# WarranWeng/EBFI-BE

Hardware: AMD Instinct MI355X
Metric: interpolated frames/sec (train fwd+bwd) at B=8 256x256 (higher is better)
Workload: dtype bf16x3 fwd (f16 KernelConv) / f16 bwd; 1 GPU; EVFIAutoEx (config/train_ours.yml defaults, 5.69 M params) train step: fwd + Lap/census loss + bwd + flat grad all-reduce + Adam; B=8 per GPU, 256x256 frames, TB=16 event bins, Poisson(0.35) event counts; global_batch=8, parallelism=dp1, world_size=1, launch=hipGraph replay of fwd+loss+bwd+grad packing; all-reduce and Adam eager, graph_capture_failed=False, fp16_steps_skipped=0

## Files before the change

ebfi-be_amd/csrc/conv2d.hip:

```cpp
#include <type_traits>

#include "common.hpp"
#include "c16.hpp"

using namespace ebfi;

namespace {

typedef float f32x16 __attribute__((ext_vector_type(16)));

enum { ACT_NONE = 0, ACT_LEAKY = 1, ACT_SIGMOID = 2 };

struct ConvGeom {
    int B, Cin, H, W, Cout, Ho, Wo, pad;
    int groups = 1;
    int store = 0;
};

struct EpiExtra {
    const float *addend;
    const float *mask_y;
    int mask_act;
    float mask_slope;
    _Float16 *out16 = nullptr;
    float *slot16 = nullptr;
    int planar16 = 0;
    const _Float16 *mask16 = nullptr;
    const float *post_scale = nullptr;
    const float *post_res = nullptr;
    int post_resC = 0;
    _Float16 *pre16 = nullptr;
    float *pre_slot = nullptr;
};

__device__ __forceinline__ float act_apply(float v, int act, float slope) {
    if (act == ACT_LEAKY) return v > 0.f ? v : v * slope;
    if (act == ACT_SIGMOID) return 1.f / (1.f + __expf(-v));
    return v;
}
__device__ __forceinline__ float act_grad(float y, int act, float slope) {
    if (act == ACT_LEAKY) return y > 0.f ? 1.f : slope;
    if (act == ACT_SIGMOID) return y * (1.f - y);
    return 1.f;
}

template <int DACT>
__device__ __forceinline__ float act_grad_c(float y, float slope) {
    if constexpr (DACT == ACT_LEAKY) return y > 0.f ? 1.f : slope;
    else if constexpr (DACT == ACT_SIGMOID) return y * (1.f - y);
    else return 1.f;
}

constexpr int TY = 4, TX = 64;

constexpr unsigned SENT = 0x80000000u;
__device__ __forceinline__ __amdgpu_buffer_rsrc_t make_rsrc(const float *p, unsigned bytes) {
    return __builtin_amdgcn_make_buffer_rsrc(const_cast<float *>(p), 0, bytes, 0x00020000);
}
template <int N>
__device__ __forceinline__ void wait_vmcnt() {
    static_assert(N >= 0 && N < 64, "vmcnt is a 6-bit counter");
    __builtin_amdgcn_s_waitcnt(((N >> 4) << 14) | (0x7 << 4) | (0xf << 8) | (N & 15));
}
__device__ __forceinline__ unsigned sel_off(bool ok, unsigned off) {
    asm volatile("" : "+v"(off));
    return ok ? off : 0x80000000u;
}
__device__ __forceinline__ float buf_ld(__amdgpu_buffer_rsrc_t r, unsigned byte_off) {
    return __uint_as_float(__builtin_amdgcn_raw_buffer_load_b32(r, byte_off, 0, 0));
}
__device__ __forceinline__ void buf_st(__amdgpu_buffer_rsrc_t r, unsigned byte_off, float v) {
    __builtin_amdgcn_raw_buffer_store_b32(__float_as_uint(v), r, byte_off, 0, 0);
}

template <int MT, int XM = 0>
__device__ __forceinline__ void store_out_tile(float *__restrict__ out, const float *__restrict__ bias, const f32x16 (&acc)[MT][2],
                                               const ConvGeom &g, int b, int co_base, int yo, int x0, int lane, int act,
                                               float slope, EpiExtra ex = EpiExtra{nullptr, nullptr, 0, 0.f}, float oscale = 1.f,
                                               float *amax16 = nullptr, float *amax_pre = nullptr) {
    const int HWo = g.Ho * g.Wo;
    const unsigned plane = (unsigned)HWo * 4u;
    constexpr bool EXTRA = (XM & 7) != 0, XAM = (XM & 1) != 0, X16 = (XM & 2) != 0, XRC = (XM & 4) != 0;
    constexpr bool XST = (XM & 8) != 0;
    if constexpr (EXTRA) {
        asm volatile("" : "+v"(lane));
    }
    const bool has32 = out != nullptr;
    const float *anyp = bias ? bias : (out ? out : reinterpret_cast<const float *>(ex.slot16));
    const __amdgpu_buffer_rsrc_t ro = make_rsrc(has32 ? out + (int64_t)b * g.Cout * HWo : anyp, has32 ? (unsigned)g.Cout * plane : 0u);
    const __amdgpu_buffer_rsrc_t rb = make_rsrc(bias ? bias : anyp, bias ? (unsigned)g.Cout * 4u : 0u);
    const bool has_a = XAM && ex.addend != nullptr, has_m = XAM && ex.mask_y != nullptr, has16 = X16 && ex.out16 != nullptr;
    const bool has_m16 = XAM && ex.mask16 != nullptr;
    const __amdgpu_buffer_rsrc_t ra = make_rsrc(has_a ? ex.addend + (int64_t)b * g.Cout * HWo : anyp, has_a ? (unsigned)g.Cout * plane : 0u);
    const __amdgpu_buffer_rsrc_t rm = make_rsrc(has_m ? ex.mask_y + (int64_t)b * g.Cout * HWo : anyp, has_m ? (unsigned)g.Cout * plane : 0u);
    const int cb16 = g.Cout >> 4;
    const bool planar = X16 && ex.planar16 != 0;
    const __amdgpu_buffer_rsrc_t rm16 = __builtin_amdgcn_make_buffer_rsrc(
        has_m16 ? const_cast<_Float16 *>(ex.mask16) + (int64_t)b * cb16 * HWo * 16 : const_cast<_Float16 *>(reinterpret_cast<const _Float16 *>(anyp)), 0,
        has_m16 ? (unsigned)cb16 * (unsigned)HWo * 32u : 0u, 0x00020000);
    const __amdgpu_buffer_rsrc_t r16 = __builtin_amdgcn_make_buffer_rsrc(
        has16 ? ex.out16 + (planar ? (int64_t)b * g.Cout * HWo : (int64_t)b * cb16 * HWo * 16)
              : const_cast<_Float16 *>(reinterpret_cast<const _Float16 *>(anyp)), 0,
        has16 ? (planar ? (unsigned)g.Cout * (unsigned)HWo * 2u : (unsigned)cb16 * (unsigned)HWo * 32u) : 0u, 0x00020000);
    const float s16 = has16 ? ex.slot16[0] : 1.f;
    const bool has_rc = XRC && ex.post_scale != nullptr;
    const __amdgpu_buffer_rsrc_t rps = make_rsrc(has_rc ? ex.post_scale + (int64_t)b * g.Cout : anyp, has_rc ? (unsigned)g.Cout * 4u : 0u);
    const __amdgpu_buffer_rsrc_t rrs = make_rsrc(has_rc ? ex.post_res + (int64_t)b * ex.post_resC * HWo : anyp,
                                                 has_rc ? (unsigned)ex.post_resC * plane : 0u);
    const bool has_p16 = has_rc && ex.pre16 != nullptr;
    const __amdgpu_buffer_rsrc_t rp16 = __builtin_amdgcn_make_buffer_rsrc(
        has_p16 ? ex.pre16 + (int64_t)b * cb16 * HWo * 16 : const_cast<_Float16 *>(reinterpret_cast<const _Float16 *>(anyp)), 0,
        has_p16 ? (unsigned)cb16 * (unsigned)HWo * 32u : 0u, 0x00020000);
    const float sp16 = has_p16 ? ex.pre_slot[0] : 1.f;
    const int res_shift = has_rc ? co_base - co_base % ex.post_resC : 0;
    float am = 0.f, amp = 0.f;
    const int h = lane >> 5, l31 = lane & 31;
    struct BlockIn {
        float add[8];
        float my[8];
        unsigned m16[4];
        float res[8];
    };
    auto shuffled_base = [&](int m) { return (unsigned)(((co_base + m * 32) >> 2) + h) * 4u * plane; };
    auto unshuffled_base = [&](int m, bool px_ok, int xo) {
        return px_ok ? (unsigned)(4 * (co_base + m * 32 + 4 * h) + 2 * (yo & 1) + (xo & 1)) * (plane >> 2) +
                           (unsigned)((yo >> 1) * (g.Wo >> 1) + (xo >> 1)) * 4u
                     : SENT;
    };
    auto blk_geom = [&](int m, int n, int j, bool &px_ok, unsigned &base, int &cblk, int &xo) {
        xo = x0 + n * 32 + l31;
        px_ok = yo < g.Ho && xo < g.Wo;
        base = (px_ok && co_base + m * 32 + 4 * h < g.Cout) ? (unsigned)(co_base + m * 32 + 4 * h) * plane + (unsigned)(yo * g.Wo + xo) * 4u : SENT;
        cblk = ((co_base + m * 32) >> 4) + j;
    };
    auto row_off = [](int j, int i) { return (unsigned)((i & 3) + 8 * (2 * j + (i >> 2))); };
    [[maybe_unused]] auto issue = [&](int m, int n, int j, BlockIn &in) {
        bool px_ok; unsigned base; int cblk, xo;
        blk_geom(m, n, j, px_ok, base, cblk, xo);
        if constexpr (XAM) {
            if (has_a) {
#pragma unroll
                for (int i = 0; i < 8; ++i) in.add[i] = buf_ld(ra, base + row_off(j, i) * plane);
            }
            if (has_m) {
#pragma unroll
                for (int i = 0; i < 8; ++i) in.my[i] = buf_ld(rm, base + row_off(j, i) * plane);
            }
            if (has_m16) {
                typedef unsigned u32x2_m __attribute__((ext_vector_type(2)));
                const unsigned om = (px_ok && cblk < cb16) ? ((unsigned)cblk * (unsigned)HWo * 2u + (unsigned)(yo * 2 * g.Wo + xo)) * 16u + 8u * (unsigned)h : SENT;
                const u32x2_m lo = __builtin_amdgcn_raw_buffer_load_b64(rm16, om, 0, 0);
                const u32x2_m hi = __builtin_amdgcn_raw_buffer_load_b64(rm16, om + (unsigned)g.Wo * 16u, 0, 0);
                in.m16[0] = lo.x; in.m16[1] = lo.y; in.m16[2] = hi.x; in.m16[3] = hi.y;
            }
        }
        if constexpr (XRC) {
            if (has_rc) {
                const unsigned rbase = base == SENT ? SENT : base - (unsigned)res_shift * plane;
#pragma unroll
                for (int i = 0; i < 8; ++i) in.res[i] = buf_ld(rrs, rbase + row_off(j, i) * plane);
            }
        }
    };
    [[maybe_unused]] auto finish = [&](int m, int n, int j, const BlockIn &in, auto actf) {
        bool px_ok; unsigned base; int cblk, xo;
        blk_geom(m, n, j, px_ok, base, cblk, xo);
        float u[8];
#pragma unroll
        for (int i = 0; i < 8; ++i) u[i] = acc[m][n][8 * j + i] * oscale;
        [[maybe_unused]] float psc[8];
        if constexpr (XRC) {
            if (has_rc) {
#pragma unroll
                for (int i = 0; i < 8; ++i) psc[i] = buf_ld(rps, (unsigned)(co_base + m * 32 + 4 * h) * 4u + row_off(j, i) * 4u);
            }
        }
        if (bias != nullptr) {
            float t[8];
#pragma unroll
            for (int i = 0; i < 8; ++i) t[i] = buf_ld(rb, (unsigned)(co_base + m * 32 + 4 * h) * 4u + row_off(j, i) * 4u);
#pragma unroll
            for (int i = 0; i < 8; ++i) u[i] += t[i];
        }
        if constexpr (XAM) {
            if (has_a) {
#pragma unroll
                for (int i = 0; i < 8; ++i) u[i] += in.add[i];
            }
        }
#pragma unroll
        for (int i = 0; i < 8; ++i) u[i] = actf(u[i]);
        if constexpr (XAM) {
            if (has_m) {
#pragma unroll
                for (int i = 0; i < 8; ++i) u[i] *= in.my[i] > 0.f ? 1.f : ex.mask_slope;
            }
            if (has_m16) {
#pragma unroll
                for (int i = 0; i < 8; ++i) {
                    const unsigned hbits = (in.m16[i >> 1] >> (16 * (i & 1))) & 0xffffu;
                    u[i] *= (hbits != 0u && hbits < 0x8000u) ? 1.f : ex.mask_slope;
                }
            }
        }
        if constexpr (XRC) {
            if (has_rc) {
                if (has_p16) {
                    const unsigned o16 = (px_ok && cblk < cb16) ? ((unsigned)cblk * (unsigned)HWo * 2u + (unsigned)((yo * 2 + h) * g.Wo + xo)) * 16u : SENT;
#pragma unroll
                    for (int i = 0; i < 8; ++i) amp = amax_acc(amp, u[i]);
                    const u32x4_c16 q = c16_gather_halves(pack_f16(u[0] * sp16, u[1] * sp16), pack_f16(u[2] * sp16, u[3] * sp16),
                                                          pack_f16(u[4] * sp16, u[5] * sp16), pack_f16(u[6] * sp16, u[7] * sp16));
                    __builtin_amdgcn_raw_buffer_store_b128(q, rp16, o16, 0, 0);
                }
#pragma unroll
                for (int i = 0; i < 8; ++i) u[i] = u[i] * psc[i] + in.res[i];
            }
        }
        if (has32) {
            if (XST && g.store == 1) {
                const unsigned b1 = px_ok ? shuffled_base(m) + (unsigned)(2 * yo * 2 * g.Wo + 2 * xo) * 4u : SENT;
#pragma unroll
                for (int q = 0; q < 2; ++q) {
#pragma unroll
                    for (int py = 0; py < 2; ++py) {
                        typedef float f32x2_st __attribute__((ext_vector_type(2)));
                        typedef unsigned u32x2_st __attribute__((ext_vector_type(2)));
                        const f32x2_st v{u[4 * q + 2 * py], u[4 * q + 2 * py + 1]};
                        __builtin_amdgcn_raw_buffer_store_b64(__builtin_bit_cast(u32x2_st, v), ro,
                                                              b1 + (unsigned)(2 * (2 * j + q)) * 4u * plane + (unsigned)(py * 2 * g.Wo) * 4u, 0, 0);
                    }
                }
            } else {
                const unsigned sb = (XST && g.store == 2) ? unshuffled_base(m, px_ok, xo) : base;
#pragma unroll
                for (int i = 0; i < 8; ++i) __builtin_amdgcn_raw_buffer_store_b32(__float_as_uint(u[i]), ro, sb + row_off(j, i) * plane, 0, 0);
            }
        }
        if constexpr (X16) {
            if (has16) {
#pragma unroll
                for (int i = 0; i < 8; ++i) am = amax_acc(am, u[i]);
                if (planar) {
                    const unsigned pb = (px_ok && co_base + m * 32 + 4 * h < g.Cout)
                                            ? (unsigned)(co_base + m * 32 + 4 * h) * (unsigned)HWo * 2u + (unsigned)(yo * g.Wo + xo) * 2u : SENT;
#pragma unroll
                    for (int i = 0; i < 8; ++i) {
                        const _Float16 hv = (_Float16)(u[i] * s16);
                        __builtin_amdgcn_raw_buffer_store_b16(__builtin_bit_cast(unsigned short, hv), r16, pb + row_off(j, i) * (unsigned)HWo * 2u, 0, 0);
                    }
                } else {
                    const u32x4_c16 q = c16_gather_halves(pack_f16(u[0] * s16, u[1] * s16), pack_f16(u[2] * s16, u[3] * s16),
                                                          pack_f16(u[4] * s16, u[5] * s16), pack_f16(u[6] * s16, u[7] * s16));
                    const unsigned o16 = (px_ok && cblk < cb16)
                                             ? ((unsigned)cblk * (unsigned)HWo * 2u + (unsigned)((yo * 2 + h) * g.Wo + xo)) * 16u : SENT;
                    __builtin_amdgcn_raw_buffer_store_b128(q, r16, o16, 0, 0);
                }
            }
        }
    };
    auto emit = [&](auto actf) {
        if constexpr (EXTRA) {
            constexpr int NBLK = MT * 4;
            BlockIn ia, ib;
            issue(0, 0, 0, ia);
#pragma unroll
            for (int k = 0; k < NBLK; ++k) {
                const int m = k >> 2, n = (k >> 1) & 1, j = k & 1;
                if (k + 1 < NBLK) issue((k + 1) >> 2, ((k + 1) >> 1) & 1, (k + 1) & 1, (k & 1) ? ia : ib);
                finish(m, n, j, (k & 1) ? ib : ia, actf);
                __builtin_amdgcn_sched_barrier(0);
            }
        } else {
#pragma unroll
            for (int m = 0; m < MT; ++m) {
                float bvm[16];
#pragma unroll
                for (int r = 0; r < 16; ++r) bvm[r] = buf_ld(rb, (unsigned)(co_base + m * 32 + (r & 3) + 8 * (r >> 2) + 4 * h) * 4u);
#pragma unroll
                for (int n = 0; n < 2; ++n) {
                    const int xo = x0 + n * 32 + l31;
                    const bool px_ok = yo < g.Ho && xo < g.Wo;
                    if (XST && g.store == 1) {
                        const unsigned b1 = px_ok ? shuffled_base(m) + (unsigned)(2 * yo * 2 * g.Wo + 2 * xo) * 4u : SENT;
#pragma unroll
                        for (int k = 0; k < 4; ++k) {
#pragma unroll
                            for (int py = 0; py < 2; ++py) {
                                typedef float f32x2_st __attribute__((ext_vector_type(2)));
                                typedef unsigned u32x2_st __attribute__((ext_vector_type(2)));
                                const int r = 4 * k + 2 * py;
                                const f32x2_st v{actf(acc[m][n][r] * oscale + bvm[r]), actf(acc[m][n][r + 1] * oscale + bvm[r + 1])};
                                __builtin_amdgcn_raw_buffer_store_b64(__builtin_bit_cast(u32x2_st, v), ro,
                                                                      b1 + (unsigned)(2 * k) * 4u * plane + (unsigned)(py * 2 * g.Wo) * 4u, 0, 0);
                            }
                        }
                        continue;
                    }
                    const unsigned base = (XST && g.store == 2) ? unshuffled_base(m, px_ok, xo)
                                          : (px_ok && co_base + m * 32 + 4 * h < g.Cout)
                                              ? (unsigned)(co_base + m * 32 + 4 * h) * plane + (unsigned)(yo * g.Wo + xo) * 4u : SENT;
#pragma unroll
                    for (int r = 0; r < 16; ++r)
                        __builtin_amdgcn_raw_buffer_store_b32(__float_as_uint(actf(acc[m][n][r] * oscale + bvm[r])), ro,
                                                              base + (unsigned)((r & 3) + 8 * (r >> 2)) * plane, 0, 0);
                }
            }
        }
    };
    if constexpr (EXTRA) {
        const float sl = act == ACT_LEAKY ? slope : 1.f;
        emit([sl](float v) { return v > 0.f ? v : v * sl; });
    } else {
        if (act == ACT_LEAKY) emit([slope](float v) { return v > 0.f ? v : v * slope; });
        else if (act == ACT_SIGMOID) emit([](float v) { return 1.f / (1.f + __expf(-v)); });
        else emit([](float v) { return v; });
    }
    if (amax16) *amax16 = amax_acc(*amax16, am);
    if constexpr (XRC) {
        if (amax_pre) *amax_pre = amax_acc(*amax_pre, amp);
    }
}

struct FacEpi {
    const float *ev;
    int C;
};

template <int MT>
__device__ __forceinline__ void fac_epilogue_tile(float *__restrict__ out, const float *__restrict__ bias, const f32x16 (&acc)[MT][2],
                                                  const ConvGeom &g, const FacEpi &fac, int b, int co_base, int yo, int x0, int lane,
                                                  float slope, float oscale = 1.f) {
    constexpr int K = 5, R = 2;
    const int HW = g.Ho * g.Wo;
    const int h = lane >> 5, l31 = lane & 31;
    const __amdgpu_buffer_rsrc_t rb = make_rsrc(bias, (unsigned)g.Cout * 4u);
    float part[MT][2];
#pragma unroll
    for (int m = 0; m < MT; ++m) {
        const int c = (co_base >> 5) + m;
        const bool c_ok = c < fac.C;
        const __amdgpu_buffer_rsrc_t rev = make_rsrc(fac.ev + ((int64_t)b * fac.C + (c_ok ? c : 0)) * HW, c_ok ? (unsigned)HW * 4u : 0u);
        float bv[16];
#pragma unroll
        for (int r = 0; r < 16; ++r) bv[r] = buf_ld(rb, (unsigned)(co_base + m * 32 + (r & 3) + 8 * (r >> 2) + 4 * h) * 4u);
#pragma unroll
        for (int n = 0; n < 2; ++n) {
            const int xo = x0 + n * 32 + l31;
            unsigned rowoff[K], coloff[K];
#pragma unroll
            for (int i = 0; i < K; ++i) {
                rowoff[i] = (unsigned)(min(max(yo + i - R, 0), g.Ho - 1) * g.Wo) * 4u;
                coloff[i] = (unsigned)min(max(xo + i - R, 0), g.Wo - 1) * 4u;
            }
            float e[16];
#pragma unroll
            for (int r = 0; r < 16; ++r) {
                constexpr int dummy = 0;
                const int t0 = (r & 3) + 8 * (r >> 2), t1 = t0 + 4;
                const unsigned o0 = t0 < K * K ? rowoff[t0 / K] + coloff[t0 % K] : rowoff[dummy] + coloff[dummy];
                const unsigned o1 = t1 < K * K ? rowoff[t1 / K] + coloff[t1 % K] : rowoff[dummy] + coloff[dummy];
                e[r] = buf_ld(rev, h ? o1 : o0);
            }
            float sum = 0.f;
#pragma unroll
            for (int r = 0; r < 16; ++r) {
                float f = acc[m][n][r] * oscale + bv[r];
                f = f > 0.f ? f : f * slope;
                sum = fmaf(f, e[r], sum);
            }
            part[m][n] = sum;
        }
    }
#pragma unroll
    for (int m = 0; m < MT; ++m) {
        const int c = (co_base >> 5) + m;
        const float p0 = part[m][0] + __shfl_xor(part[m][0], 32, 64);
        const float p1 = part[m][1] + __shfl_xor(part[m][1], 32, 64);
        const int xo = x0 + h * 32 + l31;
        if (c < fac.C && yo < g.Ho && xo < g.Wo) out[((int64_t)b * fac.C + c) * HW + (int64_t)yo * g.Wo + xo] = h ? p1 : p0;
    }
}

template <int KS, int S, int MT, int CK, bool TR, int DACT>
__global__ __launch_bounds__(256) void conv_fwd_f32(const float *__restrict__ x, const float *__restrict__ dact_y,
                                                    const float *__restrict__ w, const float *__restrict__ bias,
                                                    float *__restrict__ out, ConvGeom g, int act, float slope,
                                                    float dslope) {
    constexpr int KK = KS * KS;
    constexpr int IH = S * (TY - 1) + KS, IW = S * (TX - 1) + KS;
    constexpr int PS = IH * IW;
    constexpr int COS = 32 * MT;
    constexpr int COSP = TR ? COS + 4 : COS + 1;
    constexpr int NPOS = (PS + 255) / 256;
    constexpr int WEL = KK * CK * COS;
    constexpr int NW = (WEL + 255) / 256;
    __shared__ float sIn[CK * PS];
    __shared__ float sW[KK * CK * COSP];

    const int tid = threadIdx.x, lane = tid & 63, wave = tid >> 6;
    const int tiles_x = (g.Wo + TX - 1) / TX, tiles_y = (g.Ho + TY - 1) / TY;
    int t = blockIdx.x;
// ... 1786 lines not shown
int launch_wgrad_x3_w(hipStream_t st, const float *x, const float *gout, const float *yact, float *slab, float *gpre_out,
                      const ConvGeom &g, float dslope, int nsplit, int need_bias) {
    using C = WCfg<KS, 1, WTXO>;
    constexpr int CIB = CIBT ? CIBT : X3CIB<KS>::value;
    const size_t lds = (size_t)2 * (64 * GS + (CIB + 1) * C::PS) * sizeof(unsigned);
    if (int rc = ensure_dynamic_lds(reinterpret_cast<const void *>(&conv_wgrad_x3<KS, WTXO, DACT, WX, CIBT>), (int)lds)) return rc;
    const int64_t tiles = (int64_t)g.B * ceil_div(g.Ho, WTY) * ceil_div(g.Wo, C::WTX);
    dim3 grid((unsigned)nsplit, (unsigned)ceil_div(g.Cout, 64), (unsigned)ceil_div(g.Cin, CIB));
    ProfScope ps("conv_wgrad_x3", st, 2.0 * g.B * g.Ho * g.Wo * (double)g.Cout * g.Cin * KS * KS,
                 conv_bytes_wgrad(g, KS * KS, DACT != 0, gpre_out != nullptr));
    hipLaunchKernelGGL((conv_wgrad_x3<KS, WTXO, DACT, WX, CIBT>), grid, dim3(WX), lds, st, x, gout, yact, slab, gpre_out, g, dslope,
                       (int)tiles, need_bias);
    return check_launch("conv_wgrad_x3");
}

template <int DACT>
int launch_wgrad_x3_ws(hipStream_t st, const float *x, const float *gout, const float *yact, float *slab, float *gpre_out,
                       const ConvGeom &g, float dslope, int nsplit, int need_bias) {
    using C = WCfg<3, 1, 32>;
    const size_t lds = (size_t)2 * (64 * GS + 65 * C::PS) * sizeof(unsigned);
    if (int rc = ensure_dynamic_lds(reinterpret_cast<const void *>(&conv_wgrad_x3_ws<DACT>), (int)lds)) return rc;
    const int64_t tiles = (int64_t)g.B * ceil_div(g.Ho, WTY) * ceil_div(g.Wo, C::WTX);
    dim3 grid((unsigned)nsplit, (unsigned)ceil_div(g.Cout, 64), (unsigned)ceil_div(g.Cin, 64));
    ProfScope ps("conv_wgrad_x3_ws", st, 2.0 * g.B * g.Ho * g.Wo * (double)g.Cout * g.Cin * 9,
                 conv_bytes_wgrad(g, 9, DACT != 0, gpre_out != nullptr));
    hipLaunchKernelGGL((conv_wgrad_x3_ws<DACT>), grid, dim3(512), lds, st, x, gout, yact, slab, gpre_out, g, dslope, (int)tiles, need_bias);
    return check_launch("conv_wgrad_x3_ws");
}

template <int KS, int WTXO, int DACT>
int launch_wgrad_x3_d(hipStream_t st, const float *x, const float *gout, const float *yact, float *slab, float *gpre_out,
                      const ConvGeom &g, float dslope, int nsplit, int need_bias) {
    if constexpr (KS == 3) {
        if (wgrad_x3_ws(g, KS)) return launch_wgrad_x3_ws<DACT>(st, x, gout, yact, slab, gpre_out, g, dslope, nsplit, need_bias);
        if (wgrad_x3_small_wg(g, KS))
            return launch_wgrad_x3_w<KS, WTXO, DACT, 256, 32>(st, x, gout, yact, slab, gpre_out, g, dslope, nsplit, need_bias);
    }
    return launch_wgrad_x3_w<KS, WTXO, DACT, WXT, 0>(st, x, gout, yact, slab, gpre_out, g, dslope, nsplit, need_bias);
}

template <int KS, int WTXO>
int launch_wgrad_x3_t(hipStream_t st, const float *x, const float *gout, const float *yact, float *slab, float *gpre_out,
                      const ConvGeom &g, int dact, float dslope, int nsplit, int need_bias) {
    if (dact == ACT_LEAKY) return launch_wgrad_x3_d<KS, WTXO, ACT_LEAKY>(st, x, gout, yact, slab, gpre_out, g, dslope, nsplit, need_bias);
    if (dact == ACT_SIGMOID) return launch_wgrad_x3_d<KS, WTXO, ACT_SIGMOID>(st, x, gout, yact, slab, gpre_out, g, dslope, nsplit, need_bias);
    return launch_wgrad_x3_d<KS, WTXO, ACT_NONE>(st, x, gout, yact, slab, gpre_out, g, dslope, nsplit, need_bias);
}

int launch_wgrad_x3(hipStream_t st, const float *x, const float *gout, const float *yact, float *slab, float *gpre_out,
                    const ConvGeom &g, int ks, int dact, float dslope, int nsplit, int need_bias) {
    if (ks == 1) return launch_wgrad_x3_t<1, 0>(st, x, gout, yact, slab, gpre_out, g, dact, dslope, nsplit, need_bias);
    if (ks == 7) return launch_wgrad_x3_t<7, 32>(st, x, gout, yact, slab, gpre_out, g, dact, dslope, nsplit, need_bias);
    return launch_wgrad_x3_t<3, 32>(st, x, gout, yact, slab, gpre_out, g, dact, dslope, nsplit, need_bias);
}

template <int KS, int DACT>
int launch_wgrad_bf16_d(hipStream_t st, const float *x, const float *gout, const float *yact, float *slab, const ConvGeom &g,
                        float dslope, int nsplit, int need_bias) {
    using C = WCfgB<KS>;
    const size_t lds = (size_t)C::LDS_ELEMS * 2;
    if (int rc = ensure_dynamic_lds(reinterpret_cast<const void *>(&conv_wgrad_bf16<KS, DACT>), (int)lds)) return rc;
    const int64_t tiles = (int64_t)g.B * ceil_div(g.Ho, WTY) * ceil_div(g.Wo, C::WTX);
    dim3 grid((unsigned)nsplit, (unsigned)ceil_div(g.Cout, 64), (unsigned)ceil_div(g.Cin, C::CIB));
    ProfScope ps("conv_wgrad_bf16", st, 2.0 * g.B * g.Ho * g.Wo * (double)g.Cout * g.Cin * KS * KS,
                 conv_bytes_wgrad(g, KS * KS, DACT != 0, false));
    hipLaunchKernelGGL((conv_wgrad_bf16<KS, DACT>), grid, dim3(256), lds, st, x, gout, yact, slab, g, dslope, (int)tiles,
                       need_bias);
    return check_launch("conv_wgrad_bf16");
}

template <int KS>
int launch_wgrad_bf16(hipStream_t st, const float *x, const float *gout, const float *yact, float *slab, const ConvGeom &g,
                      int dact, float dslope, int nsplit, int need_bias) {
    if (dact == ACT_LEAKY) return launch_wgrad_bf16_d<KS, ACT_LEAKY>(st, x, gout, yact, slab, g, dslope, nsplit, need_bias);
    if (dact == ACT_SIGMOID) return launch_wgrad_bf16_d<KS, ACT_SIGMOID>(st, x, gout, yact, slab, g, dslope, nsplit, need_bias);
    return launch_wgrad_bf16_d<KS, ACT_NONE>(st, x, gout, yact, slab, g, dslope, nsplit, need_bias);
}

constexpr int NTWS = 768;
template <int XM, bool FAC = false>
__global__ __launch_bounds__(NTWS) void conv_fwd_bf16x3_ws(const float *__restrict__ x, const __bf16 *__restrict__ wp,
                                                           const float *__restrict__ bias, float *__restrict__ out, ConvGeom g, int K16,
                                                           int act, float slope, EpiExtra epi, int tiles_total, FacEpi fac) {
    constexpr bool EXTRA = (XM & 7) != 0;
    constexpr int KS = 3, KK = 9, MT = 2;
    constexpr int IH = TYB - 1 + KS, IW = TX - 1 + KS, PS = IH * IW, COS = 32 * MT;
    constexpr int NCW = 8, PT = 256;
    constexpr int WPIECES = KK * COS * 2, NWB = (2 * WPIECES + PT - 1) / PT;
    constexpr int INB = PS * 32, WB = KK * COS * 32, BUFB = 2 * INB + 2 * WB;
    extern __shared__ __attribute__((aligned(16))) char smd[];
    const int tid = threadIdx.x, lane = tid & 63, wave = tid >> 6;
    const int tiles_x = (g.Wo + TX - 1) / TX, tiles_y = (g.Ho + TYB - 1) / TYB;
    const int co_base = blockIdx.y * COS;
    const int grp = co_base / (g.Cout / g.groups);
    const int HW = g.H * g.W;
    const unsigned plane_bytes = (unsigned)HW * 4u, x_bytes = (unsigned)g.Cin * plane_bytes;
    const int nchunks = K16 / CKB;
    const int G = gridDim.x;
    int ntiles_mine = 0;
    for (int t = blockIdx.x; t < tiles_total; t += G) ++ntiles_mine;
    const int nitems = ntiles_mine * nchunks;
    const bool xcd_map = (gridDim.x & 7) == 0;
    auto tile_coords = [&](int tt, int &tb, int &ty0, int &tx0) {
        int u = xcd_map ? xcd_tile(tt, tiles_total) : tt;
        const int txi = u % tiles_x; u /= tiles_x;
        const int tyi = u % tiles_y;
        tb = u / tiles_y; ty0 = tyi * TYB; tx0 = txi * TX;
    };

    if (wave < NCW) {
        __builtin_amdgcn_s_setprio(1);
        f32x16 acc[MT][2];
#pragma unroll
        for (int m = 0; m < MT; ++m)
#pragma unroll
            for (int n = 0; n < 2; ++n)
#pragma unroll
                for (int e = 0; e < 16; ++e) acc[m][n][e] = 0.f;
        const int hsel = lane >> 5, l31 = lane & 31;
        const int a_lane = 2 * INB + l31 * 32 + ((hsel ^ ((l31 >> 3) & 1)) << 4);
        const int pbase = wave * IW + l31;
        unsigned fbits = 0;
#pragma unroll
        for (int tap = 0; tap < KK; ++tap)
            fbits |= (unsigned)((((pbase + (tap / KS) * IW + (tap % KS)) >> 3) & 1) ^ hsel) << tap;
        bf16x8 ah[2][MT], al[2][MT], bh[2][2], bl[2][2];
        [[maybe_unused]] float amax16 = 0.f, amax_pre = 0.f;
        auto tap_read = [&](const char *base, int tap, int set) {
            const int ky = tap / KS, kx = tap - ky * KS;
            const char *bp = base + pbase * 32 + (int)(((fbits >> tap) & 1u) << 4) + (ky * IW + kx) * 32;
            const char *ap = base + a_lane + tap * COS * 32;
#pragma unroll
            for (int m = 0; m < MT; ++m) {
                ah[set][m] = *reinterpret_cast<const bf16x8 *>(ap + m * 1024);
#ifndef ABL_ONE_MFMA
                al[set][m] = *reinterpret_cast<const bf16x8 *>(ap + m * 1024 + WB);
#endif
            }
#pragma unroll
            for (int n = 0; n < 2; ++n) {
                bh[set][n] = *reinterpret_cast<const bf16x8 *>(bp + n * 1024);
#ifndef ABL_ONE_MFMA
                bl[set][n] = *reinterpret_cast<const bf16x8 *>(bp + n * 1024 + INB);
#endif
            }
        };
        auto tap_mfma = [&](int set) {
#pragma unroll
            for (int m = 0; m < MT; ++m)
#pragma unroll
                for (int n = 0; n < 2; ++n) {
#ifndef ABL_ONE_MFMA
                    acc[m][n] = __builtin_amdgcn_mfma_f32_32x32x16_bf16(al[set][m], bh[set][n], acc[m][n], 0, 0, 0);
                    acc[m][n] = __builtin_amdgcn_mfma_f32_32x32x16_bf16(ah[set][m], bl[set][n], acc[m][n], 0, 0, 0);
#endif
                    acc[m][n] = __builtin_amdgcn_mfma_f32_32x32x16_bf16(ah[set][m], bh[set][n], acc[m][n], 0, 0, 0);
                }
        };
        __syncthreads();
        int item = 0, tcur = blockIdx.x;
        for (int ti = 0; ti < ntiles_mine; ++ti, tcur += G) {
            for (int chunk = 0; chunk < nchunks; ++chunk, ++item) {
                const char *base = smd + (item & 1) * BUFB;
#ifdef WSF_NO_CONSUME
                if (g.pad != 12345) { } else
#endif
                {
                    tap_read(base, 0, 0);
#pragma unroll
                    for (int tap = 0; tap < KK; ++tap) {
                        if (tap + 1 < KK) tap_read(base, tap + 1, (tap + 1) & 1);
                        __builtin_amdgcn_sched_barrier(0);
                        tap_mfma(tap & 1);
                        __builtin_amdgcn_sched_barrier(0);
                    }
                }
                __syncthreads();
            }
            int cb_, cy0, cx0;
            tile_coords(tcur, cb_, cy0, cx0);
            if constexpr (FAC) {
                fac_epilogue_tile<MT>(out, bias, acc, g, fac, cb_, co_base, cy0 + wave, cx0, lane, slope);
            } else {
                if constexpr ((XM & 6) != 0) saturate_fp16_conversions(true);
                store_out_tile<MT, XM>(out, bias, acc, g, cb_, co_base, cy0 + wave, cx0, lane, act, slope, epi, 1.f, &amax16, &amax_pre);
                if constexpr ((XM & 6) != 0) saturate_fp16_conversions(false);
            }
#pragma unroll
            for (int m = 0; m < MT; ++m)
#pragma unroll
                for (int n = 0; n < 2; ++n)
#pragma unroll
                    for (int e = 0; e < 16; ++e) acc[m][n][e] = 0.f;
        }
        if constexpr (EXTRA) {
            if (epi.out16 != nullptr) ScaleSlot{epi.slot16}.record(amax16);
            if constexpr ((XM & 4) != 0) {
                if (epi.pre16 != nullptr) ScaleSlot{epi.pre_slot}.record(amax_pre);
            }
        }
        return;
    }
    const int ptid = tid - 64 * NCW;
    const unsigned img_bytes = (unsigned)KK * (unsigned)g.Cout * (unsigned)K16 * 2u;
    const __amdgpu_buffer_rsrc_t rwt = __builtin_amdgcn_make_buffer_rsrc(const_cast<__bf16 *>(wp), 0, 2u * img_bytes, 0x00020000);
    constexpr int SH = (4 - (KS / 2) % 4) % 4;
    constexpr int NQ = (IW + SH + 3) / 4;
    constexpr int NITEM = IH * NQ * 2;
    constexpr int NIT = (NITEM + PT - 1) / PT;
    int it_qh[NIT], it_qr[NIT], it_qq[NIT];
#pragma unroll
    for (int k = 0; k < NIT; ++k) {
        const int id = ptid + k * PT;
        it_qh[k] = id & 1;
        it_qr[k] = (id >> 1) / NQ;
        it_qq[k] = (id >> 1) - it_qr[k] * NQ;
    }
    unsigned w_off[NWB];
    int w_dst[NWB];
#pragma unroll
    for (int it = 0; it < NWB; ++it) {
        const int i = ptid + it * PT;
        const int sel = i >= WPIECES ? 1 : 0, j = i - sel * WPIECES;
        const int row = j >> 1, half = j & 1;
        const int tap = row / COS, co = row - tap * COS;
        w_off[it] = i < 2 * WPIECES ? (unsigned)sel * img_bytes + (unsigned)(((tap * g.Cout + co_base + co) * K16 + half * 8) * 2) : SENT;
        w_dst[it] = 2 * INB + sel * WB + row * 32 + ((half ^ ((row >> 3) & 1)) << 4);
    }
    u32x4 rq[NIT][8];
    u32x4 rw[NWB];
    int pf_tile = blockIdx.x, pf_chunk = 0;
    unsigned pf_off[NIT];
    const float *pf_src = x;
    unsigned pf_bytes = 0u;
    auto pf_setup = [&]() {
        const bool live = pf_tile < tiles_total;
        int tb, ty0, tx0;
        tile_coords(live ? pf_tile : 0, tb, ty0, tx0);
#pragma unroll
        for (int k = 0; k < NIT; ++k) {
            const int yy = ty0 - g.pad + it_qr[k], xq = tx0 - g.pad - SH + 4 * it_qq[k];
            const bool ok = live && ptid + k * PT < NITEM && yy >= 0 && yy < g.H && xq >= 0 && xq + 3 < g.W;
            pf_off[k] = ok ? (unsigned)(yy * g.W + xq) * 4u + (unsigned)(8 * it_qh[k]) * plane_bytes : SENT;
        }
        pf_src = x + ((int64_t)tb * g.groups + grp) * g.Cin * HW;
        pf_bytes = live ? x_bytes : 0u;
    };
    auto prefetch = [&]() {
        const __amdgpu_buffer_rsrc_t r = make_rsrc(pf_src, pf_bytes);
        const unsigned cb = (unsigned)pf_chunk * (unsigned)CKB * plane_bytes;
#pragma unroll
        for (int k = 0; k < NIT; ++k)
#pragma unroll
            for (int c = 0; c < 8; ++c) rq[k][c] = __builtin_amdgcn_raw_buffer_load_b128(r, pf_off[k] + cb + (unsigned)c * plane_bytes, 0, 0);
        const unsigned wb = (unsigned)pf_chunk * (unsigned)(CKB * 2);
#pragma unroll
        for (int it = 0; it < NWB; ++it) {
#ifdef ABL_ONE_MFMA
            if (ptid + it * PT >= WPIECES) continue;
#endif
            rw[it] = __builtin_amdgcn_raw_buffer_load_b128(rwt, w_off[it] + wb, 0, 0);
        }
        if (++pf_chunk == nchunks) {
            pf_chunk = 0;
            pf_tile += G;
            pf_setup();
        }
    };
    auto commit = [&](int buf) {
        char *base = smd + buf * BUFB;
#pragma unroll
        for (int k = 0; k < NIT; ++k)
            if (ptid + k * PT < NITEM) {
#pragma unroll
                for (int j = 0; j < 4; ++j) {
                    const int c = 4 * it_qq[k] + j - SH;
                    if (c < 0 || c >= IW) continue;
                    u32x4 hv, lv;
#pragma unroll
                    for (int e = 0; e < 8; e += 2) {
                        const float v0 = __uint_as_float(rq[k][e][j]), v1 = __uint_as_float(rq[k][e + 1][j]);
                        const __bf16 a0 = (__bf16)v0, a1 = (__bf16)v1;
                        hv[e >> 1] = pack_bf16((float)a0, (float)a1);
                        lv[e >> 1] = pack_bf16(v0 - (float)a0, v1 - (float)a1);
                    }
                    const int pos = it_qr[k] * IW + c;
                    const int d = pos * 32 + ((it_qh[k] ^ ((pos >> 3) & 1)) << 4);
                    *reinterpret_cast<u32x4 *>(base + d) = hv;
#ifndef ABL_ONE_MFMA
                    *reinterpret_cast<u32x4 *>(base + INB + d) = lv;
#endif
                }
            }
#pragma unroll
        for (int it = 0; it < NWB; ++it) {
#ifdef ABL_ONE_MFMA
            if (ptid + it * PT >= WPIECES) continue;
#endif
            if (ptid + it * PT < 2 * WPIECES) *reinterpret_cast<u32x4 *>(base + w_dst[it]) = rw[it];
        }
    };
    pf_setup();
    prefetch();
    commit(0);
    prefetch();
    __syncthreads();
    for (int item = 0; item < nitems; ++item) {
#ifndef WSF_NO_PRODUCE
        commit((item + 1) & 1);
        prefetch();
#endif
        __syncthreads();
    }
}

#include "conv2d_f16.inc.hpp"
#include "conv2d_thin.inc.hpp"
#include "conv2d_shift.inc.hpp"

size_t bf16_pack_bytes(int M, int K, int ks) { return (size_t)ks * ks * M * (size_t)((K + 15) / 16 * 16) * 2; }

template <int KS>
int launch_fwd_bf16(hipStream_t st, const float *x, const float *dact_y, const float *w, const float *bias, float *out,
                    const ConvGeom &g, int transposed, int act, float slope, int dact, float dslope, void *workspace,
                    size_t ws_bytes, int x3 = 0, EpiExtra epi = EpiExtra{nullptr, nullptr, 0, 0.f}) {
    const int K16 = (g.Cin + 15) / 16 * 16;
    const size_t need = bf16_pack_bytes(g.Cout, g.Cin, KS) * (x3 ? 2 : 1);
    if (!workspace || ws_bytes < need) return fail(EBFI_ERR_WORKSPACE, "conv2d bf16: workspace %zu bytes < required %zu", ws_bytes, need);
    __bf16 *wp = static_cast<__bf16 *>(workspace);
    const int64_t total = (int64_t)KS * KS * g.Cout * K16;
    if (w != nullptr) {
        ProfScope ps("conv_pack_w_bf16", st);
        hipLaunchKernelGGL(conv_pack_w_bf16, dim3((unsigned)ceil_div(total, 256)), dim3(256), 0, st, w, wp, g.Cout, g.Cin, K16,
                           KS * KS, transposed, x3);
        if (int rc = check_launch("conv_pack_w_bf16")) return rc;
    }
    const int ty = x3 ? TYB : TY;
    const int64_t tiles = (int64_t)g.B * ceil_div(g.Ho, ty) * ceil_div(g.Wo, TX);
    if (tiles > 2147483647LL) return fail(EBFI_ERR_ARG, "conv2d: too many tiles");
    const char *name = x3 ? (transposed ? "conv_fwd_bf16x3_db/dgrad" : "conv_fwd_bf16x3_db/fwd")
                          : (transposed ? "conv_fwd_bf16/dgrad" : "conv_fwd_bf16/fwd");
    const double flops = 2.0 * g.B * g.Ho * g.Wo * (double)g.Cout * g.Cin * KS * KS;
    const bool few = x3 && epi.out16 == nullptr && epi.post_scale == nullptr && g.store == 0 && tiles * ceil_div(g.Cout, 64) <= 128;
    const int mt = (g.Cout <= 32 || few) ? 1 : 2;
    dim3 grid((unsigned)tiles, (unsigned)ceil_div(g.Cout, 32 * mt));
    if (g.store != 0 && !x3) return fail(EBFI_ERR_UNSUPPORTED, "conv2d: shuffled output layouts are written by the split-precision kernels only");
    if (x3) {
        constexpr int PSX = (TYB - 1 + KS) * (TX - 1 + KS);
        const size_t lds = (size_t)2 * (2 * PSX * 32 + 2 * KS * KS * 32 * mt * 32) + KB_LDS_BYTES;
        const bool vec4 = g.W % 4 == 0 && g.pad == KS / 2 && aligned16(x) && (!dact_y || aligned16(dact_y));
        const bool extra = epi.addend != nullptr || epi.mask_y != nullptr || epi.out16 != nullptr || epi.post_scale != nullptr;
        const bool use_ws = KS == 3 && mt == 2 && vec4 && dact == ACT_NONE;
        if (epi.out16 != nullptr && !use_ws)
            return fail(EBFI_ERR_UNSUPPORTED, "conv2d: the fp16 side image is written by the wave-specialised 3x3 kernel only "
                        "(W %% 4 == 0, same padding, more than 32 output channels, 16-byte aligned input)");
        if (epi.post_scale != nullptr && !use_ws)
            return fail(EBFI_ERR_UNSUPPORTED, "conv2d: the ResidualControl epilogue is written by the wave-specialised 3x3 kernel only");
        if (g.store != 0 && (!use_ws || extra))
            return fail(EBFI_ERR_UNSUPPORTED, "conv2d: a shuffled output layout is written by the wave-specialised 3x3 kernel only (W %% 4 == 0, "
                        "same padding, more than 32 output channels, 16-byte aligned input), without epilogue extras");
        if (use_ws) name = transposed ? "conv_fwd_bf16x3_ws/dgrad" : (epi.post_scale ? "conv_fwd_bf16x3_ws/fwd_rc" :
                                                                      (epi.out16 ? "conv_fwd_bf16x3_ws/fwd_img" :
                                                                       (g.store ? "conv_fwd_bf16x3_ws/fwd_shuffle" : "conv_fwd_bf16x3_ws/fwd")));
        ProfScope ps(name, st, flops, conv_bytes_fwd(g, KS * KS, dact != 0));
#define EBFI_LAUNCH_X3V(MT_, DA_, VEC_)                                                                                   \
    do {                                                                                                                 \
        if (int rc_ = ensure_dynamic_lds(reinterpret_cast<const void *>(&conv_fwd_bf16x3_db<KS, MT_, DA_, VEC_>), 160 * 1024)) \
            return rc_;                                                                                                  \
        hipLaunchKernelGGL((conv_fwd_bf16x3_db<KS, MT_, DA_, VEC_>), (VEC_ == 1 && DA_ == 0 && KS == 3) ? pgrid : grid,    \
                           dim3(NTB), lds, st, x, dact_y, wp, bias, out, g, K16, act, slope, dslope, epi, (int)tiles);   \
    } while (0)
#define EBFI_LAUNCH_X3(MT_, DA_)                                                                                          \
    do {                                                                                                                 \
        if constexpr (DA_ != ACT_NONE) {                                                                                 \
            if (vec == 4) EBFI_LAUNCH_X3V(MT_, DA_, 4);                                                                  \
            else EBFI_LAUNCH_X3V(MT_, DA_, 1);                                                                           \
        } else EBFI_LAUNCH_X3V(MT_, DA_, 1);                                                                             \
    } while (0)
        const int vec = vec4 && dact != ACT_NONE ? 4 : 1;
        const int64_t co_blocks = ceil_div(g.Cout, 32 * mt);
        int64_t gx = 256 / co_blocks;
        if (gx < 1) gx = 1;
        if (gx > tiles) gx = tiles;
        const dim3 pgrid((unsigned)gx, (unsigned)co_blocks);
        if constexpr (KS == 3) {
            if (use_ws) {
#define EBFI_LAUNCH_X3WS(XM_)                                                                                              \
    do {                                                                                                                   \
        if (int rc_ = ensure_dynamic_lds(reinterpret_cast<const void *>(&conv_fwd_bf16x3_ws<XM_>), 160 * 1024)) return rc_; \
        hipLaunchKernelGGL((conv_fwd_bf16x3_ws<XM_>), pgrid, dim3(NTWS), lds, st, x, wp, bias, out, g, K16, act, slope, epi,  \
                           (int)tiles, FacEpi{nullptr, 0});                                                               \
    } while (0)
                const bool xam = epi.addend != nullptr || epi.mask_y != nullptr, x16 = epi.out16 != nullptr;
                if (epi.post_scale != nullptr) {
                    if (xam) return fail(EBFI_ERR_UNSUPPORTED, "conv2d: the ResidualControl epilogue comes without addend / mask");
                    if (x16) EBFI_LAUNCH_X3WS(6);
                    else EBFI_LAUNCH_X3WS(4);
                }
                else if (g.store != 0) EBFI_LAUNCH_X3WS(8);
                else if (xam && x16) EBFI_LAUNCH_X3WS(3);
                else if (x16) EBFI_LAUNCH_X3WS(2);
                else if (xam) EBFI_LAUNCH_X3WS(1);
                else EBFI_LAUNCH_X3WS(0);
#undef EBFI_LAUNCH_X3WS
                return check_launch(name);
            }
        }
        if (mt == 1) {
            if (dact == ACT_LEAKY) EBFI_LAUNCH_X3(1, ACT_LEAKY);
            else if (dact == ACT_SIGMOID) EBFI_LAUNCH_X3(1, ACT_SIGMOID);
            else EBFI_LAUNCH_X3(1, ACT_NONE);
        } else {
            if (dact == ACT_LEAKY) EBFI_LAUNCH_X3(2, ACT_LEAKY);
            else if (dact == ACT_SIGMOID) EBFI_LAUNCH_X3(2, ACT_SIGMOID);
            else EBFI_LAUNCH_X3(2, ACT_NONE);
        }
#undef EBFI_LAUNCH_X3V
#undef EBFI_LAUNCH_X3
        return check_launch(name);
    }
    {
        ProfScope ps(name, st, flops, conv_bytes_fwd(g, KS * KS, dact != 0));
#define EBFI_LAUNCH_BF16(MT_, DA_)                                                                                     \
    hipLaunchKernelGGL((conv_fwd_bf16<KS, MT_, DA_>), grid, dim3(256), 0, st, x, dact_y, wp, bias, out, g, K16, act, slope, \
                       dslope)
        if (mt == 1) {
            if (dact == ACT_LEAKY) EBFI_LAUNCH_BF16(1, ACT_LEAKY);
            else if (dact == ACT_SIGMOID) EBFI_LAUNCH_BF16(1, ACT_SIGMOID);
            else EBFI_LAUNCH_BF16(1, ACT_NONE);
        } else {
            if (dact == ACT_LEAKY) EBFI_LAUNCH_BF16(2, ACT_LEAKY);
            else if (dact == ACT_SIGMOID) EBFI_LAUNCH_BF16(2, ACT_SIGMOID);
            else EBFI_LAUNCH_BF16(2, ACT_NONE);
        }
#undef EBFI_LAUNCH_BF16
    }
    return check_launch(name);
}

}

extern "C" size_t ebfi_conv2d_bf16_workspace(int Cin, int Cout, int ksize) {
    const int m = Cin > Cout ? Cin : Cout;
    return 2 * bf16_pack_bytes(m, m, ksize);
}

namespace {
constexpr int C7_IH = TYB + 6, C7_IW = TX + 6, C7_PS = C7_IH * C7_IW;
constexpr int C7_INB = C7_PS * 32, C7_ROWS = 16, C7_WB = 49 * C7_ROWS * 32;
constexpr int C7_LDS = 2 * C7_INB + 2 * C7_WB;
constexpr int C7_NPOS = (C7_PS + NTB - 1) / NTB;
constexpr int C7_PIECES = 49 * C7_ROWS * 2;
constexpr int C7_NWP = (C7_PIECES + NTB - 1) / NTB;

__global__ __launch_bounds__(NTB) void conv7_x3_kernel(const float *__restrict__ x, const float *__restrict__ w,
                                                       const float *__restrict__ bias, float *__restrict__ out, int K, int H,
                                                       int W, int M, int Ho, int Wo, int pad, int tr, int act, float slope) {
    extern __shared__ __attribute__((aligned(16))) char smd[];
    const int tid = threadIdx.x, lane = tid & 63, wave = tid >> 6;
    const int tiles_x = (Wo + TX - 1) / TX, tiles_y = (Ho + TYB - 1) / TYB;
    int t = (gridDim.x & 7) == 0 ? xcd_tile((int)blockIdx.x, (int)gridDim.x) : (int)blockIdx.x;
    const int tx = t % tiles_x; t /= tiles_x;
    const int ty = t % tiles_y;
    const int b = t / tiles_y;
    const int y0 = ty * TYB, x0 = tx * TX;
    const int iy0 = y0 - pad, ix0 = x0 - pad;
    const unsigned plane_bytes = (unsigned)(H * W) * 4u;
    const __amdgpu_buffer_rsrc_t rx = make_rsrc(x + (int64_t)b * K * H * W, (unsigned)K * plane_bytes);
    const __amdgpu_buffer_rsrc_t rw = make_rsrc(w, (unsigned)(M * K * 49) * 4u);

    unsigned in_off[C7_NPOS];
    int in_dst[C7_NPOS];
#pragma unroll
    for (int q = 0; q < C7_NPOS; ++q) {
        const int pos = tid + q * NTB;
        const int r = pos / C7_IW, c = pos - r * C7_IW;
        const int yy = iy0 + r, xx = ix0 + c;
// ... 669 lines not shown
        return fail(EBFI_ERR_UNSUPPORTED, "kernelconv_fac_fused_x3: needs W %% 4 == 0 and a 16-byte aligned input (W = %d)", W);
    if (B == 0) return EBFI_OK;
    hipStream_t st = static_cast<hipStream_t>(stream);
    const int64_t tiles = (int64_t)B * ceil_div(g.Ho, TYB) * ceil_div(g.Wo, TX);
    if (tiles > 2147483647LL) return fail(EBFI_ERR_ARG, "kernelconv_fac_fused_x3: too many tiles");
    constexpr int PSX = (TYB - 1 + 3) * (TX - 1 + 3);
    const size_t lds = (size_t)2 * (2 * PSX * 32 + 2 * 9 * 32 * 2 * 32) + KB_LDS_BYTES;
    const int64_t co_blocks = ceil_div(g.Cout, 64);
    int64_t gx = 256 / co_blocks;
    if (gx < 1) gx = 1;
    if (gx > tiles) gx = tiles;
    const double flops = 2.0 * B * g.Ho * g.Wo * (double)(C * 25) * Cin * 9 + 2.0 * B * g.Ho * g.Wo * (double)C * 25;
    const double bytes = 4.0 * B * (double)g.Ho * g.Wo * (Cin + 2.0 * C);
    ProfScope ps("conv_fwd_bf16x3_ws/kernelconv_fac", st, flops, bytes);
    if (int rc = ensure_dynamic_lds(reinterpret_cast<const void *>(&conv_fwd_bf16x3_ws<0, true>), 160 * 1024)) return rc;
    hipLaunchKernelGGL((conv_fwd_bf16x3_ws<0, true>), dim3((unsigned)gx, (unsigned)co_blocks), dim3(NTWS), lds, st,
                       static_cast<const float *>(input), static_cast<const __bf16 *>(packed), static_cast<const float *>(bias32),
                       static_cast<float *>(output), g, K16, ACT_LEAKY, slope, EpiExtra{nullptr, nullptr, 0, 0.f}, (int)tiles,
                       FacEpi{static_cast<const float *>(feat), C});
    return check_launch("conv_fwd_bf16x3_ws/kernelconv_fac");
}

extern "C" int ebfi_kernelconv_fac_fused_f16(const void *input, int input_is_c16, const void *packed16, size_t packed_bytes,
                                             const void *bias32, const void *feat, void *output, int B, int Cin, int H, int W, int C,
                                             int fac_ksize, float slope, void *in_slot, const void *w_slot, void *stream) {
    if (!input || !packed16 || !bias32 || !feat || !output || !in_slot || !w_slot)
        return fail(EBFI_ERR_ARG, "kernelconv_fac_fused_f16: null argument");
    if (fac_ksize != 5) return fail(EBFI_ERR_UNSUPPORTED, "kernelconv_fac_fused_f16: FAC kernel size %d (5 is built)", fac_ksize);
    if (C < 1) return fail(EBFI_ERR_ARG, "kernelconv_fac_fused_f16: %d channels", C);
    ConvGeom g;
    if (int rc = make_geom(g, B, Cin, H, W, C * 32, 3, 1, 1)) return rc;
    if ((int64_t)(Cin + 64) * H * W * 4 >= (1LL << 31) - (1LL << 26))
        return fail(EBFI_ERR_ARG, "kernelconv_fac_fused_f16: one sample exceeds the 2 GiB reach of 32-bit buffer offsets");
    const int K16 = (Cin + 15) / 16 * 16;
    const size_t need = (size_t)9 * g.Cout * K16 * 2;
    if (packed_bytes < need) return fail(EBFI_ERR_WORKSPACE, "kernelconv_fac_fused_f16: packed image %zu bytes < required %zu", packed_bytes, need);
    if (W % 4 != 0 || !aligned16(input))
        return fail(EBFI_ERR_UNSUPPORTED, "kernelconv_fac_fused_f16: needs W %% 4 == 0 and a 16-byte aligned input (W = %d)", W);
    if (input_is_c16 != 0 && input_is_c16 != 1) return fail(EBFI_ERR_ARG, "kernelconv_fac_fused_f16: input storage %d", input_is_c16);
    if (input_is_c16 && Cin % 16 != 0) return fail(EBFI_ERR_UNSUPPORTED, "kernelconv_fac_fused_f16: an fp16 input image needs Cin %% 16 == 0");
    if (B == 0) return EBFI_OK;
    hipStream_t st = static_cast<hipStream_t>(stream);
    const int64_t tiles = (int64_t)B * ceil_div(g.Ho, TYB) * ceil_div(g.Wo, TX);
    if (tiles > 2147483647LL) return fail(EBFI_ERR_ARG, "kernelconv_fac_fused_f16: too many tiles");
    constexpr int PSX = (TYB - 1 + 3) * (TX - 1 + 3);
    const size_t lds = (size_t)2 * (PSX * 32 + 9 * 64 * 32) + KB_LDS_BYTES;
    const int64_t co_blocks = ceil_div(g.Cout, 64);
    int64_t gx = 256 / co_blocks;
    if (gx < 1) gx = 1;
    if (gx > tiles) gx = tiles;
    const double flops = 2.0 * B * g.Ho * g.Wo * (double)(C * 25) * Cin * 9 + 2.0 * B * g.Ho * g.Wo * (double)C * 25;
    const double bytes = B * (double)g.Ho * g.Wo * ((input_is_c16 ? 2.0 : 4.0) * Cin + 8.0 * C);
    ProfScope ps(input_is_c16 ? "conv_fwd_f16_ws/kernelconv_fac_img" : "conv_fwd_f16_ws/kernelconv_fac", st, flops, bytes);
#define EBFI_LAUNCH_FACF16(IN_)                                                                                          \
    do {                                                                                                                 \
        if (int rc = ensure_dynamic_lds(reinterpret_cast<const void *>(&conv_fwd_f16_ws<false, IN_, false, true>), 160 * 1024)) return rc; \
        hipLaunchKernelGGL((conv_fwd_f16_ws<false, IN_, false, true>), dim3((unsigned)gx, (unsigned)co_blocks), dim3(NTF16), lds, st, \
                           static_cast<const float *>(input), static_cast<const _Float16 *>(packed16),                   \
                           static_cast<const float *>(bias32), static_cast<float *>(output), g, K16, ACT_LEAKY, slope,   \
                           EpiExtra{nullptr, nullptr, 0, 0.f}, (int)tiles, ScaleSlot{static_cast<float *>(in_slot)},    \
                           static_cast<const float *>(w_slot), FacEpi{static_cast<const float *>(feat), C});             \
    } while (0)
    if (input_is_c16) EBFI_LAUNCH_FACF16(true);
    else EBFI_LAUNCH_FACF16(false);
#undef EBFI_LAUNCH_FACF16
    return check_launch("conv_fwd_f16_ws/kernelconv_fac");
}

extern "C" int ebfi_conv2d_packed_f16_c16(const void *input, int input_is_c16, const void *packed16, size_t packed_bytes,
                                          const void *bias, void *output, int B, int Cin_per_group, int H, int W, int Cout, int ksize,
                                          int pad, int groups, int act, float slope, const void *addend, const void *mask_y,
                                          int mask_act, float mask_slope, void *in_slot, const void *w_slot, void *out16,
                                          void *slot16, int out16_planar, int mask_is_c16, void *stream);
extern "C" int ebfi_conv2d_packed_f16(const void *input, const void *packed16, size_t packed_bytes, const void *bias, void *output,
                                      int B, int Cin_per_group, int H, int W, int Cout, int ksize, int pad, int groups, int act,
                                      float slope, const void *addend, const void *mask_y, int mask_act, float mask_slope,
                                      void *in_slot, const void *w_slot, void *stream) {
    if (!output) return fail(EBFI_ERR_ARG, "conv2d_packed_f16: null argument");
    return ebfi_conv2d_packed_f16_c16(input, 0, packed16, packed_bytes, bias, output, B, Cin_per_group, H, W, Cout, ksize, pad, groups,
                                      act, slope, addend, mask_y, mask_act, mask_slope, in_slot, w_slot, nullptr, nullptr, 0, 0, stream);
}

namespace {
int packed_f16_impl(const void *input, int input_is_c16, const void *packed16, size_t packed_bytes,
                    const void *bias, void *output, int B, int Cin_per_group, int H, int W, int Cout, int ksize,
                    int pad, int groups, int act, float slope, const void *addend, const void *mask_y,
                    int mask_act, float mask_slope, void *in_slot, const void *w_slot, void *out16,
                    void *slot16, int out16_planar, int mask_is_c16, int out_layout, void *stream);
}

extern "C" int ebfi_conv2d_packed_f16_c16(const void *input, int input_is_c16, const void *packed16, size_t packed_bytes,
                                          const void *bias, void *output, int B, int Cin_per_group, int H, int W, int Cout, int ksize,
                                          int pad, int groups, int act, float slope, const void *addend, const void *mask_y,
                                          int mask_act, float mask_slope, void *in_slot, const void *w_slot, void *out16,
                                          void *slot16, int out16_planar, int mask_is_c16, void *stream) {
    return packed_f16_impl(input, input_is_c16, packed16, packed_bytes, bias, output, B, Cin_per_group, H, W, Cout, ksize, pad, groups, act,
                           slope, addend, mask_y, mask_act, mask_slope, in_slot, w_slot, out16, slot16, out16_planar, mask_is_c16, 0, stream);
}

extern "C" int ebfi_conv2d_packed_f16_shuffled(const void *input, int input_is_c16, const void *packed16, size_t packed_bytes,
                                               const void *bias, void *output, int B, int Cin, int H, int W, int Cout, int act, float slope,
                                               const void *mask_y, int mask_act, float mask_slope, void *in_slot, const void *w_slot,
                                               int out_layout, void *stream) {
    return packed_f16_impl(input, input_is_c16, packed16, packed_bytes, bias, output, B, Cin, H, W, Cout, 3, 1, 1, act, slope, nullptr, mask_y,
                           mask_act, mask_slope, in_slot, w_slot, nullptr, nullptr, 0, 0, out_layout, stream);
}

namespace {
int packed_f16_impl(const void *input, int input_is_c16, const void *packed16, size_t packed_bytes,
                    const void *bias, void *output, int B, int Cin_per_group, int H, int W, int Cout, int ksize,
                    int pad, int groups, int act, float slope, const void *addend, const void *mask_y,
                    int mask_act, float mask_slope, void *in_slot, const void *w_slot, void *out16,
                    void *slot16, int out16_planar, int mask_is_c16, int out_layout, void *stream) {
    if (!input || !packed16 || (!output && !out16)) return fail(EBFI_ERR_ARG, "conv2d_packed_f16: null argument");
    if ((out16 != nullptr) != (slot16 != nullptr)) return fail(EBFI_ERR_ARG, "conv2d_packed_f16: out16 and slot16 come together");
    if (out16 && !out16_planar && (Cout % 16 != 0 || !aligned16(out16)))
        return fail(EBFI_ERR_UNSUPPORTED, "conv2d_packed_f16: fp16 output image needs Cout %% 16 == 0");
    if (mask_is_c16 && mask_y && (Cout % 16 != 0 || !aligned16(mask_y)))
        return fail(EBFI_ERR_UNSUPPORTED, "conv2d_packed_f16: an fp16 mask image needs Cout %% 16 == 0");
    if (out16_planar && (!out16 || output || W % 4 != 0 || !aligned16(out16)))
        return fail(EBFI_ERR_UNSUPPORTED, "conv2d_packed_f16: planar fp16 output comes alone (output NULL), W %% 4 == 0");
    if (input_is_c16 < 0 || input_is_c16 > 2) return fail(EBFI_ERR_ARG, "conv2d_packed_f16: input storage %d", input_is_c16);
    if (input_is_c16 == 1 && (Cin_per_group % 16 != 0 || !in_slot))
        return fail(EBFI_ERR_UNSUPPORTED, "conv2d_packed_f16: an fp16 input image needs Cin %% 16 == 0 and its scale slot");
    if (input_is_c16 == 2 && !in_slot) return fail(EBFI_ERR_ARG, "conv2d_packed_f16: a planar fp16 input needs its scale slot");
    if (act < 0 || act > 2 || mask_act < 0 || mask_act > 2) return fail(EBFI_ERR_ARG, "conv2d_packed_f16: unknown activation");
    if (ksize != 3 || pad != 1) return fail(EBFI_ERR_UNSUPPORTED, "conv2d_packed_f16: 3x3 same-padded convolutions only (k=%d pad=%d)", ksize, pad);
    if (groups < 1 || Cout % groups != 0 || (groups > 1 && (Cout / groups) % 64 != 0))
        return fail(EBFI_ERR_ARG, "conv2d_packed_f16: %d output channels in %d groups (groups need multiples of 64 channels)", Cout, groups);
    if ((input_is_c16 != 1 && W % 4 != 0) || !aligned16(input))
        return fail(EBFI_ERR_UNSUPPORTED, "conv2d_packed_f16: needs W %% 4 == 0 and a 16-byte aligned input (W = %d)", W);
    ConvGeom g;
    if (int rc = make_geom(g, B, Cin_per_group, H, W, Cout, ksize, 1, pad)) return rc;
    if ((int64_t)groups * (Cin_per_group + 64) * H * W * 4 >= (1LL << 31) - (1LL << 26) || (int64_t)(Cout + 64) * H * W * 4 >= (1LL << 31) - (1LL << 26))
        return fail(EBFI_ERR_ARG, "conv2d_packed_f16: one sample exceeds the 2 GiB reach of 32-bit buffer offsets");
    g.groups = groups;
    if (int rc = check_out_layout("conv2d_packed_f16", out_layout, Cout, g.Ho, g.Wo, output, addend, out16)) return rc;
    g.store = out_layout;
    const int K16 = (g.Cin + 15) / 16 * 16;
    const size_t need = (size_t)9 * g.Cout * K16 * 2;
    if (packed_bytes < need) return fail(EBFI_ERR_WORKSPACE, "conv2d_packed_f16: packed image %zu bytes < required %zu", packed_bytes, need);
    if (B == 0) return EBFI_OK;
    hipStream_t st = static_cast<hipStream_t>(stream);
    if ((addend || mask_y || out16) && (act == ACT_SIGMOID || mask_act == ACT_SIGMOID))
        return fail(EBFI_ERR_UNSUPPORTED, "conv2d_packed_f16: the epilogue extras take LeakyReLU / no activation only");
    const bool m16 = mask_is_c16 != 0 && mask_y != nullptr && mask_act == ACT_LEAKY;
    const EpiExtra epi{static_cast<const float *>(addend), (mask_act == ACT_LEAKY && !m16) ? static_cast<const float *>(mask_y) : nullptr,
                       mask_act, mask_slope, static_cast<_Float16 *>(out16), static_cast<float *>(slot16), out16_planar ? 1 : 0,
                       m16 ? static_cast<const _Float16 *>(mask_y) : nullptr};
    const int64_t tiles = (int64_t)B * ceil_div(g.Ho, TYB) * ceil_div(g.Wo, TX);
    if (tiles > 2147483647LL) return fail(EBFI_ERR_ARG, "conv2d_packed_f16: too many tiles");
    constexpr int PSX = (TYB - 1 + 3) * (TX - 1 + 3);
    const size_t lds = (size_t)2 * (PSX * 32 + 9 * 64 * 32) + KB_LDS_BYTES;
    const int64_t co_blocks = ceil_div(g.Cout, 64);
    int64_t gx = 256 / co_blocks;
    if (gx < 1) gx = 1;
    if (gx > tiles) gx = tiles;
    const dim3 grid((unsigned)gx, (unsigned)co_blocks);
    const bool extra = epi.addend != nullptr || epi.mask_y != nullptr || epi.mask16 != nullptr || epi.out16 != nullptr;
    const double flops = 2.0 * g.B * g.Ho * g.Wo * (double)g.Cout * g.Cin * 9;
    const double px = (double)g.B * g.Ho * g.Wo;
    const double io_bytes = px * g.groups * g.Cin * (input_is_c16 ? 2.0 : 4.0) + px * g.Cout * ((output ? 4.0 : 0.0) + (out16 ? 2.0 : 0.0)) +
                            px * g.Cout * ((addend ? 4.0 : 0.0) + (mask_y ? (m16 ? 2.0 : 4.0) : 0.0)) + 2.0 * 9 * (double)g.Cout * g.Cin;
    ProfScope ps(g.store ? (input_is_c16 ? "conv_fwd_f16_ws/img_shuffle" : "conv_fwd_f16_ws/f32_shuffle") :
                 input_is_c16 == 2 ? "conv_fwd_f16_ws/p16_f32" : out16_planar ? (input_is_c16 ? "conv_fwd_f16_ws/img_p16" : "conv_fwd_f16_ws/f32_p16") :
                 input_is_c16 ? (out16 ? (output ? "conv_fwd_f16_ws/img_both" : "conv_fwd_f16_ws/img_img") : "conv_fwd_f16_ws/img_f32")
                              : (out16 ? "conv_fwd_f16_ws/f32_img" : "conv_fwd_f16_ws/f32_f32"), st, flops, io_bytes);
    const ScaleSlot isl{static_cast<float *>(in_slot)};
    const float *x = static_cast<const float *>(input), *bs = static_cast<const float *>(bias);
    const _Float16 *wp = static_cast<const _Float16 *>(packed16);
    float *o = static_cast<float *>(output);
#define EBFI_LAUNCH_F16WS(EX_, IN_)                                                                                      \
    do {                                                                                                                 \
        if (int rc_ = ensure_dynamic_lds(reinterpret_cast<const void *>(&conv_fwd_f16_ws<EX_, IN_>), 160 * 1024)) return rc_; \
        hipLaunchKernelGGL((conv_fwd_f16_ws<EX_, IN_>), grid, dim3(NTF16), lds, st, x, wp, bs, o, g, K16, act, slope, epi,   \
                           (int)tiles, isl, static_cast<const float *>(w_slot), FacEpi{nullptr, 0});                    \
    } while (0)
    if (input_is_c16 == 2) {
        if (extra || g.store) return fail(EBFI_ERR_UNSUPPORTED, "conv2d_packed_f16: planar fp16 input with epilogue extras / a shuffled output");
        if (int rc_ = ensure_dynamic_lds(reinterpret_cast<const void *>(&conv_fwd_f16_ws<false, false, true>), 160 * 1024)) return rc_;
        hipLaunchKernelGGL((conv_fwd_f16_ws<false, false, true>), grid, dim3(NTF16), lds, st, x, wp, bs, o, g, K16, act, slope, epi,
                           (int)tiles, isl, static_cast<const float *>(w_slot), FacEpi{nullptr, 0});
    } else if (g.store != 0) {
#define EBFI_LAUNCH_F16ST(IN_)                                                                                           \
    do {                                                                                                                 \
        if (int rc_ = ensure_dynamic_lds(reinterpret_cast<const void *>(&conv_fwd_f16_ws<true, IN_, false, false, true>), 160 * 1024)) return rc_; \
        hipLaunchKernelGGL((conv_fwd_f16_ws<true, IN_, false, false, true>), grid, dim3(NTF16), lds, st, x, wp, bs, o, g, K16, act, slope, epi, \
                           (int)tiles, isl, static_cast<const float *>(w_slot), FacEpi{nullptr, 0});                    \
    } while (0)
        if (input_is_c16) EBFI_LAUNCH_F16ST(true);
        else EBFI_LAUNCH_F16ST(false);
#undef EBFI_LAUNCH_F16ST
    } else if (extra && input_is_c16) EBFI_LAUNCH_F16WS(true, true);
    else if (extra) EBFI_LAUNCH_F16WS(true, false);
    else if (input_is_c16) EBFI_LAUNCH_F16WS(false, true);
    else EBFI_LAUNCH_F16WS(false, false);
#undef EBFI_LAUNCH_F16WS
    return check_launch("conv_fwd_f16_ws");
}
}

extern "C" int ebfi_conv2d_backward_weight_f16g_ex(const void *input, const void *grad_output, const void *saved_output,
                                                   void *grad_weight, void *grad_bias, void *grad_preact_out, int grad_preact_is_c16,
                                                   int B, int Cin_per_group, int H, int W, int Cout, int ksize, int pad, int groups,
                                                   int act, float slope, void *x_slot, void *g_slot, void *workspace,
                                                   size_t workspace_bytes, void *stream);
extern "C" int ebfi_conv2d_backward_weight_f16g(const void *input, const void *grad_output, const void *saved_output,
                                                void *grad_weight, void *grad_bias, void *grad_preact_out, int B,
                                                int Cin_per_group, int H, int W, int Cout, int ksize, int pad, int groups, int act,
                                                float slope, void *x_slot, void *g_slot, void *workspace,
                                                size_t workspace_bytes, void *stream) {
    return ebfi_conv2d_backward_weight_f16g_ex(input, grad_output, saved_output, grad_weight, grad_bias, grad_preact_out, 0, B,
                                               Cin_per_group, H, W, Cout, ksize, pad, groups, act, slope, x_slot, g_slot, workspace,
                                               workspace_bytes, stream);
}

extern "C" int ebfi_conv2d_backward_weight_f16g_ex(const void *input, const void *grad_output, const void *saved_output,
                                                   void *grad_weight, void *grad_bias, void *grad_preact_out, int grad_preact_is_c16,
                                                   int B, int Cin_per_group, int H, int W, int Cout, int ksize, int pad, int groups,
                                                   int act, float slope, void *x_slot, void *g_slot, void *workspace,
                                                   size_t workspace_bytes, void *stream) {
    if (!input || !grad_output || !grad_weight) return fail(EBFI_ERR_ARG, "conv2d_backward_weight_f16g: null argument");
    const bool gp16 = grad_preact_is_c16 != 0 && grad_preact_out != nullptr;
    if (gp16 && (act == ACT_NONE || Cout % 16 != 0 || !g_slot))
        return fail(EBFI_ERR_ARG, "conv2d_backward_weight_f16g: an fp16 image of grad * act' needs an activation, Cout %% 16 == 0 and g_slot");
    if (ksize != 3) return fail(EBFI_ERR_UNSUPPORTED, "conv2d_backward_weight_f16g: k=%d", ksize);
    const bool ragged_ci = Cin_per_group % 64 != 0;
    if (ragged_ci && (groups != 1 || Cin_per_group < 16))
        return fail(EBFI_ERR_UNSUPPORTED, "conv2d_backward_weight_f16g: %d input channels per group", Cin_per_group);
    if (act < 0 || act > 2 || (act != ACT_NONE && !saved_output)) return fail(EBFI_ERR_ARG, "conv2d_backward_weight_f16g: activation / saved_output");
    if (groups < 1 || Cout % groups != 0 || (groups > 1 && (Cout / groups) % 64 != 0))
        return fail(EBFI_ERR_ARG, "conv2d_backward_weight_f16g: %d output channels in %d groups", Cout, groups);
    ConvGeom g;
    if (int rc = make_geom(g, B, Cin_per_group, H, W, Cout, ksize, 1, pad)) return rc;
    g.groups = groups;
    const size_t need = ebfi_conv2d_backward_weight_workspace(B, Cin_per_group, H, W, Cout, ksize, 1, pad, EBFI_F32);
    if (!workspace || workspace_bytes < need)
        return fail(EBFI_ERR_WORKSPACE, "conv2d_backward_weight_f16g: workspace %zu bytes < required %zu", workspace_bytes, need);
    hipStream_t st = static_cast<hipStream_t>(stream);
    const int64_t n_weight = (int64_t)Cout * Cin_per_group * 9, n_total = n_weight + Cout;
    if (B == 0) {
        (void)hipMemsetAsync(grad_weight, 0, (size_t)n_weight * sizeof(float), st);
        if (grad_bias) (void)hipMemsetAsync(grad_bias, 0, (size_t)Cout * sizeof(float), st);
        return EBFI_OK;
    }
    float *slab = static_cast<float *>(workspace);
    if (!gp16) {
        if (const ShiftPlan sp = shift_wgrad_plan(g, 3, 1, input, grad_output, saved_output, grad_preact_out); sp.kind != 0)
            return launch_wgrad_shift(st, sp, static_cast<const float *>(input), static_cast<const float *>(grad_output),
                                      static_cast<const float *>(saved_output), static_cast<float *>(grad_preact_out), slab, g, act, slope,
                                      static_cast<float *>(grad_weight), static_cast<float *>(grad_bias));
        if (const ThinPlan tp = thin_wgrad_plan(g, 3, 1, input, grad_output, saved_output, grad_preact_out); tp.kind != 0)
            return launch_wgrad_thin(st, tp, static_cast<const float *>(input), static_cast<const float *>(grad_output),
                                     static_cast<const float *>(saved_output), static_cast<float *>(grad_preact_out), slab, g, 3, act, slope,
                                     static_cast<float *>(grad_weight), static_cast<float *>(grad_bias));
    }
    int nsplit = wgrad_x3_splits(g, 3);
    const int64_t tr_tiles = (int64_t)g.B * ceil_div(g.Ho, TRH) * ceil_div(g.Wo, TRW);
    const bool tr_ok = pad == 1 && W % 4 == 0 && aligned16(input) && aligned16(grad_output) &&
                       (act == ACT_NONE || aligned16(saved_output)) && (!grad_preact_out || aligned16(grad_preact_out));
    if (tr_ok) {
        const int64_t tiles = tr_tiles;
        if (tiles > 2147483647LL) return fail(EBFI_ERR_ARG, "conv2d_backward_weight_f16g: too many tiles");
        if (nsplit > tiles) nsplit = (int)tiles;
        dim3 grid((unsigned)nsplit, (unsigned)ceil_div(g.Cout, 64), (unsigned)ceil_div(g.Cin, 64));
        const ScaleSlot xs{static_cast<float *>(x_slot)}, gs{static_cast<float *>(g_slot)};
        ProfScope ps("conv_wgrad_f16_tr/f32", st, 2.0 * g.B * g.Ho * g.Wo * (double)g.Cout * g.Cin * 9,
                     conv_bytes_wgrad(g, 9, act != ACT_NONE, grad_preact_out != nullptr) -
                         (gp16 ? 2.0 * g.B * g.Ho * g.Wo * (double)g.Cout : 0.0));
#define EBFI_LAUNCH_WTR(DA_)                                                                                               \
    do {                                                                                                                   \
        if (int rc_ = ensure_dynamic_lds(reinterpret_cast<const void *>(&conv_wgrad_f16_tr<DA_>), TR_LDS + KB_LDS_BYTES)) return rc_;       \
        hipLaunchKernelGGL((conv_wgrad_f16_tr<DA_>), grid, dim3(512), TR_LDS + KB_LDS_BYTES, st, static_cast<const float *>(input),           \
                           static_cast<const float *>(grad_output), static_cast<const float *>(saved_output),              \
                           static_cast<float *>(grad_preact_out), slab, g, slope, (int)tiles, grad_bias != nullptr ? 1 : 0,  \
                           xs, gs, gp16 ? 1 : 0);                                                                          \
    } while (0)
        if (act == ACT_LEAKY) EBFI_LAUNCH_WTR(ACT_LEAKY);
        else if (act == ACT_SIGMOID) EBFI_LAUNCH_WTR(ACT_SIGMOID);
        else EBFI_LAUNCH_WTR(ACT_NONE);
#undef EBFI_LAUNCH_WTR
        if (int rc = check_launch("conv_wgrad_f16_tr")) return rc;
// ... 219 lines not shown
```

ebfi-be_amd/csrc/conv2d_f16.inc.hpp:

```cpp


constexpr int NTF16 = 512;
template <bool EXTRA, bool IN16 = false, bool INP16 = false, bool FAC = false, bool ST = false>
__global__ __launch_bounds__(NTF16) void conv_fwd_f16_ws(const float *__restrict__ x, const _Float16 *__restrict__ wp,
                                                         const float *__restrict__ bias, float *__restrict__ out, ConvGeom g, int K16,
                                                         int act, float slope, EpiExtra epi, int tiles_total, ScaleSlot in_slot,
                                                         const float *__restrict__ w_slot, FacEpi fac) {
    static_assert(!FAC || (!EXTRA && !INP16), "the FAC epilogue comes without epilogue extras (input: fp32 planes or a c16 image)");
    constexpr int KS = 3, KK = 9, MT = 2, RW = 2;
    constexpr int IH = TYB - 1 + KS, IW = TX - 1 + KS, PS = IH * IW, COS = 32 * MT;
    constexpr int NCW = TYB / RW, PT = 256;
    constexpr int WPIECES = KK * COS * 2, NWB = (WPIECES + PT - 1) / PT;
    constexpr int INB = PS * 32, WB = KK * COS * 32, BUFB = INB + WB;
    static_assert(NCW == 4 && NTF16 == 64 * NCW + PT, "wave roles");
    extern __shared__ __attribute__((aligned(16))) char smd[];
    const int tid = threadIdx.x, lane = tid & 63, wave = tid >> 6;
    const int tiles_x = (g.Wo + TX - 1) / TX, tiles_y = (g.Ho + TYB - 1) / TYB;
    const int co_base = blockIdx.y * COS;
    const int grp = co_base / (g.Cout / g.groups);
    const int HW = g.H * g.W;
    constexpr unsigned ES = INP16 ? 2u : 4u;
    const unsigned plane_bytes = (unsigned)HW * ES, x_bytes = (unsigned)g.Cin * plane_bytes;
    const int nchunks = K16 / CKB;
    const int G = gridDim.x;
    int ntiles_mine = 0;
    for (int t = blockIdx.x; t < tiles_total; t += G) ++ntiles_mine;
    const int nitems = ntiles_mine * nchunks;
    constexpr int NSTG = IN16 ? 3 : 2;
    const int nitems_pad = (nitems + NSTG - 1) / NSTG * NSTG;
    const bool xcd_map = (gridDim.x & 7) == 0;
    auto tile_coords = [&](int tt, int &tb, int &ty0, int &tx0) {
        int u = xcd_map ? xcd_tile(tt, tiles_total) : tt;
        const int txi = u % tiles_x; u /= tiles_x;
        const int tyi = u % tiles_y;
        tb = u / tiles_y; ty0 = tyi * TYB; tx0 = txi * TX;
    };
    const float sx = in_slot.scale();
    [[maybe_unused]] constexpr int KB_LDS_OFF = 2 * BUFB;
    KB_CLEAR_SELF();
    KB_STAMP(0);

    if (wave < NCW) {
        __builtin_amdgcn_s_setprio(1);
        f32x16 acc[RW][MT][2];
#pragma unroll
        for (int r = 0; r < RW; ++r)
#pragma unroll
            for (int m = 0; m < MT; ++m)
#pragma unroll
                for (int n = 0; n < 2; ++n)
#pragma unroll
                    for (int e = 0; e < 16; ++e) acc[r][m][n][e] = 0.f;
        const float oscale = 1.f / (sx * (w_slot ? w_slot[0] : 1.f));
        [[maybe_unused]] float amax16 = 0.f;
        const int hsel = lane >> 5, l31 = lane & 31;
        const int a_lane = INB + l31 * 32 + ((hsel ^ ((l31 >> 3) & 1)) << 4);
        const int pbase = RW * wave * IW + l31;
        unsigned fbits = 0;
#pragma unroll
        for (int r = 0; r < RW; ++r)
#pragma unroll
            for (int tap = 0; tap < KK; ++tap)
                fbits |= (unsigned)((((pbase + r * IW + (tap / KS) * IW + (tap % KS)) >> 3) & 1) ^ hsel) << (r * KK + tap);
        f16x8 af[2][MT], bf[2][RW][2];
        auto tap_read = [&](const char *base, int tap, int set) {
            const int ky = tap / KS, kx = tap - ky * KS;
            const char *ap = base + a_lane + tap * COS * 32;
#pragma unroll
            for (int m = 0; m < MT; ++m) af[set][m] = *reinterpret_cast<const f16x8 *>(ap + m * 1024);
#pragma unroll
            for (int r = 0; r < RW; ++r) {
                const char *bp = base + (pbase + r * IW) * 32 + (int)(((fbits >> (r * KK + tap)) & 1u) << 4) + (ky * IW + kx) * 32;
#pragma unroll
                for (int n = 0; n < 2; ++n) bf[set][r][n] = *reinterpret_cast<const f16x8 *>(bp + n * 1024);
            }
        };
        auto tap_mfma = [&](int set) {
#pragma unroll
            for (int r = 0; r < RW; ++r)
#pragma unroll
                for (int m = 0; m < MT; ++m)
#pragma unroll
                    for (int n = 0; n < 2; ++n)
                        acc[r][m][n] = __builtin_amdgcn_mfma_f32_32x32x16_f16(af[set][m], bf[set][r][n], acc[r][m][n], 0, 0, 0);
        };
        __syncthreads();
        KB_STAMP(1);
        int item = 0, tcur = blockIdx.x;
        for (int ti = 0; ti < ntiles_mine; ++ti, tcur += G) {
            for (int chunk = 0; chunk < nchunks; ++chunk, ++item) {
                const char *base = smd + (item & 1) * BUFB;
                if (item < 12) KB_STAMP(2 + 2 * item);
                tap_read(base, 0, 0);
#pragma unroll
                for (int tap = 0; tap < KK; ++tap) {
                    if (tap + 1 < KK) tap_read(base, tap + 1, (tap + 1) & 1);
                    __builtin_amdgcn_sched_barrier(0);
                    tap_mfma(tap & 1);
                    __builtin_amdgcn_sched_barrier(0);
                }
                if (item < 12) KB_STAMP(3 + 2 * item);
                __syncthreads();
            }
            KB_STAMP(30);
            int cb_, cy0, cx0;
            tile_coords(tcur, cb_, cy0, cx0);
            static_assert(RW == 2, "epilogue is written out for two rows");
            if constexpr (FAC) {
                fac_epilogue_tile<MT>(out, bias, acc[0], g, fac, cb_, co_base, cy0 + RW * wave, cx0, lane, slope, oscale);
                fac_epilogue_tile<MT>(out, bias, acc[1], g, fac, cb_, co_base, cy0 + RW * wave + 1, cx0, lane, slope, oscale);
            } else {
                if constexpr (EXTRA) saturate_fp16_conversions(true);
                store_out_tile<MT, (EXTRA ? 3 : 0) | (ST ? 8 : 0)>(out, bias, acc[0], g, cb_, co_base, cy0 + RW * wave, cx0, lane, act, slope, epi, oscale, &amax16);
                store_out_tile<MT, (EXTRA ? 3 : 0) | (ST ? 8 : 0)>(out, bias, acc[1], g, cb_, co_base, cy0 + RW * wave + 1, cx0, lane, act, slope, epi, oscale, &amax16);
                if constexpr (EXTRA) saturate_fp16_conversions(false);
            }
#pragma unroll
            for (int r = 0; r < RW; ++r)
#pragma unroll
                for (int m = 0; m < MT; ++m)
#pragma unroll
                    for (int n = 0; n < 2; ++n)
#pragma unroll
                        for (int e = 0; e < 16; ++e) acc[r][m][n][e] = 0.f;
        }
        for (int k = nitems; k < nitems_pad; ++k) __syncthreads();
        KB_STAMP(31);
        KB_FLUSH_SELF();
        if constexpr (EXTRA) {
            if (epi.out16 != nullptr) ScaleSlot{epi.slot16}.record(amax16);
        }
        return;
    }
    saturate_fp16_conversions();
    KB_STAMP(20);
    const int ptid = tid - 64 * NCW;
    const unsigned img_bytes = (unsigned)KK * (unsigned)g.Cout * (unsigned)K16 * 2u;
    const __amdgpu_buffer_rsrc_t rwt = __builtin_amdgcn_make_buffer_rsrc(const_cast<_Float16 *>(wp), 0, img_bytes, 0x00020000);
    if constexpr (IN16) {
        constexpr int NPIECE = PS * 2, NPK = (NPIECE + PT - 1) / PT;
        int p_row[NPK], p_col[NPK], p_half[NPK], p_dst[NPK];
#pragma unroll
        for (int k = 0; k < NPK; ++k) {
            const int id = ptid + k * PT;
            const int t = id / IW;
            p_col[k] = id - t * IW;
            p_half[k] = t & 1;
            p_row[k] = t >> 1;
            const int pos = p_row[k] * IW + p_col[k];
            p_dst[k] = pos * 32 + ((p_half[k] ^ ((pos >> 3) & 1)) << 4);
        }
        unsigned w_off[NWB];
        int w_dst[NWB];
#pragma unroll
        for (int it = 0; it < NWB; ++it) {
            const int j = ptid + it * PT;
            const int row = j >> 1, half = j & 1;
            const int tap = row / COS, co = row - tap * COS;
            w_off[it] = j < WPIECES ? (unsigned)(((tap * g.Cout + co_base + co) * K16 + half * 8) * 2) : SENT;
            w_dst[it] = INB + row * 32 + ((half ^ ((row >> 3) & 1)) << 4);
        }
        struct Stage16 {
            u32x4 rq[NPK];
            u32x4 rw[NWB];
        };
        Stage16 sa, sb, sc;
        const unsigned blk_bytes = (unsigned)HW * 32u;
        const _Float16 *x16 = reinterpret_cast<const _Float16 *>(x);
        const int cbg = g.Cin >> 4;
        int pf_tile = blockIdx.x, pf_chunk = 0;
        unsigned pf_off[NPK];
        const _Float16 *pf_src = x16;
        unsigned pf_bytes = 0u;
        auto pf_setup = [&]() {
            const bool live = pf_tile < tiles_total;
            int tb, ty0, tx0;
            tile_coords(live ? pf_tile : 0, tb, ty0, tx0);
#pragma unroll
            for (int k = 0; k < NPK; ++k) {
                const int yy = ty0 - g.pad + p_row[k], xx = tx0 - g.pad + p_col[k];
                const bool ok = live && ptid + k * PT < NPIECE && yy >= 0 && yy < g.H && xx >= 0 && xx < g.W;
                pf_off[k] = ok ? (unsigned)((yy * 2 + p_half[k]) * g.W + xx) * 16u : SENT;
            }
            pf_src = x16 + ((int64_t)tb * g.groups + grp) * cbg * HW * 16;
            pf_bytes = live ? (unsigned)cbg * blk_bytes : 0u;
        };
        auto prefetch = [&](Stage16 &s) {
            const uint64_t pa = reinterpret_cast<uint64_t>(pf_src);
            const uint64_t pu = ((uint64_t)(unsigned)__builtin_amdgcn_readfirstlane((unsigned)(pa >> 32)) << 32) |
                                (uint64_t)(unsigned)__builtin_amdgcn_readfirstlane((unsigned)pa);
            const __amdgpu_buffer_rsrc_t r = __builtin_amdgcn_make_buffer_rsrc(
                reinterpret_cast<_Float16 *>(pu), 0, (unsigned)__builtin_amdgcn_readfirstlane(pf_bytes), 0x00020000);
            const unsigned cb = (unsigned)__builtin_amdgcn_readfirstlane(pf_chunk) * blk_bytes;
#pragma unroll
            for (int k = 0; k < NPK; ++k) s.rq[k] = __builtin_amdgcn_raw_buffer_load_b128(r, pf_off[k] + cb, 0, 0);
            const unsigned wb = (unsigned)__builtin_amdgcn_readfirstlane(pf_chunk) * (unsigned)(CKB * 2);
#pragma unroll
            for (int it = 0; it < NWB; ++it) s.rw[it] = __builtin_amdgcn_raw_buffer_load_b128(rwt, w_off[it] + wb, 0, 0);
            if (++pf_chunk == nchunks) {
                pf_chunk = 0;
                pf_tile += G;
                pf_setup();
            }
        };
        auto commit = [&](int buf, Stage16 &s) {
            char *base = smd + buf * BUFB;
            wait_vmcnt<2 * (NPK + NWB)>();
#pragma unroll
            for (int k = 0; k < NPK; ++k)
                if (ptid + k * PT < NPIECE) *reinterpret_cast<u32x4 *>(base + p_dst[k]) = s.rq[k];
#pragma unroll
            for (int it = 0; it < NWB; ++it)
                if (ptid + it * PT < WPIECES) *reinterpret_cast<u32x4 *>(base + w_dst[it]) = s.rw[it];
// ... 1014 lines not shown
```

ebfi-be_amd/csrc/fuse.hip:

```cpp
#include "common.hpp"
#include "c16.hpp"

using namespace ebfi;

namespace {

typedef float f4 __attribute__((ext_vector_type(4)));

__global__ __launch_bounds__(256) void src_fwd_kernel(const float *__restrict__ a0, const float *__restrict__ s0,
                                                      const float *__restrict__ a1, const float *__restrict__ s1,
                                                      const float *__restrict__ x, float *__restrict__ out, int C, int64_t HW4,
                                                      int64_t total4, int64_t a_bs4) {
    const int64_t i = (int64_t)blockIdx.x * 256 + threadIdx.x;
    if (i >= total4) return;
    const int64_t bc = i / HW4, r = i - bc * HW4;
    const int64_t b = bc / C, c = bc - b * C;
    const f4 zero = {0.f, 0.f, 0.f, 0.f};
    const f4 xv = x ? reinterpret_cast<const f4 *>(x)[i] : zero;
    const int64_t ia = b * a_bs4 + c * HW4 + r;
    const f4 v0 = reinterpret_cast<const f4 *>(a0)[ia], v1 = reinterpret_cast<const f4 *>(a1)[ia];
    const float k0 = s0[bc], k1 = s1 ? s1[bc] : 1.f;
    f4 *o = reinterpret_cast<f4 *>(out);
    o[(b * 2 * C + c) * HW4 + r] = v0 * k0 + xv;
    o[(b * 2 * C + C + c) * HW4 + r] = v1 * k1 + xv;
// ... 60 lines not shown
    float acc = 0.f;
    for (int r = 0; r < R; ++r) {
        const int j = idx[i * R + r];
        if (j >= 0) acc += src[j];
    }
    out[i] = acc;
}

__global__ __launch_bounds__(256) void prodmean_fwd_kernel(const float *__restrict__ a, const float *__restrict__ b,
                                                           float *__restrict__ out, int64_t HW4) {
    __shared__ float red[4];
    const f4 *pa = reinterpret_cast<const f4 *>(a) + (int64_t)blockIdx.x * HW4;
    const f4 *pb = reinterpret_cast<const f4 *>(b) + (int64_t)blockIdx.x * HW4;
    float d = 0.f;
    for (int64_t i = threadIdx.x; i < HW4; i += 256) {
        const f4 u = pa[i], v = pb[i];
        d += (u.x * v.x + u.y * v.y) + (u.z * v.z + u.w * v.w);
    }
#pragma unroll
    for (int s = 32; s >= 1; s >>= 1) d += __shfl_xor(d, s, 64);
    if ((threadIdx.x & 63) == 0) red[threadIdx.x >> 6] = d;
    __syncthreads();
    if (threadIdx.x == 0) out[blockIdx.x] = ((red[0] + red[1]) + (red[2] + red[3])) / (float)(HW4 * 4);
}

__global__ __launch_bounds__(256) void prodmean_bwd_kernel(const float *__restrict__ a, const float *__restrict__ b,
                                                           const float *__restrict__ g, float *__restrict__ ga,
                                                           float *__restrict__ gb, int64_t HW4, int64_t total4) {
    const int64_t i = (int64_t)blockIdx.x * 256 + threadIdx.x;
    if (i >= total4) return;
    const float k = g[i / HW4] / (float)(HW4 * 4);
    const f4 u = reinterpret_cast<const f4 *>(a)[i], v = reinterpret_cast<const f4 *>(b)[i];
    reinterpret_cast<f4 *>(ga)[i] = v * k;
    reinterpret_cast<f4 *>(gb)[i] = u * k;
}

typedef unsigned u4 __attribute__((ext_vector_type(4)));

__device__ __forceinline__ void c16_store_quad(_Float16 *__restrict__ dst, int64_t piece0, const f4 (&v)[8], float s, float &amax) {
#pragma unroll
    for (int j = 0; j < 4; ++j) {
        u4 q;
#pragma unroll
        for (int e = 0; e < 8; e += 2) {
            const float a = v[e][j], b = v[e + 1][j];
            amax = amax_acc(amax, a, b);
            q[e >> 1] = pack_f16(a * s, b * s);
        }
        *reinterpret_cast<u4 *>(dst + (piece0 + j) * 8) = q;
    }
}
__device__ __forceinline__ int64_t c16_piece(int64_t b, int64_t CB, int64_t cb, int64_t HW4, int64_t q, int W4, int half) {
    const int64_t y = q / W4, xq = q - y * W4;
    return ((b * CB + cb) * (HW4 * 4) * 2) + ((y * 2 + half) * W4 + xq) * 4;
}

__global__ __launch_bounds__(256) void to_c16_kernel(const float *__restrict__ src, const float *__restrict__ mask_y, float mask_slope,
                                                     _Float16 *__restrict__ dst, float *__restrict__ slot, int C, int64_t HW4,
                                                     int W4, int64_t total) {
    saturate_fp16_conversions();
    const int64_t i = (int64_t)blockIdx.x * 256 + threadIdx.x;
    float amax = 0.f;
    if (i < total) {
        const int64_t q = i % HW4, bg = i / HW4;
        const int64_t G8 = C / 8, b = bg / G8, cg = bg - b * G8;
        const f4 *p = reinterpret_cast<const f4 *>(src) + (b * C + cg * 8) * HW4 + q;
        f4 v[8];
#pragma unroll
        for (int e = 0; e < 8; ++e) v[e] = p[e * HW4];
        if (mask_y) {
            const f4 *m = reinterpret_cast<const f4 *>(mask_y) + (b * C + cg * 8) * HW4 + q;
#pragma unroll
            for (int e = 0; e < 8; ++e) {
                const f4 y = m[e * HW4];
                v[e].x *= y.x > 0.f ? 1.f : mask_slope; v[e].y *= y.y > 0.f ? 1.f : mask_slope;
                v[e].z *= y.z > 0.f ? 1.f : mask_slope; v[e].w *= y.w > 0.f ? 1.f : mask_slope;
            }
        }
        c16_store_quad(dst, c16_piece(b, C / 16, cg / 2, HW4, q, W4, (int)(cg & 1)), v, slot[0], amax);
    }
    ScaleSlot{slot}.record(amax);
}

__global__ __launch_bounds__(256) void to_c16_cat2_kernel(const float *__restrict__ src0, int C0, const float *__restrict__ src1, int C1,
                                                          _Float16 *__restrict__ dst, float *__restrict__ slot, int64_t HW4, int W4,
                                                          int64_t total) {
    saturate_fp16_conversions();
    const int64_t i = (int64_t)blockIdx.x * 256 + threadIdx.x;
    float amax = 0.f;
    if (i < total) {
        const int C = C0 + C1;
        const int64_t q = i % HW4, bg = i / HW4;
        const int64_t G8 = C / 8, b = bg / G8, cg = bg - b * G8;
        const int64_t c = cg * 8;
        const f4 *p = c < C0 ? reinterpret_cast<const f4 *>(src0) + (b * C0 + c) * HW4 + q
                             : reinterpret_cast<const f4 *>(src1) + (b * C1 + (c - C0)) * HW4 + q;
        f4 v[8];
#pragma unroll
        for (int e = 0; e < 8; ++e) v[e] = p[e * HW4];
        c16_store_quad(dst, c16_piece(b, C / 16, cg / 2, HW4, q, W4, (int)(cg & 1)), v, slot[0], amax);
    }
    ScaleSlot{slot}.record(amax);
}

__global__ __launch_bounds__(256) void src_fwd_c16_kernel(const float *__restrict__ a0, const float *__restrict__ s0,
                                                          const float *__restrict__ a1, const float *__restrict__ s1,
                                                          const float *__restrict__ x, float *__restrict__ out,
                                                          _Float16 *__restrict__ out16, float *__restrict__ slot, int C, int64_t HW4,
                                                          int W4, int64_t total, int64_t a_bs4) {
    saturate_fp16_conversions();
    const int64_t i = (int64_t)blockIdx.x * 256 + threadIdx.x;
    float amax = 0.f;
    if (i < total) {
        const int64_t q = i % HW4, bg = i / HW4;
        const int64_t G8 = 2 * C / 8, b = bg / G8, cg = bg - b * G8;
        const int64_t co = cg * 8;
        const bool second = co >= C;
        const int64_t c = second ? co - C : co;
        const f4 *pa = reinterpret_cast<const f4 *>(second ? a1 : a0) + b * a_bs4 + c * HW4 + q;
        const f4 *px = reinterpret_cast<const f4 *>(x) + (b * C + c) * HW4 + q;
        const float *ps = (second ? s1 : s0) + b * C + c;
        f4 v[8];
#pragma unroll
        for (int e = 0; e < 8; ++e) v[e] = pa[e * HW4] * ps[e] + px[e * HW4];
        if (out) {
            f4 *o = reinterpret_cast<f4 *>(out) + (b * 2 * C + co) * HW4 + q;
#pragma unroll
            for (int e = 0; e < 8; ++e) o[e * HW4] = v[e];
        }
        c16_store_quad(out16, c16_piece(b, 2 * C / 16, cg / 2, HW4, q, W4, (int)(cg & 1)), v, slot[0], amax);
    }
    ScaleSlot{slot}.record(amax);
}

template <bool A16>
__global__ __launch_bounds__(256) void src_bwd_c16_kernel(const float *__restrict__ gout, const float *__restrict__ a0,
                                                          const float *__restrict__ s0, const float *__restrict__ a1,
                                                          const float *__restrict__ s1, _Float16 *__restrict__ ga16,
                                                          float *__restrict__ slot, float *__restrict__ gx, float *__restrict__ gs0p,
                                                          float *__restrict__ gs1p, int B, int C, int64_t HW4, int W4, int64_t a_bs4,
                                                          int nslice, float mask_slope, const float *__restrict__ a_slot = nullptr) {
    saturate_fp16_conversions();
    __shared__ float red[4][16];
    const int G8 = C / 8;
    const int slice = blockIdx.x % nslice, bg = blockIdx.x / nslice;
    const int b = bg / G8, cg = bg - b * G8, c = cg * 8;
    const int64_t q0 = HW4 * slice / nslice, q1 = HW4 * (slice + 1) / nslice;
    float k0[8], k1[8], d0[8], d1[8];
#pragma unroll
    for (int e = 0; e < 8; ++e) k0[e] = s0[b * C + c + e], k1[e] = s1[b * C + c + e], d0[e] = 0.f, d1[e] = 0.f;
    const float sc = slot[0];
    float amax = 0.f;
    auto dm = [&](const f4 &v) {
        f4 m;
        m.x = v.x > 0.f ? 1.f : mask_slope; m.y = v.y > 0.f ? 1.f : mask_slope;
        m.z = v.z > 0.f ? 1.f : mask_slope; m.w = v.w > 0.f ? 1.f : mask_slope;
        return m;
    };
    const f4 *g0 = reinterpret_cast<const f4 *>(gout) + ((int64_t)b * 2 * C + c) * HW4;
    const f4 *g1 = reinterpret_cast<const f4 *>(gout) + ((int64_t)b * 2 * C + C + c) * HW4;
    const f4 *p0 = reinterpret_cast<const f4 *>(a0) + (int64_t)b * a_bs4 + (int64_t)c * HW4;
    const f4 *p1 = reinterpret_cast<const f4 *>(a1) + (int64_t)b * a_bs4 + (int64_t)c * HW4;
    [[maybe_unused]] const _Float16 *img = reinterpret_cast<const _Float16 *>(a0);
    [[maybe_unused]] const float ainv = A16 ? 1.f / a_slot[0] : 1.f;
    auto quad_from_image = [&](int64_t piece0, f4 (&v)[8]) {
        u4 pc[4];
// ... 127 lines not shown
            if (lane == 0) gv[p] = acc;
        }
    }
}
}

extern "C" int ebfi_scale_residual_cat_forward_ex(const float *a0, const float *s0, const float *a1, const float *s1,
                                                  const float *x, float *out, int B, int C, int64_t HW, int64_t a_batch_stride,
                                                  void *stream);
extern "C" int ebfi_scale_residual_cat_forward(const float *a0, const float *s0, const float *a1, const float *s1,
                                               const float *x, float *out, int B, int C, int64_t HW, void *stream) {
    return ebfi_scale_residual_cat_forward_ex(a0, s0, a1, s1, x, out, B, C, HW, (int64_t)C * HW, stream);
}

extern "C" int ebfi_scale_residual_cat_forward_ex(const float *a0, const float *s0, const float *a1, const float *s1,
                                                  const float *x, float *out, int B, int C, int64_t HW, int64_t a_batch_stride,
                                                  void *stream) {
    if (!a0 || !s0 || !a1 || !out) return fail(EBFI_ERR_ARG, "scale_residual_cat_forward: null argument");
    if (a_batch_stride % 4 != 0 || a_batch_stride < (int64_t)C * HW) return fail(EBFI_ERR_ARG, "scale_residual_cat_forward: batch stride");
    if (int rc = check_planes("scale_residual_cat_forward", B, C, HW)) return rc;
    if (B == 0) return EBFI_OK;
    hipStream_t st = static_cast<hipStream_t>(stream);
    const int64_t total4 = (int64_t)B * C * HW / 4;
    {
        ProfScope ps("scale_residual_cat_fwd", st, 0.0, 20.0 * B * C * (double)HW);
        hipLaunchKernelGGL(src_fwd_kernel, dim3((unsigned)ceil_div(total4, 256)), dim3(256), 0, st, a0, s0, a1, s1, x, out, C, HW / 4,
                           total4, a_batch_stride / 4);
    }
    return check_launch("scale_residual_cat_fwd");
}

extern "C" int ebfi_scale_residual_cat_backward_ex(const float *grad_out, const float *a0, const float *s0, const float *a1,
                                                   const float *s1, float *grad_a0, float *grad_a1, float *grad_x,
                                                   float *grad_s0, float *grad_s1, int B, int C, int64_t HW,
                                                   int64_t a_batch_stride, int64_t grad_a_batch_stride, int mask_leaky,
                                                   float mask_slope, void *stream);
extern "C" int ebfi_scale_residual_cat_backward(const float *grad_out, const float *a0, const float *s0, const float *a1,
                                                const float *s1, float *grad_a0, float *grad_a1, float *grad_x,
                                                float *grad_s0, float *grad_s1, int B, int C, int64_t HW, void *stream) {
    return ebfi_scale_residual_cat_backward_ex(grad_out, a0, s0, a1, s1, grad_a0, grad_a1, grad_x, grad_s0, grad_s1, B, C, HW,
                                               (int64_t)C * HW, (int64_t)C * HW, 0, 0.f, stream);
}

extern "C" int ebfi_scale_residual_cat_backward_ex(const float *grad_out, const float *a0, const float *s0, const float *a1,
                                                   const float *s1, float *grad_a0, float *grad_a1, float *grad_x,
                                                   float *grad_s0, float *grad_s1, int B, int C, int64_t HW,
                                                   int64_t a_batch_stride, int64_t grad_a_batch_stride, int mask_leaky,
                                                   float mask_slope, void *stream) {
    if (a_batch_stride % 4 != 0 || grad_a_batch_stride % 4 != 0 || a_batch_stride < (int64_t)C * HW ||
        grad_a_batch_stride < (int64_t)C * HW || (mask_leaky && !a1))
        return fail(EBFI_ERR_ARG, "scale_residual_cat_backward: batch stride / mask");
    if (!grad_out || !a0 || !s0 || !grad_a0 || !grad_a1 || !grad_s0 || (s1 && (!a1 || !grad_s1)))
        return fail(EBFI_ERR_ARG, "scale_residual_cat_backward: null argument");
    if (int rc = check_planes("scale_residual_cat_backward", B, C, HW)) return rc;
    if (B == 0) return EBFI_OK;
    hipStream_t st = static_cast<hipStream_t>(stream);
    {
        ProfScope ps("scale_residual_cat_bwd", st, 0.0, 28.0 * B * C * (double)HW);
        hipLaunchKernelGGL(src_bwd_kernel, dim3((unsigned)(B * C)), dim3(256), 0, st, grad_out, a0, s0, a1, s1, grad_a0, grad_a1,
                           grad_x, grad_s0, grad_s1, C, HW / 4, a_batch_stride / 4, grad_a_batch_stride / 4, mask_leaky, mask_slope);
    }
    return check_launch("scale_residual_cat_bwd");
}

extern "C" int ebfi_to_c16(const float *src, const float *mask_y, float mask_slope, void *dst16, void *slot, int B, int C, int H, int W,
                           void *stream) {
    const int64_t HW = (int64_t)H * W;
    if (!src || !dst16 || !slot) return fail(EBFI_ERR_ARG, "to_c16: null argument");
    if (W % 4 != 0) return fail(EBFI_ERR_UNSUPPORTED, "to_c16: W %% 4 != 0 (W = %d)", W);
    if (C % 16 != 0) return fail(EBFI_ERR_UNSUPPORTED, "to_c16: %d channels (multiples of 16)", C);
    if (int rc = check_planes("to_c16", B, C, HW)) return rc;
    if (!aligned16(src) || !aligned16(dst16) || (mask_y && !aligned16(mask_y))) return fail(EBFI_ERR_ARG, "to_c16: 16-byte aligned tensors");
    if (B == 0) return EBFI_OK;
    hipStream_t st = static_cast<hipStream_t>(stream);
    const int64_t total = (int64_t)B * (C / 8) * (HW / 4);
    {
        ProfScope ps("to_c16", st, 0.0, (mask_y ? 10.0 : 6.0) * B * C * (double)HW);
        hipLaunchKernelGGL(to_c16_kernel, dim3((unsigned)ceil_div(total, 256)), dim3(256), 0, st, src, mask_y, mask_slope,
                           static_cast<_Float16 *>(dst16), static_cast<float *>(slot), C, HW / 4, W / 4, total);
    }
    return check_launch("to_c16");
}

extern "C" int ebfi_to_c16_cat2(const float *src0, int C0, const float *src1, int C1, void *dst16, void *slot, int B, int H, int W,
                                void *stream) {
    const int64_t HW = (int64_t)H * W;
    if (!src0 || !src1 || !dst16 || !slot) return fail(EBFI_ERR_ARG, "to_c16_cat2: null argument");
    if (W % 4 != 0) return fail(EBFI_ERR_UNSUPPORTED, "to_c16_cat2: W %% 4 != 0 (W = %d)", W);
    if (C0 < 8 || C1 < 8 || C0 % 8 != 0 || C1 % 8 != 0 || (C0 + C1) % 16 != 0)
        return fail(EBFI_ERR_UNSUPPORTED, "to_c16_cat2: %d + %d channels (multiples of 8, a multiple of 16 together)", C0, C1);
    if (int rc = check_planes("to_c16_cat2", B, C0 + C1, HW)) return rc;
    if (!aligned16(src0) || !aligned16(src1) || !aligned16(dst16)) return fail(EBFI_ERR_ARG, "to_c16_cat2: 16-byte aligned tensors");
    if (B == 0) return EBFI_OK;
    hipStream_t st = static_cast<hipStream_t>(stream);
    const int64_t total = (int64_t)B * ((C0 + C1) / 8) * (HW / 4);
    {
        ProfScope ps("to_c16/cat2", st, 0.0, 6.0 * B * (C0 + C1) * (double)HW);
        hipLaunchKernelGGL(to_c16_cat2_kernel, dim3((unsigned)ceil_div(total, 256)), dim3(256), 0, st, src0, C0, src1, C1,
                           static_cast<_Float16 *>(dst16), static_cast<float *>(slot), HW / 4, W / 4, total);
    }
    return check_launch("to_c16/cat2");
}

extern "C" int ebfi_scale_residual_cat_forward_c16(const float *a0, const float *s0, const float *a1, const float *s1, const float *x,
                                                   float *out, void *out16, void *slot, int B, int C, int H, int W,
                                                   int64_t a_batch_stride, void *stream) {
    const int64_t HW = (int64_t)H * W;
    if (!a0 || !s0 || !a1 || !s1 || !x || !out16 || !slot) return fail(EBFI_ERR_ARG, "scale_residual_cat_forward_c16: null argument");
    if (W % 4 != 0) return fail(EBFI_ERR_UNSUPPORTED, "scale_residual_cat_forward_c16: W %% 4 != 0 (W = %d)", W);
    if (a_batch_stride % 4 != 0 || a_batch_stride < (int64_t)C * HW) return fail(EBFI_ERR_ARG, "scale_residual_cat_forward_c16: batch stride");
    if (C % 8 != 0) return fail(EBFI_ERR_UNSUPPORTED, "scale_residual_cat_forward_c16: %d channels (multiples of 8)", C);
    if (int rc = check_planes("scale_residual_cat_forward_c16", B, C, HW)) return rc;
    if (B == 0) return EBFI_OK;
    hipStream_t st = static_cast<hipStream_t>(stream);
    const int64_t total = (int64_t)B * (2 * C / 8) * (HW / 4);
    {
        ProfScope ps("scale_residual_cat_fwd", st, 0.0, (out ? 24.0 : 16.0) * B * C * (double)HW);
        hipLaunchKernelGGL(src_fwd_c16_kernel, dim3((unsigned)ceil_div(total, 256)), dim3(256), 0, st, a0, s0, a1, s1, x, out,
                           static_cast<_Float16 *>(out16), static_cast<float *>(slot), C, HW / 4, W / 4, total, a_batch_stride / 4);
    }
    return check_launch("scale_residual_cat_fwd");
}

extern "C" int ebfi_scale_residual_cat_backward_slices(void) { return 8; }

extern "C" int ebfi_scale_residual_cat_backward_c16(const float *grad_out, const float *a0, const float *s0, const float *a1,
                                                    const float *s1, void *grad_a16, void *slot, float *grad_x, float *grad_s0_part,
                                                    float *grad_s1_part, int B, int C, int H, int W, int64_t a_batch_stride,
                                                    float mask_slope, void *stream) {
    const int64_t HW = (int64_t)H * W;
    if (W % 4 != 0) return fail(EBFI_ERR_UNSUPPORTED, "scale_residual_cat_backward_c16: W %% 4 != 0 (W = %d)", W);
    if (!grad_out || !a0 || !s0 || !a1 || !s1 || !grad_a16 || !slot || !grad_x || !grad_s0_part || !grad_s1_part)
        return fail(EBFI_ERR_ARG, "scale_residual_cat_backward_c16: null argument");
    if (a_batch_stride % 4 != 0 || a_batch_stride < (int64_t)C * HW) return fail(EBFI_ERR_ARG, "scale_residual_cat_backward_c16: batch stride");
    if (C % 16 != 0) return fail(EBFI_ERR_UNSUPPORTED, "scale_residual_cat_backward_c16: %d channels (multiples of 16)", C);
    if (int rc = check_planes("scale_residual_cat_backward_c16", B, C, HW)) return rc;
    if (B == 0) return EBFI_OK;
    hipStream_t st = static_cast<hipStream_t>(stream);
    const int nslice = ebfi_scale_residual_cat_backward_slices();
    {
        ProfScope ps("scale_residual_cat_bwd", st, 0.0, 24.0 * B * C * (double)HW);
        hipLaunchKernelGGL(src_bwd_c16_kernel<false>, dim3((unsigned)(B * (C / 8) * nslice)), dim3(256), 0, st, grad_out, a0, s0, a1, s1,
                           static_cast<_Float16 *>(grad_a16), static_cast<float *>(slot), grad_x, grad_s0_part, grad_s1_part, B, C,
                           HW / 4, W / 4, a_batch_stride / 4, nslice, mask_slope, nullptr);
    }
    return check_launch("scale_residual_cat_bwd");
}

extern "C" int ebfi_scale_residual_cat_backward_c16a(const float *grad_out, const void *a16, const void *a_slot, const float *s0,
                                                     const float *s1, void *grad_a16, void *slot, float *grad_x, float *grad_s0_part,
                                                     float *grad_s1_part, int B, int C, int H, int W, float mask_slope, void *stream) {
    const int64_t HW = (int64_t)H * W;
    if (W % 4 != 0) return fail(EBFI_ERR_UNSUPPORTED, "scale_residual_cat_backward_c16a: W %% 4 != 0 (W = %d)", W);
    if (!grad_out || !a16 || !a_slot || !s0 || !s1 || !grad_a16 || !slot || !grad_x || !grad_s0_part || !grad_s1_part)
        return fail(EBFI_ERR_ARG, "scale_residual_cat_backward_c16a: null argument");
    if (C % 16 != 0) return fail(EBFI_ERR_UNSUPPORTED, "scale_residual_cat_backward_c16a: %d channels (multiples of 16)", C);
    if (!aligned16(a16) || !aligned16(grad_a16)) return fail(EBFI_ERR_ARG, "scale_residual_cat_backward_c16a: 16-byte aligned images");
    if (int rc = check_planes("scale_residual_cat_backward_c16a", B, C, HW)) return rc;
    if (B == 0) return EBFI_OK;
    hipStream_t st = static_cast<hipStream_t>(stream);
    const int nslice = ebfi_scale_residual_cat_backward_slices();
    {
        ProfScope ps("scale_residual_cat_bwd", st, 0.0, 20.0 * B * C * (double)HW);
        hipLaunchKernelGGL(src_bwd_c16_kernel<true>, dim3((unsigned)(B * (C / 8) * nslice)), dim3(256), 0, st, grad_out,
                           static_cast<const float *>(a16), s0, static_cast<const float *>(a16), s1, static_cast<_Float16 *>(grad_a16),
                           static_cast<float *>(slot), grad_x, grad_s0_part, grad_s1_part, B, C, HW / 4, W / 4, (int64_t)0, nslice,
// ... 84 lines not shown
```

ebfi-be_amd/ebfi_amd/_native.py:

```python
import ctypes
import os
import re
import subprocess
import threading

PKG_ROOT = os.path.dirname(os.path.dirname(os.path.abspath(__file__)))
REPO_ROOT = os.path.dirname(PKG_ROOT)
_DEV = os.environ.get("EBFI_DEV") == "1"


def dev_env(name, default=None):
    return os.environ.get(name, default) if _DEV else default


LIB_PATH = dev_env("EBFI_LIB_PATH") or os.path.join(PKG_ROOT, "lib", "libebfi_hip.so")
HEADER = os.path.join(REPO_ROOT, "include", "ebfi_hip.h")
BUILD_SCRIPT = os.path.join(PKG_ROOT, "csrc", "build.sh")

EBFI_F32, EBFI_F32_BF16MMA, EBFI_F32_BF16X3MMA = 0, 2, 3
EBFI_ERR_UNSUPPORTED = -3
ABI_VERSION = 14


class EbfiNativeError(RuntimeError):
    pass


_lock = threading.Lock()
_lib = None

_c = ctypes
_vp, _i, _i64, _sz = _c.c_void_p, _c.c_int, _c.c_int64, _c.c_size_t
_p64 = _c.POINTER(_c.c_int64)

SIGNATURES = {
    "ebfi_abi_version": (_i, []),
    "ebfi_last_error": (_c.c_char_p, []),
    "ebfi_fac_forward": (_i, [_vp, _p64, _p64, _vp, _p64, _p64, _i, _vp, _p64, _p64, _i, _vp]),
    "ebfi_fac_backward": (_i, [_vp, _p64, _p64, _vp, _p64, _p64, _i, _vp, _p64, _vp, _p64, _vp, _p64, _i, _vp]),
    "ebfi_fac_backward_ex": (_i, [_vp, _p64, _p64, _vp, _p64, _p64, _i, _vp, _p64, _vp, _p64, _vp, _p64, _c.c_float, _i, _vp]),
    "ebfi_dcn_forward": (_i, [_vp] * 6 + [_i] * 14 + [_i, _vp]),
    "ebfi_dcn_backward_workspace": (_sz, [_i] * 14 + [_i]),
    "ebfi_dcn_backward": (_i, [_vp] * 11 + [_i] * 14 + [_vp, _sz, _i, _vp]),
    "ebfi_conv2d_forward": (_i, [_vp] * 4 + [_i] * 8 + [_i, _c.c_float, _i, _vp]),
    "ebfi_conv2d_backward_data": (_i, [_vp] * 4 + [_i] * 8 + [_i, _c.c_float, _i, _vp]),
    "ebfi_conv2d_backward_weight_workspace": (_sz, [_i] * 8 + [_i]),
    "ebfi_conv2d_backward_weight": (_i, [_vp] * 5 + [_i] * 8 + [_i, _c.c_float, _vp, _sz, _i, _vp]),
    "ebfi_conv2d_backward_weight_ex": (_i, [_vp] * 6 + [_i] * 8 + [_i, _c.c_float, _vp, _sz, _i, _vp]),
    "ebfi_conv2d_bf16_workspace": (_sz, [_i, _i, _i]),
    "ebfi_conv2d_forward_bf16mma": (_i, [_vp] * 4 + [_i] * 8 + [_i, _c.c_float, _vp, _sz, _vp]),
    "ebfi_conv2d_backward_data_bf16mma": (_i, [_vp] * 4 + [_i] * 8 + [_i, _c.c_float, _vp, _sz, _vp]),
    "ebfi_conv2d_forward_bf16x3": (_i, [_vp] * 4 + [_i] * 8 + [_i, _c.c_float, _vp, _sz, _vp]),
    "ebfi_conv2d_backward_data_bf16x3": (_i, [_vp] * 4 + [_i] * 8 + [_i, _c.c_float, _vp, _sz, _vp]),
    "ebfi_conv2d_packed_bytes": (_sz, [_i, _i, _i, _i]),
    "ebfi_conv2d_pack_bf16x3": (_i, [_vp, _i, _i, _i, _i, _vp, _sz, _vp]),
    "ebfi_pack_table_bf16": (_i, [_vp, _vp, _i64, _vp, _vp]),
    "ebfi_f16_scales_finish": (_i, [_vp, _i, _vp, _vp]),
    "ebfi_pack_table_f16": (_i, [_vp, _vp, _i64, _vp, _vp, _vp, _vp]),
    "ebfi_conv2d_packed_f16": (_i, [_vp, _vp, _sz, _vp, _vp] + [_i] * 8 + [_i, _c.c_float, _vp, _vp, _i, _c.c_float, _vp, _vp, _vp]),
    "ebfi_conv2d_backward_weight_f16g": (_i, [_vp] * 6 + [_i] * 8 + [_i, _c.c_float, _vp, _vp, _vp, _sz, _vp]),
    "ebfi_conv2d_backward_weight_f16g_ex": (_i, [_vp] * 6 + [_i] * 9 + [_i, _c.c_float, _vp, _vp, _vp, _sz, _vp]),
    "ebfi_to_c16": (_i, [_vp, _vp, _c.c_float, _vp, _vp, _i, _i, _i, _i, _vp]),
    "ebfi_to_c16_cat2": (_i, [_vp, _i, _vp, _i, _vp, _vp, _i, _i, _i, _vp]),
    "ebfi_conv2d_packed_x3_c16": (_i, [_vp, _vp, _sz, _vp, _vp] + [_i] * 8 + [_i, _c.c_float, _vp, _vp, _i, _c.c_float, _vp, _vp, _i, _vp]),
    "ebfi_conv2d_packed_f16_c16": (_i, [_vp, _i, _vp, _sz, _vp, _vp] + [_i] * 8 + [_i, _c.c_float, _vp, _vp, _i, _c.c_float,
                                        _vp, _vp, _vp, _vp, _i, _i, _vp]),
    "ebfi_conv2d_backward_weight_f16c": (_i, [_vp, _vp, _i, _vp, _vp] + [_i] * 6 + [_vp, _vp, _vp, _sz, _vp]),
    "ebfi_conv2d_backward_weight_f16c_batch_workspace": (_sz, [_i, _vp, _vp]),
    "ebfi_conv2d_backward_weight_f16c_batch": (_i, [_i] + [_vp] * 9 + [_i, _i, _i, _vp, _sz, _vp]),
    "ebfi_fac_forward_p16": (_i, [_vp, _i, _vp, _vp, _vp, _i, _i, _i, _i, _i, _vp]),
    "ebfi_fac_backward_p16": (_i, [_vp, _i, _vp, _vp, _vp, _vp, _vp, _vp, _c.c_float, _i, _i, _i, _i, _i, _vp]),
    "ebfi_scale_residual_cat_forward_c16": (_i, [_vp] * 8 + [_i, _i, _i, _i, _i64, _vp]),
    "ebfi_scale_residual_cat_backward_slices": (_i, []),
    "ebfi_scale_residual_cat_backward_c16": (_i, [_vp] * 10 + [_i, _i, _i, _i, _i64, _c.c_float, _vp]),
    "ebfi_scale_residual_cat_backward_c16a": (_i, [_vp] * 10 + [_i, _i, _i, _i, _c.c_float, _vp]),
    "ebfi_conv2d_packed_x3_rc": (_i, [_vp, _vp, _sz, _vp, _vp] + [_i] * 6 + [_c.c_float, _vp, _vp, _i, _vp, _vp, _vp, _vp, _vp]),
    "ebfi_conv2d_thin_forward": (_i, [_vp, _vp, _vp, _vp] + [_i] * 8 + [_i, _c.c_float, _vp]),
    "ebfi_kernelconv_fac_fused_x3": (_i, [_vp, _vp, _sz, _vp, _vp, _vp] + [_i] * 6 + [_c.c_float, _vp]),
    "ebfi_kernelconv_fac_fused_f16": (_i, [_vp, _i, _vp, _sz, _vp, _vp, _vp] + [_i] * 6 + [_c.c_float, _vp, _vp, _vp]),
    "ebfi_conv2d_packed_x3": (_i, [_vp, _vp, _sz, _vp, _vp] + [_i] * 8 + [_i, _c.c_float, _vp, _vp, _i, _c.c_float, _vp]),
    "ebfi_conv2d_backward_weight_x3g": (_i, [_vp] * 4 + [_i] * 8 + [_vp, _sz, _vp]),
    "ebfi_scale_residual_cat_forward_ex": (_i, [_vp] * 6 + [_i, _i, _i64, _i64, _vp]),
    "ebfi_scale_residual_cat_backward_ex": (_i, [_vp] * 10 + [_i, _i, _i64, _i64, _i64, _i, _c.c_float, _vp]),
    "ebfi_scalar_conv_forward": (_i, [_vp, _vp, _vp, _vp, _i, _i, _i, _i, _c.c_float, _vp]),
    "ebfi_scalar_conv_backward": (_i, [_vp, _vp, _vp, _vp, _vp, _vp, _vp, _i, _i, _i, _i, _c.c_float, _vp]),
    "ebfi_events_workspace": (_sz, [_i]),
    "ebfi_events_to_stack": (_i, [_vp, _vp, _vp, _vp, _i64, _i, _i, _i, _vp, _vp, _sz, _vp]),
    "ebfi_frame2lap": (_i, [_vp, _vp, _i, _i, _i, _vp]),
    "ebfi_frame2dcp": (_i, [_vp, _vp, _vp, _i, _i, _i, _i, _vp]),
    "ebfi_scale_residual_cat_forward": (_i, [_vp] * 6 + [_i, _i, _i64, _vp]),
    "ebfi_scale_residual_cat_backward": (_i, [_vp] * 10 + [_i, _i, _i64, _vp]),
    "ebfi_prodmean_forward": (_i, [_vp, _vp, _vp, _i64, _i64, _vp]),
    "ebfi_prodmean_backward": (_i, [_vp] * 5 + [_i64, _i64, _vp]),
    "ebfi_gather_sum": (_i, [_vp, _vp, _vp, _i64, _i, _vp]),
    "ebfi_se_gate_workspace": (_c.c_size_t, [_i, _i, _i64]),
    "ebfi_se_gate_forward": (_i, [_vp] * 8 + [_i, _i, _i64, _i, _c.c_float, _vp]),
    "ebfi_se_gate_backward": (_i, [_vp] * 11 + [_i, _i, _i64, _i, _c.c_float, _vp]),
    "ebfi_conv2d_packed_x3_shuffled": (_i, [_vp, _vp, _c.c_size_t, _vp, _vp] + [_i] * 6 + [_c.c_float, _i, _vp]),
    "ebfi_conv2d_packed_f16_shuffled": (_i, [_vp, _i, _vp, _c.c_size_t, _vp, _vp] + [_i] * 6 + [_c.c_float, _vp, _i, _c.c_float, _vp, _vp, _i, _vp]),
    "ebfi_se_gate_forward_ps": (_i, [_vp] * 7 + [_i, _i, _i, _i, _i, _c.c_float, _vp]),
    "ebfi_se_gate_backward_ps": (_i, [_vp] * 10 + [_i, _i, _i, _i, _i, _c.c_float, _vp]),
    "ebfi_groupnorm_workspace": (_sz, [_i, _i]),
    "ebfi_groupnorm_forward": (_i, [_vp] * 6 + [_i, _i, _i64, _i, _c.c_float, _vp, _sz, _vp]),
    "ebfi_groupnorm_backward": (_i, [_vp] * 8 + [_i, _i, _i64, _i, _vp, _sz, _vp]),
    "ebfi_census_partials": (_i64, [_i, _i, _i]),
    "ebfi_census_forward": (_i, [_vp, _vp, _vp, _i, _i, _i, _i, _vp]),
    "ebfi_census_backward": (_i, [_vp, _vp, _vp, _vp, _i, _i, _i, _i, _vp]),
    "ebfi_gauss5_forward": (_i, [_vp, _vp, _i64, _i, _i, _c.c_float, _vp]),
    "ebfi_gauss5_backward": (_i, [_vp, _vp, _i64, _i, _i, _c.c_float, _vp]),
    "ebfi_ed_head_workspace": (_sz, [_i, _i, _i64]),
    "ebfi_ed_head_forward": (_i, [_vp] * 7 + [_i, _i, _i64, _i, _c.c_float, _vp, _sz, _vp]),
    "ebfi_ed_head_backward": (_i, [_vp] * 11 + [_i, _i, _i64, _i, _vp, _sz, _vp]),
    "ebfi_conv2d_backward_data_s2_bf16x3": (_i, [_vp, _vp, _vp, _i, _i, _i, _i, _i, _i, _i, _vp]),
    "ebfi_adam_step": (_i, [_vp, _vp, _vp, _vp, _vp, _i64] + [_c.c_double] * 4 + [_vp]),
    "ebfi_adam_step_guarded": (_i, [_vp, _vp, _vp, _vp, _vp, _i64] + [_c.c_double] * 4 + [_vp, _vp, _vp]),
    "ebfi_pad2d_backward": (_i, [_vp, _vp, _i64, _i, _i, _i, _i, _vp]),
    "ebfi_grad_gather": (_i, [_vp, _vp, _i, _vp, _i64, _i, _vp, _vp]),
    "ebfi_laploss_workspace_floats": (_i64, [_i64, _i, _i, _i]),
    "ebfi_laploss_partials": (_i64, [_i64, _i, _i, _i]),
    "ebfi_laploss_forward": (_i, [_vp, _vp, _vp, _c.c_float, _c.c_float, _vp, _vp, _i64, _i, _i, _i, _vp]),
    "ebfi_laploss_backward": (_i, [_vp, _vp, _vp, _i64, _i, _i, _i, _vp]),
    "ebfi_image_metrics_workspace": (_i64, [_i64, _i, _i, _i]),
    "ebfi_image_metrics": (_i, [_vp, _p64, _vp, _p64, _i64, _i, _i, _i, _c.c_float, _vp, _i64, _vp, _vp, _vp, _vp]),
    "ebfi_lpips_params_bytes": (_i64, []),
    "ebfi_lpips_pack_params": (_i, [_vp, _vp, _vp, _vp, _i64, _vp]),
    "ebfi_lpips_workspace": (_i64, [_i64, _i, _i, _i]),
    "ebfi_lpips_alex": (_i, [_vp, _p64, _vp, _p64, _i64, _i, _i, _i, _i, _vp, _vp, _i64, _vp, _vp, _vp]),
    "ebfi_charbonnier_workspace": (_i64, [_i64, _i, _i, _i]),
    "ebfi_charbonnier_forward": (_i, [_vp, _p64, _vp, _p64, _i64, _i, _i, _i, _c.c_float, _vp, _i64, _vp, _vp]),
    "ebfi_charbonnier_backward": (_i, [_vp, _p64, _vp, _p64, _i64, _i, _i, _i, _c.c_float, _vp, _vp, _vp]),
    "ebfi_duty_head_workspace": (_i64, [_i64, _i, _i]),
    "ebfi_duty_head_forward": (_i, [_vp, _p64, _vp, _i64, _i, _i, _c.c_float, _vp, _i64, _vp, _vp, _vp]),
    "ebfi_duty_head_backward": (_i, [_vp, _vp, _vp, _i64, _i, _i, _c.c_float, _vp, _vp]),
    "ebfi_prof_enable": (None, [_i]),
    "ebfi_prof_set_capacity": (_i, [_i]),
    "ebfi_prof_reset": (None, []),
    "ebfi_prof_collect": (_i, [_c.POINTER(_i)]),
    "ebfi_prof_num_kernels": (_i, []),
    "ebfi_prof_get": (_i, [_i, _c.POINTER(_c.c_char_p), _c.POINTER(_i64), _c.POINTER(_c.c_double)]),
    "ebfi_prof_get_work": (_i, [_i, _c.POINTER(_c.c_double), _c.POINTER(_c.c_double)]),
}


def declared_symbols():
    text = open(HEADER).read()
    text = re.sub(r"/\*.*?\*/", "", text, flags=re.S)
    return sorted(set(re.findall(r"\b(ebfi_[a-z0-9_]+)\s*\(", text)))


def build(verbose=False):
    out = None if verbose else subprocess.DEVNULL
    subprocess.check_call(["bash", BUILD_SCRIPT], stdout=out)
    return LIB_PATH


def _counted(fn, name, n):
    def call(*a):
        if len(a) != n:
            raise TypeError("%s takes %d arguments (include/ebfi_hip.h), %d given" % (name, n, len(a)))
# ... 99 lines not shown
```

ebfi-be_amd/ebfi_amd/model.py:

```python
from math import ceil, floor

import torch
import torch.nn as nn
import torch.nn.functional as F

from . import conv, fold3d, fused, norm
from .blur import Frame2DCP, Frame2Lap
from .fac import KernelConv2D


class BaseModel(nn.Module):

    def __str__(self):
        trainable = sum(p.numel() for p in self.parameters() if p.requires_grad)
        total = sum(p.numel() for p in self.parameters())
        return super().__str__() + "\nTrainable parameters: {} \nAll parameters: {}".format(trainable, total)


class ConvLayer(nn.Module):

    def __init__(self, in_channels, out_channels, kernel_size, stride=1, padding=0, activation="ReLU", norm=None,
                 BN_momentum=0.1):
        super().__init__()
        self.conv2d = nn.Conv2d(in_channels, out_channels, kernel_size, stride, padding, bias=(norm != "BN"))
# ... 89 lines not shown
                p.requires_grad = False
            self.eval()

    def ex_map(self, Event, BlurryLevel):
        ev = self.EventFeatExtract(Event)
        bl = self.BLFeatExtract(BlurryLevel)
        cat = fused.ed_head(ev, bl, self.GroupNorm)
        if cat is None:
            atten = torch.sigmoid(fused.product_mean(norm.group_norm(ev, self.GroupNorm), norm.group_norm(bl, self.GroupNorm)))
            cat = fused.scale_cat(ev, atten, bl)
        return self.Conv1(cat)

    def forward(self, Event, BlurryLevel):
        return torch.sigmoid(self.AVGPool(self.ex_map(Event, BlurryLevel)).view(-1, 1))


class ResidualControl(BaseModel):

    def __init__(self, BLinch=2, Tinch=1, Basech=16, step=4, norm=None, activation="LeakyReLU"):
        super().__init__()
        self.step = step

        def bank(make):
            return nn.ModuleList([nn.Sequential(*make()) for _ in range(step)])

        c3 = lambda cin: _conv(cin, Basech, 3, 1, 1, norm, activation)
        self.Conv1 = bank(lambda: [_conv(BLinch, Basech, 1, 1, 0, norm, activation)])
        self.Conv2 = bank(lambda: [_conv(Tinch, Basech, 1, 1, 0, norm, activation)])
        self.Conv3 = bank(lambda: [c3(Basech), c3(Basech)])
        self.Conv4 = bank(lambda: [c3(Basech), c3(Basech)])
        self.Conv5 = bank(lambda: [c3(2 * Basech)])
        initialize_weights([self.Conv1, self.Conv2, self.Conv3, self.Conv4, self.Conv5], 0.1)

    def _ebfi_bank_register(self, bank):
        from . import rc_fused
        rc_fused.register(bank, self)

    def forward(self, data, Ex, T):
        from . import rc_fused
        if rc_fused.usable(self, data):
            out = rc_fused.residual_control(self, data, Ex, T)
            if out is not None:
                return out
        ex, t = Ex[:, :, None, None], T[:, :, None, None]
        x = data
        for i in range(self.step):
            x = self.Conv5[i](fused.scale_residual_cat(self.Conv3[i](x), self.Conv1[i](ex), self.Conv4[i](x), self.Conv2[i](t), x))
        return x


class Modification(BaseModel):

    def __init__(self, FrameBasech=64, EventBasech=32, TB=16, KernelSize=5, norm=None, activation="LeakyReLU"):
        super().__init__()
        self.Conv1 = _conv(EventBasech, FrameBasech, 1, 1, 0, norm, activation)
        self.Conv2 = _conv(FrameBasech, FrameBasech, 3, 1, 1, norm, activation)
        self.KernelConv = _conv(2 * FrameBasech, FrameBasech * KernelSize ** 2, 3, 1, 1, norm, activation)
        self.KPN = KernelConv2D(kernel_size=KernelSize)
        self.Conv3 = _conv(FrameBasech, FrameBasech, 3, 1, 1, norm, activation)
        initialize_weights([self.Conv1, self.Conv2, self.Conv3, self.KernelConv], 0.1)
        self.KernelConv.conv2d._ebfi_fwd16 = "filters"

    def _ebfi_bank_register(self, bank):
        from . import fac
        kc, k = self.KernelConv, self.KPN.kernel_size
        c = kc.conv2d
        if bank.inference and k == 5 and kc.norm is None and isinstance(kc.activation, nn.LeakyReLU) and c.bias is not None and \
                c.kernel_size == (3, 3) and c.stride == (1, 1) and c.padding == (1, 1) and c.out_channels % (k * k) == 0:
            bank.register(c.weight, c.bias, "facrows", fac.fac_rows_fold_weight, fac.fac_rows_fold_bias, need_tr=False,
                          fwd16=bank.book is not None)

    def _fused_filters_apply(self, ev, frame):
        from . import fac, weightbank
        if torch.is_grad_enabled() and (ev.requires_grad or frame.requires_grad or any(p.requires_grad for p in self.KernelConv.parameters())):
            return None
        if conv.get_compute_dtype() != "bf16x3" or not frame.is_cuda or frame.dtype != torch.float32 or ev.dtype != torch.float32 or \
                frame.shape[-1] % 4 != 0 or frame.shape[0] != ev.shape[0] or frame.shape[2:] != ev.shape[2:]:
            return None
        site = weightbank.lookup(self.KernelConv.conv2d.weight, "facrows")
        if site is None:
            return None
        return fac.kernelconv_fac_fused((ev, frame), ev, site, self.KPN.kernel_size, float(self.KernelConv.activation.negative_slope))

    def forward(self, FrameTensor, EventTensor):
        ev = self.Conv1(EventTensor)
        from . import f16scale, fac as facmod, weightbank
        book = f16scale.active_book()
        c = self.KernelConv.conv2d
        site = weightbank.lookup(c.weight, "id") if (book is not None and conv.get_compute_dtype() == "bf16x3") else None
        if torch.is_grad_enabled() and site is not None and FrameTensor.shape[0] == ev.shape[0] and \
                FrameTensor.shape[2:] == ev.shape[2:]:
            fuse = self.KernelConv.native(FrameTensor)
            if fuse is not None and fuse[0] == conv.ACT_LEAKY and \
                    facmod.kernelconv_fac_train_usable(site, book, FrameTensor, ev, self.KPN.kernel_size):
                ev1 = self.Conv3(facmod.KernelConvFacTrain.apply(FrameTensor, ev, site, fuse[1], self.KPN.kernel_size, c.weight, c.bias))
                return FrameTensor * ev1 + self.Conv2(ev1)
        fused = self._fused_filters_apply(ev, FrameTensor)
        if fused is not None:
            ev1 = self.Conv3(fused)
            return FrameTensor * ev1 + self.Conv2(ev1)
        cat = torch.cat([ev, FrameTensor], dim=1)
        fuse = self.KernelConv.native(cat)
        if fuse is not None and fuse[0] == conv.ACT_LEAKY and ev.is_cuda:
            filters = self.KernelConv(cat, grad_is_preact=True)
            if site is not None and torch.is_grad_enabled():
                book.operand((site.key, "f"), filters)
            ev1 = self.Conv3(self.KPN(ev, filters, kernel_leaky_slope=fuse[1]))
        else:
            ev1 = self.Conv3(self.KPN(ev, self.KernelConv(cat)))
        return FrameTensor * ev1 + self.Conv2(ev1)


class identity(nn.Module):
    def __init__(self, *args):
        super().__init__()

    def forward(self, x):
        return x


class SEGating(nn.Module):

    def __init__(self, inplanes, reduction=16):
        super().__init__()
        self.pool = nn.AdaptiveAvgPool3d(1)
        self.attn_layer = nn.Sequential(nn.Conv3d(inplanes, inplanes, kernel_size=1, stride=1, bias=True), nn.Sigmoid())

    def forward(self, x, res=None, post_act=None):
        if fold3d.usable(x):
            return fold3d.se_gate(x, self.attn_layer[0], res, 0 if post_act is None else 1, post_act or 0.0)
        y = x * self.attn_layer(self.pool(x))
        if res is not None:
            y = y + res
        return y if post_act is None else F.leaky_relu(y, post_act)


def _norm3d(bn, ch):
    return nn.BatchNorm3d(ch) if bn else identity(ch)


class BasicBlock(nn.Module):
    expansion = 1

    def __init__(self, inplanes, planes, stride=1, downsample=None, bn=False):
        super().__init__()
        c3 = lambda cin, s: nn.Conv3d(cin, planes, kernel_size=(3, 3, 3), stride=s, padding=1, bias=False)
        self.conv1 = nn.Sequential(c3(inplanes, stride), _norm3d(bn, planes), nn.ReLU(inplace=True))
        self.conv2 = nn.Sequential(c3(planes, 1), _norm3d(bn, planes))
        self.fg = SEGating(planes)
        self.relu = nn.ReLU(inplace=True)
        self.downsample = downsample

    def forward(self, x):
        if fold3d.usable(x) and isinstance(self.conv1[1], identity):
            out = fold3d.conv3d_d2(x, self.conv1[0], conv.ACT_LEAKY, 0.0)
            res = x if self.downsample is None else fold3d.conv3d_d2(x, self.downsample[0])
            return self.fg(fold3d.conv3d_d2(out, self.conv2[0]), res, 0.0)
        out = self.fg(self.conv2(self.conv1(x)))
        res = x if self.downsample is None else self.downsample(x)
        return self.relu(out + res)


class VideoResNet(nn.Module):

    def __init__(self, channels, bn=False, layers=(2, 2, 2, 2)):
        super().__init__()
        self.stem = nn.Sequential(
            nn.Conv3d(3, channels[0], kernel_size=(3, 7, 7), stride=(1, 2, 2), padding=(1, 3, 3), bias=False),
            _norm3d(bn, channels[0]), nn.ReLU(inplace=True))
        inplanes = channels[0]
        spatial = [1, 2, 2, 1]
        for li in range(4):
            planes = channels[li]
            blocks = []
            for bi in range(layers[li]):
                ds, s = None, 1
                if bi == 0 and (spatial[li] != 1 or inplanes != planes):
                    s = (1, spatial[li], spatial[li])
                    ds = nn.Sequential(nn.Conv3d(inplanes, planes, kernel_size=1, stride=s, bias=False),
                                       _norm3d(bn, planes))
                blocks.append(BasicBlock(inplanes, planes, s, ds, bn))
                inplanes = planes
            setattr(self, "layer%d" % (li + 1), nn.Sequential(*blocks))
        for m in self.modules():
            if isinstance(m, nn.Conv3d):
                nn.init.kaiming_normal_(m.weight, mode="fan_out", nonlinearity="relu")
                if m.bias is not None:
                    nn.init.constant_(m.bias, 0)
            elif isinstance(m, nn.BatchNorm3d):
                nn.init.constant_(m.weight, 1)
# ... 222 lines not shown
```

include/ebfi_hip.h:

```cpp
#ifndef EBFI_HIP_H
#define EBFI_HIP_H

#include <stddef.h>
#include <stdint.h>

#ifdef __cplusplus
extern "C" {
#endif

#define EBFI_ABI_VERSION 14

typedef enum {
    EBFI_OK = 0,
    EBFI_ERR_ARG = -1,
    EBFI_ERR_LAUNCH = -2,
    EBFI_ERR_UNSUPPORTED = -3,
    EBFI_ERR_WORKSPACE = -4
} ebfi_status;

typedef enum { EBFI_F32 = 0, EBFI_F32_BF16MMA = 2, EBFI_F32_BF16X3MMA = 3 } ebfi_dtype;

int ebfi_abi_version(void);
const char *ebfi_last_error(void);

// ... 37 lines not shown
                      void *workspace, size_t workspace_bytes, int dtype, void *stream);

int ebfi_conv2d_forward(const void *input, const void *weight, const void *bias, void *output,
                        int B, int Cin, int H, int W, int Cout, int ksize, int stride, int pad,
                        int act, float slope, int dtype, void *stream);

int ebfi_conv2d_backward_data(const void *grad_output, const void *saved_output, const void *weight,
                              void *grad_input, int B, int Cin, int H, int W, int Cout, int ksize,
                              int stride, int pad, int act, float slope, int dtype, void *stream);

size_t ebfi_conv2d_backward_weight_workspace(int B, int Cin, int H, int W, int Cout, int ksize,
                                             int stride, int pad, int dtype);

int ebfi_conv2d_backward_weight(const void *input, const void *grad_output, const void *saved_output,
                                void *grad_weight, void *grad_bias,
                                int B, int Cin, int H, int W, int Cout, int ksize, int stride, int pad,
                                int act, float slope, void *workspace, size_t workspace_bytes,
                                int dtype, void *stream);

int ebfi_conv2d_backward_weight_ex(const void *input, const void *grad_output, const void *saved_output,
                                   void *grad_weight, void *grad_bias, void *grad_preact_out,
                                   int B, int Cin, int H, int W, int Cout, int ksize, int stride, int pad,
                                   int act, float slope, void *workspace, size_t workspace_bytes,
                                   int dtype, void *stream);

size_t ebfi_conv2d_bf16_workspace(int Cin, int Cout, int ksize);
int ebfi_conv2d_forward_bf16mma(const void *input, const void *weight, const void *bias, void *output,
                                int B, int Cin, int H, int W, int Cout, int ksize, int stride, int pad,
                                int act, float slope, void *workspace, size_t workspace_bytes, void *stream);
int ebfi_conv2d_backward_data_bf16mma(const void *grad_output, const void *saved_output, const void *weight,
                                      void *grad_input, int B, int Cin, int H, int W, int Cout, int ksize,
                                      int stride, int pad, int act, float slope,
                                      void *workspace, size_t workspace_bytes, void *stream);

int ebfi_conv2d_forward_bf16x3(const void *input, const void *weight, const void *bias, void *output,
                               int B, int Cin, int H, int W, int Cout, int ksize, int stride, int pad,
                               int act, float slope, void *workspace, size_t workspace_bytes, void *stream);
int ebfi_conv2d_backward_data_bf16x3(const void *grad_output, const void *saved_output, const void *weight,
                                     void *grad_input, int B, int Cin, int H, int W, int Cout, int ksize,
                                     int stride, int pad, int act, float slope,
                                     void *workspace, size_t workspace_bytes, void *stream);

int ebfi_conv2d_backward_data_s2_bf16x3(const void *grad_preact, const void *weight, void *grad_input, int B, int Cin,
                                        int H, int W, int Cout, int ksize, int pad, void *stream);

size_t ebfi_conv2d_packed_bytes(int Cin, int Cout, int ksize, int transposed);
int ebfi_conv2d_pack_bf16x3(const void *weight, int Cin, int Cout, int ksize, int transposed, void *packed,
                            size_t packed_bytes, void *stream);
int ebfi_pack_table_bf16(const float *src, const int32_t *table, int64_t n, void *out, void *stream);

int ebfi_conv2d_thin_forward(const void *input, const void *weight, const void *bias, void *output, int B, int Cin, int H, int W,
                             int Cout, int ksize, int stride, int pad, int act, float slope, void *stream);

int ebfi_conv2d_packed_x3(const void *input, const void *packed, size_t packed_bytes, const void *bias, void *output,
                          int B, int Cin_per_group, int H, int W, int Cout, int ksize, int pad, int groups, int act,
                          float slope, const void *addend, const void *mask_y, int mask_act, float mask_slope, void *stream);
int ebfi_kernelconv_fac_fused_x3(const void *input, const void *packed, size_t packed_bytes, const void *bias32,
                                 const void *feat, void *output, int B, int Cin, int H, int W, int C, int fac_ksize,
                                 float slope, void *stream);

int ebfi_kernelconv_fac_fused_f16(const void *input, int input_is_c16, const void *packed16, size_t packed_bytes,
                                  const void *bias32, const void *feat, void *output, int B, int Cin, int H, int W, int C,
                                  int fac_ksize, float slope, void *in_slot, const void *w_slot, void *stream);
int ebfi_f16_scales_finish(void *slots, int n, void *flag, void *stream);
int ebfi_pack_table_f16(const float *src, const int32_t *table, int64_t n, void *out, const int32_t *block_slot,
                        void *slots, void *stream);
int ebfi_conv2d_packed_f16(const void *input, const void *packed16, size_t packed_bytes, const void *bias, void *output,
                           int B, int Cin_per_group, int H, int W, int Cout, int ksize, int pad, int groups, int act,
                           float slope, const void *addend, const void *mask_y, int mask_act, float mask_slope,
                           void *in_slot, const void *w_slot, void *stream);
int ebfi_conv2d_backward_weight_f16g(const void *input, const void *grad_output, const void *saved_output,
                                     void *grad_weight, void *grad_bias, void *grad_preact_out, int B,
                                     int Cin_per_group, int H, int W, int Cout, int ksize, int pad, int groups, int act,
                                     float slope, void *x_slot, void *g_slot, void *workspace,
                                     size_t workspace_bytes, void *stream);
int ebfi_conv2d_backward_weight_f16g_ex(const void *input, const void *grad_output, const void *saved_output,
                                        void *grad_weight, void *grad_bias, void *grad_preact_out, int grad_preact_is_c16, int B,
                                        int Cin_per_group, int H, int W, int Cout, int ksize, int pad, int groups, int act,
                                        float slope, void *x_slot, void *g_slot, void *workspace,
                                        size_t workspace_bytes, void *stream);
int ebfi_to_c16(const float *src, const float *mask_y, float mask_slope, void *dst16, void *slot, int B, int C, int H, int W,
                void *stream);
int ebfi_to_c16_cat2(const float *src0, int C0, const float *src1, int C1, void *dst16, void *slot, int B, int H, int W, void *stream);
int ebfi_conv2d_packed_x3_c16(const void *input, const void *packed, size_t packed_bytes, const void *bias, void *output,
                              int B, int Cin_per_group, int H, int W, int Cout, int ksize, int pad, int groups, int act,
                              float slope, const void *addend, const void *mask_y, int mask_act, float mask_slope,
                              void *out16, void *slot16, int out16_planar, void *stream);
int ebfi_conv2d_packed_f16_c16(const void *input, int input_is_c16, const void *packed16, size_t packed_bytes,
                               const void *bias, void *output, int B, int Cin_per_group, int H, int W, int Cout, int ksize,
                               int pad, int groups, int act, float slope, const void *addend, const void *mask_y,
                               int mask_act, float mask_slope, void *in_slot, const void *w_slot, void *out16,
                               void *slot16, int out16_planar, int mask_is_c16, void *stream);
int ebfi_conv2d_packed_x3_shuffled(const void *input, const void *packed, size_t packed_bytes, const void *bias, void *output,
                                   int B, int Cin, int H, int W, int Cout, int act, float slope, int out_layout, void *stream);
int ebfi_conv2d_packed_f16_shuffled(const void *input, int input_is_c16, const void *packed16, size_t packed_bytes,
                                    const void *bias, void *output, int B, int Cin, int H, int W, int Cout, int act, float slope,
                                    const void *mask_y, int mask_act, float mask_slope, void *in_slot, const void *w_slot,
                                    int out_layout, void *stream);
int ebfi_conv2d_backward_weight_f16c(const void *input16, const void *grad16, int grad_is_planar, void *grad_weight,
                                     void *grad_bias, int B, int Cin_per_group, int H, int W, int Cout, int groups,
                                     const void *x_slot, const void *g_slot, void *workspace, size_t workspace_bytes,
                                     void *stream);
size_t ebfi_conv2d_backward_weight_f16c_batch_workspace(int n, const int *Cin_per_group, const int *Cout);
int ebfi_conv2d_backward_weight_f16c_batch(int n, const void *const *input16, const void *const *grad16, void *const *grad_weight,
                                           void *const *grad_bias, const int *Cin_per_group, const int *Cout, const int *groups,
                                           void *const *x_slot, void *const *g_slot, int B, int H, int W, void *workspace,
                                           size_t workspace_bytes, void *stream);
int ebfi_fac_forward_p16(const float *input, int input_is_unpadded, const void *filters16, const void *f_slot, float *output, int B,
                         int C, int Ho, int Wo, int K, void *stream);
int ebfi_fac_backward_p16(const float *input, int input_is_unpadded, const void *filters16, const void *f_slot,
                          const float *grad_output, float *grad_input, void *grad_kernel16, void *g_slot, float kernel_leaky_slope,
                          int B, int C, int Ho, int Wo, int K, void *stream);
int ebfi_scale_residual_cat_forward_c16(const float *a0, const float *s0, const float *a1, const float *s1, const float *x,
                                        float *out, void *out16, void *slot, int B, int C, int H, int W,
                                        int64_t a_batch_stride, void *stream);
int ebfi_scale_residual_cat_backward_slices(void);
int ebfi_scale_residual_cat_backward_c16(const float *grad_out, const float *a0, const float *s0, const float *a1,
                                         const float *s1, void *grad_a16, void *slot, float *grad_x, float *grad_s0_part,
                                         float *grad_s1_part, int B, int C, int H, int W, int64_t a_batch_stride,
                                         float mask_slope, void *stream);
int ebfi_scale_residual_cat_backward_c16a(const float *grad_out, const void *a16, const void *a_slot, const float *s0, const float *s1,
                                          void *grad_a16, void *slot, float *grad_x, float *grad_s0_part, float *grad_s1_part, int B,
                                          int C, int H, int W, float mask_slope, void *stream);
int ebfi_conv2d_packed_x3_rc(const void *input, const void *packed, size_t packed_bytes, const void *bias, void *output, int B,
                             int Cin_per_group, int H, int W, int Cout, int groups, float slope, const void *post_scale,
                             const void *post_res, int res_channels, void *pre16, void *pre_slot, void *out16, void *slot16,
                             void *stream);
int ebfi_conv2d_backward_weight_x3g(const void *input, const void *grad_output, void *grad_weight, void *grad_bias,
                                    int B, int Cin_per_group, int H, int W, int Cout, int ksize, int pad, int groups,
                                    void *workspace, size_t workspace_bytes, void *stream);

size_t ebfi_events_workspace(int bins);
int ebfi_events_to_stack(const double *xs, const double *ys, const double *ts, const float *ps,
                         int64_t n, int bins, int H, int W, float *out,
                         void *workspace, size_t workspace_bytes, void *stream);

int ebfi_frame2lap(const float *frame, float *out, int B, int H, int W, void *stream);
int ebfi_frame2dcp(const float *frame, float *out, float *scratch , int B, int H, int W,
                   int window, void *stream);

int ebfi_scalar_conv_forward(const float *v, const void *const *weights, const void *const *biases, float *out, int S, int B,
                             int K, int C, float slope, void *stream);
int ebfi_scalar_conv_backward(const float *v, const void *const *weights, const float *out, const float *grad_out,
                              float *grad_weight, float *grad_bias, float *grad_v, int S, int B, int K, int C, float slope,
                              void *stream);

int ebfi_scale_residual_cat_forward(const float *a0, const float *s0, const float *a1, const float *s1, const float *x,
                                    float *out, int B, int C, int64_t HW, void *stream);
int ebfi_scale_residual_cat_backward(const float *grad_out, const float *a0, const float *s0, const float *a1,
                                     const float *s1, float *grad_a0, float *grad_a1, float *grad_x,
                                     float *grad_s0, float *grad_s1, int B, int C, int64_t HW, void *stream);

int ebfi_scale_residual_cat_forward_ex(const float *a0, const float *s0, const float *a1, const float *s1, const float *x,
                                       float *out, int B, int C, int64_t HW, int64_t a_batch_stride, void *stream);
int ebfi_scale_residual_cat_backward_ex(const float *grad_out, const float *a0, const float *s0, const float *a1,
                                        const float *s1, float *grad_a0, float *grad_a1, float *grad_x, float *grad_s0,
                                        float *grad_s1, int B, int C, int64_t HW, int64_t a_batch_stride,
                                        int64_t grad_a_batch_stride, int mask_leaky, float mask_slope, void *stream);

int ebfi_prodmean_forward(const float *a, const float *b, float *out, int64_t planes, int64_t HW, void *stream);
int ebfi_prodmean_backward(const float *a, const float *b, const float *grad_out, float *grad_a, float *grad_b,
                           int64_t planes, int64_t HW, void *stream);

int ebfi_gather_sum(const float *src, const int32_t *idx, float *out, int64_t n_out, int R, void *stream);

size_t ebfi_se_gate_workspace(int B, int C, int64_t N);
int ebfi_se_gate_forward(const float *x, const float *weight, const float *bias, const float *res, float *out, float *mean,
                         float *gate, float *workspace, int B, int C, int64_t N, int act, float slope, void *stream);
int ebfi_se_gate_backward(const float *grad_out, const float *out, const float *x, const float *weight, const float *gate,
                          const float *mean, float *grad_x, float *grad_res, float *grad_weight, float *grad_bias,
                          float *workspace, int B, int C, int64_t N, int act, float slope, void *stream);

int ebfi_se_gate_forward_ps(const float *x, const float *weight, const float *bias, float *out, float *mean, float *gate,
                            float *workspace, int B, int C, int h, int w, int act, float slope, void *stream);
int ebfi_se_gate_backward_ps(const float *grad_out, const float *out, const float *x, const float *weight, const float *gate,
                             const float *mean, float *grad_x, float *grad_weight, float *grad_bias, float *workspace, int B, int C,
                             int h, int w, int act, float slope, void *stream);

size_t ebfi_groupnorm_workspace(int B, int C);
int ebfi_groupnorm_forward(const float *x, const float *gamma, const float *beta, float *y, float *mean, float *rstd,
                           int B, int C, int64_t HW, int groups, float eps,
                           void *workspace, size_t workspace_bytes, void *stream);
int ebfi_groupnorm_backward(const float *grad_y, const float *x, const float *gamma, const float *mean,
                            const float *rstd, float *grad_x, float *grad_gamma, float *grad_beta,
                            int B, int C, int64_t HW, int groups,
                            void *workspace, size_t workspace_bytes, void *stream);

size_t ebfi_ed_head_workspace(int B, int C, int64_t HW);
int ebfi_ed_head_forward(const float *ev, const float *bl, const float *gamma, const float *beta, float *out, float *atten,
                         double *stats, int B, int C, int64_t HW, int groups, float eps,
                         void *workspace, size_t workspace_bytes, void *stream);
int ebfi_ed_head_backward(const float *grad_out, const float *ev, const float *bl, const float *gamma, const float *beta,
                          const float *atten, const double *stats, float *grad_ev, float *grad_bl, float *grad_gamma,
                          float *grad_beta, int B, int C, int64_t HW, int groups,
                          void *workspace, size_t workspace_bytes, void *stream);

int ebfi_gauss5_forward(const float *input, float *output, int64_t planes, int H, int W, float factor, void *stream);
int ebfi_gauss5_backward(const float *grad_output, float *grad_input, int64_t planes, int H, int W, float factor,
                         void *stream);

int64_t ebfi_census_partials(int B, int H, int W);
int ebfi_census_forward(const float *x, const float *y, float *partial, int B, int C, int H, int W, void *stream);
int ebfi_census_backward(const float *x, const float *y, const float *grad_loss, float *grad_x,
                         int B, int C, int H, int W, void *stream);

int64_t ebfi_laploss_workspace_floats(int64_t planes, int H, int W, int levels);
int64_t ebfi_laploss_partials(int64_t planes, int H, int W, int levels);
int ebfi_laploss_forward(const float *pred_a, const float *pred_b, const float *target, float coef_a, float coef_b,
                         float *workspace, float *partial, int64_t planes_per_term, int H, int W, int levels, void *stream);
int ebfi_laploss_backward(const float *grad_loss, float *workspace, float *grad_pred, int64_t planes, int H, int W,
// ... 52 lines not shown
```

Baseline: 546.4 frames/s.

## Fuse modification tail product-sum into Conv2 epilogue for forward and backward

Adds a product-sum epilogue (XM bit 16) to the wave-specialised conv kernels. In the forward pass, Conv2's output is combined with FrameTensor*ev1 directly in the epilogue, and an fp16 pre-activation image is written there too. In the backward pass, the dgrad conv adds g*frame into the gradient and writes g*ev1 as a second output. A new autograd function, ModificationTailFn, routes the Conv3/Conv2 tail through these kernels to remove separate elementwise multiply/add passes and extra full-resolution memory traffic. The cost is more kernel variants, extra register pressure in the epilogue, and a disabled few-tiles path for this case.

```diff
diff --git a/ebfi-be_amd/csrc/conv2d.hip b/ebfi-be_amd/csrc/conv2d.hip
--- a/ebfi-be_amd/csrc/conv2d.hip
+++ b/ebfi-be_amd/csrc/conv2d.hip
@@ -31,7 +31,17 @@
     int post_resC = 0;
     _Float16 *pre16 = nullptr;
     float *pre_slot = nullptr;
+    const float *ps_p = nullptr;
+    const float *ps_q = nullptr;
+    const float *ps_g = nullptr;
+    float *ps_out2 = nullptr;
 };
+
+__device__ __forceinline__ float add_product(float a, float p, float q) {
+#pragma clang fp contract(off)
+    const float t = p * q;
+    return a + t;
+}
 
 __device__ __forceinline__ float act_apply(float v, int act, float slope) {
     if (act == ACT_LEAKY) return v > 0.f ? v : v * slope;
@@ -80,7 +90,8 @@
                                                float *amax16 = nullptr, float *amax_pre = nullptr) {
     const int HWo = g.Ho * g.Wo;
     const unsigned plane = (unsigned)HWo * 4u;
-    constexpr bool EXTRA = (XM & 7) != 0, XAM = (XM & 1) != 0, X16 = (XM & 2) != 0, XRC = (XM & 4) != 0;
+    constexpr bool EXTRA = (XM & 0x17) != 0, XAM = (XM & 1) != 0, X16 = (XM & 2) != 0, XRC = (XM & 4) != 0;
+    constexpr bool XPS = (XM & 16) != 0;
     constexpr bool XST = (XM & 8) != 0;
     if constexpr (EXTRA) {
         asm volatile("" : "+v"(lane));
@@ -89,7 +100,7 @@
     const float *anyp = bias ? bias : (out ? out : reinterpret_cast<const float *>(ex.slot16));
     const __amdgpu_buffer_rsrc_t ro = make_rsrc(has32 ? out + (int64_t)b * g.Cout * HWo : anyp, has32 ? (unsigned)g.Cout * plane : 0u);
     const __amdgpu_buffer_rsrc_t rb = make_rsrc(bias ? bias : anyp, bias ? (unsigned)g.Cout * 4u : 0u);
-    const bool has_a = XAM && ex.addend != nullptr, has_m = XAM && ex.mask_y != nullptr, has16 = X16 && ex.out16 != nullptr;
+    const bool has_a = XAM && !XPS && ex.addend != nullptr, has_m = XAM && !XPS && ex.mask_y != nullptr, has16 = X16 && ex.out16 != nullptr;
     const bool has_m16 = XAM && ex.mask16 != nullptr;
     const __amdgpu_buffer_rsrc_t ra = make_rsrc(has_a ? ex.addend + (int64_t)b * g.Cout * HWo : anyp, has_a ? (unsigned)g.Cout * plane : 0u);
     const __amdgpu_buffer_rsrc_t rm = make_rsrc(has_m ? ex.mask_y + (int64_t)b * g.Cout * HWo : anyp, has_m ? (unsigned)g.Cout * plane : 0u);
@@ -107,12 +118,18 @@
     const __amdgpu_buffer_rsrc_t rps = make_rsrc(has_rc ? ex.post_scale + (int64_t)b * g.Cout : anyp, has_rc ? (unsigned)g.Cout * 4u : 0u);
     const __amdgpu_buffer_rsrc_t rrs = make_rsrc(has_rc ? ex.post_res + (int64_t)b * ex.post_resC * HWo : anyp,
                                                  has_rc ? (unsigned)ex.post_resC * plane : 0u);
-    const bool has_p16 = has_rc && ex.pre16 != nullptr;
+    const bool has_p16 = (has_rc || XPS) && ex.pre16 != nullptr;
     const __amdgpu_buffer_rsrc_t rp16 = __builtin_amdgcn_make_buffer_rsrc(
         has_p16 ? ex.pre16 + (int64_t)b * cb16 * HWo * 16 : const_cast<_Float16 *>(reinterpret_cast<const _Float16 *>(anyp)), 0,
         has_p16 ? (unsigned)cb16 * (unsigned)HWo * 32u : 0u, 0x00020000);
     const float sp16 = has_p16 ? ex.pre_slot[0] : 1.f;
     const int res_shift = has_rc ? co_base - co_base % ex.post_resC : 0;
+    const bool ps_bwd = XPS && ex.ps_g != nullptr, has_o2 = ps_bwd && ex.ps_out2 != nullptr;
+    const int64_t ps_off = (int64_t)b * g.Cout * HWo;
+    const __amdgpu_buffer_rsrc_t rpp = make_rsrc(XPS ? ex.ps_p + ps_off : anyp, XPS ? (unsigned)g.Cout * plane : 0u);
+    const __amdgpu_buffer_rsrc_t rpq = make_rsrc(XPS && ex.ps_q ? ex.ps_q + ps_off : anyp, XPS && ex.ps_q ? (unsigned)g.Cout * plane : 0u);
+    const __amdgpu_buffer_rsrc_t rpg = make_rsrc(ps_bwd ? ex.ps_g + ps_off : anyp, ps_bwd ? (unsigned)g.Cout * plane : 0u);
+    const __amdgpu_buffer_rsrc_t ro2 = make_rsrc(has_o2 ? ex.ps_out2 + ps_off : anyp, has_o2 ? (unsigned)g.Cout * plane : 0u);
     float am = 0.f, amp = 0.f;
     const int h = lane >> 5, l31 = lane & 31;
     struct BlockIn {
@@ -120,6 +137,7 @@
         float my[8];
         unsigned m16[4];
         float res[8];
+        float pp[8], pq[8], pg[8];
     };
     auto shuffled_base = [&](int m) { return (unsigned)(((co_base + m * 32) >> 2) + h) * 4u * plane; };
     auto unshuffled_base = [&](int m, bool px_ok, int xo) {
@@ -161,6 +179,16 @@
                 for (int i = 0; i < 8; ++i) in.res[i] = buf_ld(rrs, rbase + row_off(j, i) * plane);
             }
         }
+        if constexpr (XPS) {
+#pragma unroll
+            for (int i = 0; i < 8; ++i) in.pp[i] = buf_ld(rpp, base + row_off(j, i) * plane);
+#pragma unroll
+            for (int i = 0; i < 8; ++i) in.pq[i] = buf_ld(rpq, base + row_off(j, i) * plane);
+            if (ps_bwd) {
+#pragma unroll
+                for (int i = 0; i < 8; ++i) in.pg[i] = buf_ld(rpg, base + row_off(j, i) * plane);
+            }
+        }
     };
     [[maybe_unused]] auto finish = [&](int m, int n, int j, const BlockIn &in, auto actf) {
         bool px_ok; unsigned base; int cblk, xo;
@@ -188,6 +216,16 @@
                 for (int i = 0; i < 8; ++i) u[i] += in.add[i];
             }
         }
+        if constexpr (XPS) {
+            if (ps_bwd) {
+#pragma unroll
+                for (int i = 0; i < 8; ++i) u[i] = add_product(u[i], in.pg[i], in.pp[i]);
+                if (has_o2) {
+#pragma unroll
+                    for (int i = 0; i < 8; ++i) buf_st(ro2, base + row_off(j, i) * plane, in.pg[i] * in.pq[i]);
+                }
+            }
+        }
 #pragma unroll
         for (int i = 0; i < 8; ++i) u[i] = actf(u[i]);
         if constexpr (XAM) {
@@ -215,6 +253,20 @@
                 }
 #pragma unroll
                 for (int i = 0; i < 8; ++i) u[i] = u[i] * psc[i] + in.res[i];
+            }
+        }
+        if constexpr (XPS) {
+            if (!ps_bwd) {
+                if (has_p16) {
+                    const unsigned o16 = (px_ok && cblk < cb16) ? ((unsigned)cblk * (unsigned)HWo * 2u + (unsigned)((yo * 2 + h) * g.Wo + xo)) * 16u : SENT;
+#pragma unroll
+                    for (int i = 0; i < 8; ++i) amp = amax_acc(amp, u[i]);
+                    const u32x4_c16 q = c16_gather_halves(pack_f16(u[0] * sp16, u[1] * sp16), pack_f16(u[2] * sp16, u[3] * sp16),
+                                                          pack_f16(u[4] * sp16, u[5] * sp16), pack_f16(u[6] * sp16, u[7] * sp16));
+                    __builtin_amdgcn_raw_buffer_store_b128(q, rp16, o16, 0, 0);
+                }
+#pragma unroll
+                for (int i = 0; i < 8; ++i) u[i] = add_product(u[i], in.pp[i], in.pq[i]);
             }
         }
         if (has32) {
@@ -317,7 +369,7 @@
         else emit([](float v) { return v; });
     }
     if (amax16) *amax16 = amax_acc(*amax16, am);
-    if constexpr (XRC) {
+    if constexpr (XRC || XPS) {
         if (amax_pre) *amax_pre = amax_acc(*amax_pre, amp);
     }
 }
@@ -2270,7 +2322,7 @@
 __global__ __launch_bounds__(NTWS) void conv_fwd_bf16x3_ws(const float *__restrict__ x, const __bf16 *__restrict__ wp,
                                                            const float *__restrict__ bias, float *__restrict__ out, ConvGeom g, int K16,
                                                            int act, float slope, EpiExtra epi, int tiles_total, FacEpi fac) {
-    constexpr bool EXTRA = (XM & 7) != 0;
+    constexpr bool EXTRA = (XM & 0x17) != 0;
     constexpr int KS = 3, KK = 9, MT = 2;
     constexpr int IH = TYB - 1 + KS, IW = TX - 1 + KS, PS = IH * IW, COS = 32 * MT;
     constexpr int NCW = 8, PT = 256;
@@ -2370,9 +2422,9 @@
             if constexpr (FAC) {
                 fac_epilogue_tile<MT>(out, bias, acc, g, fac, cb_, co_base, cy0 + wave, cx0, lane, slope);
             } else {
-                if constexpr ((XM & 6) != 0) saturate_fp16_conversions(true);
+                if constexpr ((XM & 0x16) != 0) saturate_fp16_conversions(true);
                 store_out_tile<MT, XM>(out, bias, acc, g, cb_, co_base, cy0 + wave, cx0, lane, act, slope, epi, 1.f, &amax16, &amax_pre);
-                if constexpr ((XM & 6) != 0) saturate_fp16_conversions(false);
+                if constexpr ((XM & 0x16) != 0) saturate_fp16_conversions(false);
             }
 #pragma unroll
             for (int m = 0; m < MT; ++m)
@@ -2383,7 +2435,7 @@
         }
         if constexpr (EXTRA) {
             if (epi.out16 != nullptr) ScaleSlot{epi.slot16}.record(amax16);
-            if constexpr ((XM & 4) != 0) {
+            if constexpr ((XM & 0x14) != 0) {
                 if (epi.pre16 != nullptr) ScaleSlot{epi.pre_slot}.record(amax_pre);
             }
         }
@@ -2529,7 +2581,7 @@
     const char *name = x3 ? (transposed ? "conv_fwd_bf16x3_db/dgrad" : "conv_fwd_bf16x3_db/fwd")
                           : (transposed ? "conv_fwd_bf16/dgrad" : "conv_fwd_bf16/fwd");
     const double flops = 2.0 * g.B * g.Ho * g.Wo * (double)g.Cout * g.Cin * KS * KS;
-    const bool few = x3 && epi.out16 == nullptr && epi.post_scale == nullptr && g.store == 0 && tiles * ceil_div(g.Cout, 64) <= 128;
+    const bool few = x3 && epi.out16 == nullptr && epi.post_scale == nullptr && epi.ps_p == nullptr && g.store == 0 && tiles * ceil_div(g.Cout, 64) <= 128;
     const int mt = (g.Cout <= 32 || few) ? 1 : 2;
     dim3 grid((unsigned)tiles, (unsigned)ceil_div(g.Cout, 32 * mt));
     if (g.store != 0 && !x3) return fail(EBFI_ERR_UNSUPPORTED, "conv2d: shuffled output layouts are written by the split-precision kernels only");
@@ -2544,10 +2596,13 @@
                         "(W %% 4 == 0, same padding, more than 32 output channels, 16-byte aligned input)");
         if (epi.post_scale != nullptr && !use_ws)
             return fail(EBFI_ERR_UNSUPPORTED, "conv2d: the ResidualControl epilogue is written by the wave-specialised 3x3 kernel only");
+        if (epi.ps_p != nullptr && (!use_ws || extra || g.store != 0))
+            return fail(EBFI_ERR_UNSUPPORTED, "conv2d: the product-sum epilogue is written by the wave-specialised 3x3 kernel only (W %% 4 == 0, "
+                        "same padding, more than 32 output channels, 16-byte aligned input), without other epilogue extras");
         if (g.store != 0 && (!use_ws || extra))
             return fail(EBFI_ERR_UNSUPPORTED, "conv2d: a shuffled output layout is written by the wave-specialised 3x3 kernel only (W %% 4 == 0, "
                         "same padding, more than 32 output channels, 16-byte aligned input), without epilogue extras");
-        if (use_ws) name = transposed ? "conv_fwd_bf16x3_ws/dgrad" : (epi.post_scale ? "conv_fwd_bf16x3_ws/fwd_rc" :
+        if (use_ws) name = transposed ? "conv_fwd_bf16x3_ws/dgrad" : epi.ps_p ? "conv_fwd_bf16x3_ws/fwd_prodsum" : (epi.post_scale ? "conv_fwd_bf16x3_ws/fwd_rc" :
                                                                       (epi.out16 ? "conv_fwd_bf16x3_ws/fwd_img" :
                                                                        (g.store ? "conv_fwd_bf16x3_ws/fwd_shuffle" : "conv_fwd_bf16x3_ws/fwd")));
         ProfScope ps(name, st, flops, conv_bytes_fwd(g, KS * KS, dact != 0));
@@ -2580,7 +2635,8 @@
                            (int)tiles, FacEpi{nullptr, 0});                                                               \
     } while (0)
                 const bool xam = epi.addend != nullptr || epi.mask_y != nullptr, x16 = epi.out16 != nullptr;
-                if (epi.post_scale != nullptr) {
+                if (epi.ps_p != nullptr) EBFI_LAUNCH_X3WS(16);
+                else if (epi.post_scale != nullptr) {
                     if (xam) return fail(EBFI_ERR_UNSUPPORTED, "conv2d: the ResidualControl epilogue comes without addend / mask");
                     if (x16) EBFI_LAUNCH_X3WS(6);
                     else EBFI_LAUNCH_X3WS(4);
@@ -3416,11 +3472,15 @@
 }
 
 namespace {
+struct ProdSumArgs {
+    const void *p, *q, *g;
+    void *out2, *pre16, *pre_slot;
+};
 int packed_f16_impl(const void *input, int input_is_c16, const void *packed16, size_t packed_bytes,
                     const void *bias, void *output, int B, int Cin_per_group, int H, int W, int Cout, int ksize,
                     int pad, int groups, int act, float slope, const void *addend, const void *mask_y,
                     int mask_act, float mask_slope, void *in_slot, const void *w_slot, void *out16,
-                    void *slot16, int out16_planar, int mask_is_c16, int out_layout, void *stream);
+                    void *slot16, int out16_planar, int mask_is_c16, int out_layout, void *stream, const ProdSumArgs *ps_args = nullptr);
 }
 
 extern "C" int ebfi_conv2d_packed_f16_c16(const void *input, int input_is_c16, const void *packed16, size_t packed_bytes,
@@ -3445,7 +3505,7 @@
                     const void *bias, void *output, int B, int Cin_per_group, int H, int W, int Cout, int ksize,
                     int pad, int groups, int act, float slope, const void *addend, const void *mask_y,
                     int mask_act, float mask_slope, void *in_slot, const void *w_slot, void *out16,
-                    void *slot16, int out16_planar, int mask_is_c16, int out_layout, void *stream) {
+                    void *slot16, int out16_planar, int mask_is_c16, int out_layout, void *stream, const ProdSumArgs *ps_args) {
     if (!input || !packed16 || (!output && !out16)) return fail(EBFI_ERR_ARG, "conv2d_packed_f16: null argument");
     if ((out16 != nullptr) != (slot16 != nullptr)) return fail(EBFI_ERR_ARG, "conv2d_packed_f16: out16 and slot16 come together");
     if (out16 && !out16_planar && (Cout % 16 != 0 || !aligned16(out16)))
@@ -3479,9 +3539,19 @@
     if ((addend || mask_y || out16) && (act == ACT_SIGMOID || mask_act == ACT_SIGMOID))
         return fail(EBFI_ERR_UNSUPPORTED, "conv2d_packed_f16: the epilogue extras take LeakyReLU / no activation only");
     const bool m16 = mask_is_c16 != 0 && mask_y != nullptr && mask_act == ACT_LEAKY;
-    const EpiExtra epi{static_cast<const float *>(addend), (mask_act == ACT_LEAKY && !m16) ? static_cast<const float *>(mask_y) : nullptr,
-                       mask_act, mask_slope, static_cast<_Float16 *>(out16), static_cast<float *>(slot16), out16_planar ? 1 : 0,
-                       m16 ? static_cast<const _Float16 *>(mask_y) : nullptr};
+    EpiExtra epi{static_cast<const float *>(addend), (mask_act == ACT_LEAKY && !m16) ? static_cast<const float *>(mask_y) : nullptr,
+                 mask_act, mask_slope, static_cast<_Float16 *>(out16), static_cast<float *>(slot16), out16_planar ? 1 : 0,
+                 m16 ? static_cast<const _Float16 *>(mask_y) : nullptr};
+    if (ps_args) {
+        if (act == ACT_SIGMOID || addend || out16_planar || out_layout != 0 || input_is_c16 == 2)
+            return fail(EBFI_ERR_UNSUPPORTED, "conv2d_packed_f16: the product-sum epilogue takes LeakyReLU / no activation, no addend, plain layouts");
+        epi.ps_p = static_cast<const float *>(ps_args->p);
+        epi.ps_q = static_cast<const float *>(ps_args->q);
+        epi.ps_g = static_cast<const float *>(ps_args->g);
+        epi.ps_out2 = static_cast<float *>(ps_args->out2);
+        epi.pre16 = static_cast<_Float16 *>(ps_args->pre16);
+        epi.pre_slot = static_cast<float *>(ps_args->pre_slot);
+    }
     const int64_t tiles = (int64_t)B * ceil_div(g.Ho, TYB) * ceil_div(g.Wo, TX);
     if (tiles > 2147483647LL) return fail(EBFI_ERR_ARG, "conv2d_packed_f16: too many tiles");
     constexpr int PSX = (TYB - 1 + 3) * (TX - 1 + 3);
@@ -3496,7 +3566,7 @@
     const double px = (double)g.B * g.Ho * g.Wo;
     const double io_bytes = px * g.groups * g.Cin * (input_is_c16 ? 2.0 : 4.0) + px * g.Cout * ((output ? 4.0 : 0.0) + (out16 ? 2.0 : 0.0)) +
                             px * g.Cout * ((addend ? 4.0 : 0.0) + (mask_y ? (m16 ? 2.0 : 4.0) : 0.0)) + 2.0 * 9 * (double)g.Cout * g.Cin;
-    ProfScope ps(g.store ? (input_is_c16 ? "conv_fwd_f16_ws/img_shuffle" : "conv_fwd_f16_ws/f32_shuffle") :
+    ProfScope ps(ps_args ? (ps_args->g ? "conv_fwd_f16_ws/prodsum_dgrad" : "conv_fwd_f16_ws/prodsum_fwd") : g.store ? (input_is_c16 ? "conv_fwd_f16_ws/img_shuffle" : "conv_fwd_f16_ws/f32_shuffle") :
                  input_is_c16 == 2 ? "conv_fwd_f16_ws/p16_f32" : out16_planar ? (input_is_c16 ? "conv_fwd_f16_ws/img_p16" : "conv_fwd_f16_ws/f32_p16") :
                  input_is_c16 ? (out16 ? (output ? "conv_fwd_f16_ws/img_both" : "conv_fwd_f16_ws/img_img") : "conv_fwd_f16_ws/img_f32")
                               : (out16 ? "conv_fwd_f16_ws/f32_img" : "conv_fwd_f16_ws/f32_f32"), st, flops, io_bytes);
@@ -3510,7 +3580,17 @@
         hipLaunchKernelGGL((conv_fwd_f16_ws<EX_, IN_>), grid, dim3(NTF16), lds, st, x, wp, bs, o, g, K16, act, slope, epi,   \
                            (int)tiles, isl, static_cast<const float *>(w_slot), FacEpi{nullptr, 0});                    \
     } while (0)
-    if (input_is_c16 == 2) {
+    if (ps_args) {
+#define EBFI_LAUNCH_F16PS(IN_)                                                                                           \
+    do {                                                                                                                 \
+        if (int rc_ = ensure_dynamic_lds(reinterpret_cast<const void *>(&conv_fwd_f16_ws<true, IN_, false, false, false, true>), 160 * 1024)) return rc_; \
+        hipLaunchKernelGGL((conv_fwd_f16_ws<true, IN_, false, false, false, true>), grid, dim3(NTF16), lds, st, x, wp, bs, o, g, K16, act, slope, epi, \
+                           (int)tiles, isl, static_cast<const float *>(w_slot), FacEpi{nullptr, 0});                    \
+    } while (0)
+        if (input_is_c16) EBFI_LAUNCH_F16PS(true);
+        else EBFI_LAUNCH_F16PS(false);
+#undef EBFI_LAUNCH_F16PS
+    } else if (input_is_c16 == 2) {
         if (extra || g.store) return fail(EBFI_ERR_UNSUPPORTED, "conv2d_packed_f16: planar fp16 input with epilogue extras / a shuffled output");
         if (int rc_ = ensure_dynamic_lds(reinterpret_cast<const void *>(&conv_fwd_f16_ws<false, false, true>), 160 * 1024)) return rc_;
         hipLaunchKernelGGL((conv_fwd_f16_ws<false, false, true>), grid, dim3(NTF16), lds, st, x, wp, bs, o, g, K16, act, slope, epi,
@@ -3532,6 +3612,52 @@
 #undef EBFI_LAUNCH_F16WS
     return check_launch("conv_fwd_f16_ws");
 }
+}
+
+namespace {
+int prodsum_check(const char *who, const void *output, const void *p, const void *q, const void *pre16, const void *pre_slot, int Cout) {
+    if (!output || !p || !q) return fail(EBFI_ERR_ARG, "%s: null argument", who);
+    if ((pre16 != nullptr) != (pre_slot != nullptr)) return fail(EBFI_ERR_ARG, "%s: pre16 and pre_slot come together", who);
+    if (Cout % 64 != 0 || (pre16 && !aligned16(pre16)))
+        return fail(EBFI_ERR_UNSUPPORTED, "%s: needs Cout %% 64 == 0 and a 16-byte aligned image (Cout = %d)", who, Cout);
+    return EBFI_OK;
+}
+}
+
+extern "C" int ebfi_conv2d_packed_x3_prodsum(const void *input, const void *packed, size_t packed_bytes, const void *bias, void *output,
+                                             int B, int Cin, int H, int W, int Cout, int act, float slope, const void *p, const void *q,
+                                             void *pre16, void *pre_slot, void *stream) {
+    if (!input || !packed) return fail(EBFI_ERR_ARG, "conv2d_packed_x3_prodsum: null argument");
+    if (int rc = prodsum_check("conv2d_packed_x3_prodsum", output, p, q, pre16, pre_slot, Cout)) return rc;
+    if (act != ACT_NONE && act != ACT_LEAKY) return fail(EBFI_ERR_UNSUPPORTED, "conv2d_packed_x3_prodsum: LeakyReLU / no activation only");
+    ConvGeom g;
+    if (int rc = make_geom(g, B, Cin, H, W, Cout, 3, 1, 1)) return rc;
+    if (((int64_t)Cin + 64) * H * W * 4 >= (1LL << 31) - (1LL << 26) || ((int64_t)Cout + 64) * H * W * 4 >= (1LL << 31) - (1LL << 26))
+        return fail(EBFI_ERR_ARG, "conv2d_packed_x3_prodsum: one sample exceeds the 2 GiB reach of 32-bit buffer offsets");
+    if (B == 0) return EBFI_OK;
+    EpiExtra epi{nullptr, nullptr, 0, 0.f};
+    epi.ps_p = static_cast<const float *>(p);
+    epi.ps_q = static_cast<const float *>(q);
+    epi.pre16 = static_cast<_Float16 *>(pre16);
+    epi.pre_slot = static_cast<float *>(pre_slot);
+    return launch_fwd_bf16<3>(static_cast<hipStream_t>(stream), static_cast<const float *>(input), nullptr, nullptr,
+                              static_cast<const float *>(bias), static_cast<float *>(output), g, 0, act, slope, 0, 0.f,
+                              const_cast<void *>(packed), packed_bytes, 1, epi);
+}
+
+extern "C" int ebfi_conv2d_packed_f16_prodsum(const void *input, int input_is_c16, const void *packed16, size_t packed_bytes,
+                                              const void *bias, void *output, void *output2, int B, int Cin, int H, int W, int Cout,
+                                              int act, float slope, const void *g, const void *p, const void *q, const void *mask_y,
+                                              int mask_is_c16, float mask_slope, void *in_slot, const void *w_slot, void *out16,
+                                              void *slot16, void *pre16, void *pre_slot, void *stream) {
+    if (!p || (!g && !q) || (output2 && (!g || !q))) return fail(EBFI_ERR_ARG, "conv2d_packed_f16_prodsum: null argument");
+    if (mask_y && !mask_is_c16) return fail(EBFI_ERR_UNSUPPORTED, "conv2d_packed_f16_prodsum: the mask comes as a c16 image");
+    if ((pre16 != nullptr) != (pre_slot != nullptr) || (pre16 && (g || !aligned16(pre16))))
+        return fail(EBFI_ERR_ARG, "conv2d_packed_f16_prodsum: pre16 comes with its slot, in the forward form");
+    if (Cout % 64 != 0 || input_is_c16 < 0 || input_is_c16 > 1) return fail(EBFI_ERR_UNSUPPORTED, "conv2d_packed_f16_prodsum: Cout %% 64 == 0, fp32 or c16 input");
+    const ProdSumArgs ps{p, q, g, output2, pre16, pre_slot};
+    return packed_f16_impl(input, input_is_c16, packed16, packed_bytes, bias, output, B, Cin, H, W, Cout, 3, 1, 1, act, slope, nullptr, mask_y,
+                           mask_y ? ACT_LEAKY : ACT_NONE, mask_slope, in_slot, w_slot, out16, slot16, 0, mask_is_c16, 0, stream, &ps);
 }
 
 extern "C" int ebfi_conv2d_backward_weight_f16g_ex(const void *input, const void *grad_output, const void *saved_output,
diff --git a/ebfi-be_amd/csrc/conv2d_f16.inc.hpp b/ebfi-be_amd/csrc/conv2d_f16.inc.hpp
--- a/ebfi-be_amd/csrc/conv2d_f16.inc.hpp
+++ b/ebfi-be_amd/csrc/conv2d_f16.inc.hpp
@@ -1,12 +1,13 @@
 
 
 constexpr int NTF16 = 512;
-template <bool EXTRA, bool IN16 = false, bool INP16 = false, bool FAC = false, bool ST = false>
+template <bool EXTRA, bool IN16 = false, bool INP16 = false, bool FAC = false, bool ST = false, bool PSUM = false>
 __global__ __launch_bounds__(NTF16) void conv_fwd_f16_ws(const float *__restrict__ x, const _Float16 *__restrict__ wp,
                                                          const float *__restrict__ bias, float *__restrict__ out, ConvGeom g, int K16,
                                                          int act, float slope, EpiExtra epi, int tiles_total, ScaleSlot in_slot,
                                                          const float *__restrict__ w_slot, FacEpi fac) {
     static_assert(!FAC || (!EXTRA && !INP16), "the FAC epilogue comes without epilogue extras (input: fp32 planes or a c16 image)");
+    static_assert(!PSUM || (EXTRA && !ST), "the product-sum epilogue is an EXTRA form with the plain output layout");
     constexpr int KS = 3, KK = 9, MT = 2, RW = 2;
     constexpr int IH = TYB - 1 + KS, IW = TX - 1 + KS, PS = IH * IW, COS = 32 * MT;
     constexpr int NCW = TYB / RW, PT = 256;
@@ -52,7 +53,7 @@
 #pragma unroll
                     for (int e = 0; e < 16; ++e) acc[r][m][n][e] = 0.f;
         const float oscale = 1.f / (sx * (w_slot ? w_slot[0] : 1.f));
-        [[maybe_unused]] float amax16 = 0.f;
+        [[maybe_unused]] float amax16 = 0.f, amax_pre = 0.f;
         const int hsel = lane >> 5, l31 = lane & 31;
         const int a_lane = INB + l31 * 32 + ((hsel ^ ((l31 >> 3) & 1)) << 4);
         const int pbase = RW * wave * IW + l31;
@@ -111,8 +112,13 @@
                 fac_epilogue_tile<MT>(out, bias, acc[1], g, fac, cb_, co_base, cy0 + RW * wave + 1, cx0, lane, slope, oscale);
             } else {
                 if constexpr (EXTRA) saturate_fp16_conversions(true);
+                if constexpr (PSUM) {
+                    store_out_tile<MT, 19>(out, bias, acc[0], g, cb_, co_base, cy0 + RW * wave, cx0, lane, act, slope, epi, oscale, &amax16, &amax_pre);
+                    store_out_tile<MT, 19>(out, bias, acc[1], g, cb_, co_base, cy0 + RW * wave + 1, cx0, lane, act, slope, epi, oscale, &amax16, &amax_pre);
+                } else {
                 store_out_tile<MT, (EXTRA ? 3 : 0) | (ST ? 8 : 0)>(out, bias, acc[0], g, cb_, co_base, cy0 + RW * wave, cx0, lane, act, slope, epi, oscale, &amax16);
                 store_out_tile<MT, (EXTRA ? 3 : 0) | (ST ? 8 : 0)>(out, bias, acc[1], g, cb_, co_base, cy0 + RW * wave + 1, cx0, lane, act, slope, epi, oscale, &amax16);
+                }
                 if constexpr (EXTRA) saturate_fp16_conversions(false);
             }
 #pragma unroll
@@ -129,6 +135,9 @@
         KB_FLUSH_SELF();
         if constexpr (EXTRA) {
             if (epi.out16 != nullptr) ScaleSlot{epi.slot16}.record(amax16);
+            if constexpr (PSUM) {
+                if (epi.pre16 != nullptr) ScaleSlot{epi.pre_slot}.record(amax_pre);
+            }
         }
         return;
     }
diff --git a/ebfi-be_amd/csrc/fuse.hip b/ebfi-be_amd/csrc/fuse.hip
--- a/ebfi-be_amd/csrc/fuse.hip
+++ b/ebfi-be_amd/csrc/fuse.hip
@@ -166,6 +166,34 @@
     ScaleSlot{slot}.record(amax);
 }
 
+__global__ __launch_bounds__(256) void to_c16_mask16_kernel(const float *__restrict__ src, const _Float16 *__restrict__ mask16, float mask_slope,
+                                                            _Float16 *__restrict__ dst, float *__restrict__ slot, int C, int64_t HW4,
+                                                            int W4, int64_t total) {
+    saturate_fp16_conversions();
+    const int64_t i = (int64_t)blockIdx.x * 256 + threadIdx.x;
+    float amax = 0.f;
+    if (i < total) {
+        const int64_t q = i % HW4, bg = i / HW4;
+        const int64_t G8 = C / 8, b = bg / G8, cg = bg - b * G8;
+        const f4 *p = reinterpret_cast<const f4 *>(src) + (b * C + cg * 8) * HW4 + q;
+        f4 v[8];
+#pragma unroll
+        for (int e = 0; e < 8; ++e) v[e] = p[e * HW4];
+        const int64_t piece0 = c16_piece(b, C / 16, cg / 2, HW4, q, W4, (int)(cg & 1));
+#pragma unroll
+        for (int j = 0; j < 4; ++j) {
+            const u4 m = *reinterpret_cast<const u4 *>(mask16 + (piece0 + j) * 8);
+#pragma unroll
+            for (int e = 0; e < 8; ++e) {
+                const unsigned hbits = (m[e >> 1] >> (16 * (e & 1))) & 0xffffu;
+                v[e][j] *= (hbits != 0u && hbits < 0x8000u) ? 1.f : mask_slope;
+            }
+        }
+        c16_store_quad(dst, piece0, v, slot[0], amax);
+    }
+    ScaleSlot{slot}.record(amax);
+}
+
 __global__ __launch_bounds__(256) void to_c16_cat2_kernel(const float *__restrict__ src0, int C0, const float *__restrict__ src1, int C1,
                                                           _Float16 *__restrict__ dst, float *__restrict__ slot, int64_t HW4, int W4,
                                                           int64_t total) {
@@ -459,6 +487,26 @@
     return check_launch("to_c16");
 }
 
+extern "C" int ebfi_to_c16_mask16(const float *src, const void *mask16, float mask_slope, void *dst16, void *slot, int B, int C, int H,
+                                  int W, void *stream) {
+    const int64_t HW = (int64_t)H * W;
+    if (!src || !mask16 || !dst16 || !slot) return fail(EBFI_ERR_ARG, "to_c16_mask16: null argument");
+    if (W % 4 != 0) return fail(EBFI_ERR_UNSUPPORTED, "to_c16_mask16: W %% 4 != 0 (W = %d)", W);
+    if (C % 16 != 0) return fail(EBFI_ERR_UNSUPPORTED, "to_c16_mask16: %d channels (multiples of 16)", C);
+    if (int rc = check_planes("to_c16_mask16", B, C, HW)) return rc;
+    if (!aligned16(src) || !aligned16(dst16) || !aligned16(mask16)) return fail(EBFI_ERR_ARG, "to_c16_mask16: 16-byte aligned tensors");
+    const int64_t total = (int64_t)B * (C / 8) * (HW / 4);
+    if (total == 0) return EBFI_OK;
+    hipStream_t st = static_cast<hipStream_t>(stream);
+    {
+        ProfScope ps("to_c16/mask16", st, 0.0, 8.0 * B * C * (double)HW);
+        hipLaunchKernelGGL(to_c16_mask16_kernel, dim3((unsigned)ceil_div(total, 256)), dim3(256), 0, st, src,
+                           static_cast<const _Float16 *>(mask16), mask_slope, static_cast<_Float16 *>(dst16), static_cast<float *>(slot), C,
+                           HW / 4, W / 4, total);
+    }
+    return check_launch("to_c16/mask16");
+}
+
 extern "C" int ebfi_to_c16_cat2(const float *src0, int C0, const float *src1, int C1, void *dst16, void *slot, int B, int H, int W,
                                 void *stream) {
     const int64_t HW = (int64_t)H * W;
diff --git a/ebfi-be_amd/ebfi_amd/_native.py b/ebfi-be_amd/ebfi_amd/_native.py
--- a/ebfi-be_amd/ebfi_amd/_native.py
+++ b/ebfi-be_amd/ebfi_amd/_native.py
@@ -61,6 +61,7 @@
     "ebfi_conv2d_backward_weight_f16g": (_i, [_vp] * 6 + [_i] * 8 + [_i, _c.c_float, _vp, _vp, _vp, _sz, _vp]),
     "ebfi_conv2d_backward_weight_f16g_ex": (_i, [_vp] * 6 + [_i] * 9 + [_i, _c.c_float, _vp, _vp, _vp, _sz, _vp]),
     "ebfi_to_c16": (_i, [_vp, _vp, _c.c_float, _vp, _vp, _i, _i, _i, _i, _vp]),
+    "ebfi_to_c16_mask16": (_i, [_vp, _vp, _c.c_float, _vp, _vp, _i, _i, _i, _i, _vp]),
     "ebfi_to_c16_cat2": (_i, [_vp, _i, _vp, _i, _vp, _vp, _i, _i, _i, _vp]),
     "ebfi_conv2d_packed_x3_c16": (_i, [_vp, _vp, _sz, _vp, _vp] + [_i] * 8 + [_i, _c.c_float, _vp, _vp, _i, _c.c_float, _vp, _vp, _i, _vp]),
     "ebfi_conv2d_packed_f16_c16": (_i, [_vp, _i, _vp, _sz, _vp, _vp] + [_i] * 8 + [_i, _c.c_float, _vp, _vp, _i, _c.c_float,
@@ -75,6 +76,9 @@
     "ebfi_scale_residual_cat_backward_c16": (_i, [_vp] * 10 + [_i, _i, _i, _i, _i64, _c.c_float, _vp]),
     "ebfi_scale_residual_cat_backward_c16a": (_i, [_vp] * 10 + [_i, _i, _i, _i, _c.c_float, _vp]),
     "ebfi_conv2d_packed_x3_rc": (_i, [_vp, _vp, _sz, _vp, _vp] + [_i] * 6 + [_c.c_float, _vp, _vp, _i, _vp, _vp, _vp, _vp, _vp]),
+    "ebfi_conv2d_packed_x3_prodsum": (_i, [_vp, _vp, _sz, _vp, _vp] + [_i] * 5 + [_i, _c.c_float, _vp, _vp, _vp, _vp, _vp]),
+    "ebfi_conv2d_packed_f16_prodsum": (_i, [_vp, _i, _vp, _sz, _vp, _vp, _vp] + [_i] * 5 + [_i, _c.c_float, _vp, _vp, _vp, _vp, _i, _c.c_float,
+                                            _vp, _vp, _vp, _vp, _vp, _vp, _vp]),
     "ebfi_conv2d_thin_forward": (_i, [_vp, _vp, _vp, _vp] + [_i] * 8 + [_i, _c.c_float, _vp]),
     "ebfi_kernelconv_fac_fused_x3": (_i, [_vp, _vp, _sz, _vp, _vp, _vp] + [_i] * 6 + [_c.c_float, _vp]),
     "ebfi_kernelconv_fac_fused_f16": (_i, [_vp, _i, _vp, _sz, _vp, _vp, _vp] + [_i] * 6 + [_c.c_float, _vp, _vp, _vp]),
diff --git a/ebfi-be_amd/ebfi_amd/mod_fused.py b/ebfi-be_amd/ebfi_amd/mod_fused.py
--- /dev/null
+++ b/ebfi-be_amd/ebfi_amd/mod_fused.py
@@ -0,0 +1,114 @@
+import torch
+from torch.autograd import Function
+
+from . import _native as N
+from . import conv, rc_fused, weightbank
+
+ROLES = (("c3", "x"), ("c3", "g"), ("c2", "x"), ("c2", "g"), ("c2", "y"))
+
+
+def _plain(m):
+    return rc_fused._plain_layer(m, 3)
+
+
+def sites_of(mod):
+    if not (_plain(mod.Conv3) and _plain(mod.Conv2)):
+        return None
+    s3, s2 = weightbank.lookup(mod.Conv3.conv2d.weight, "id"), weightbank.lookup(mod.Conv2.conv2d.weight, "id")
+    for s in (s3, s2):
+        if s is None or not s.has_bias or s.kind != "id" or s.groups != 1 or len(s.w_shapes) != 1 or s.tr16_ptr() is None:
+            return None
+    return s3, s2
+
+
+def _slot_keys(s3, s2):
+    site = {"c3": s3, "c2": s2}
+    return [(site[n].key, role) for n, role in ROLES]
+
+
+def usable(mod, frame, fac, book):
+    if book is None or conv.get_compute_dtype() != "bf16x3" or not torch.is_grad_enabled() or torch.is_autocast_enabled():
+        return None
+    if not (frame.is_cuda and frame.dtype == torch.float32 and fac.dtype == torch.float32 and frame.shape == fac.shape and fac.dim() == 4):
+        return None
+    if fac.shape[1] % 64 != 0 or fac.shape[3] % 4 != 0 or fac.shape[2] * fac.shape[3] < 2:
+        return None
+    sites = sites_of(mod)
+    if sites is None or sites[0].K != fac.shape[1] or sites[0].M != sites[1].K or sites[1].M != frame.shape[1] or sites[0].M % 64 != 0:
+        return None
+    if float(mod.Conv3.activation.negative_slope) != float(mod.Conv2.activation.negative_slope):
+        return None
+    if not all(book.index.get(k) in book.calibrated for k in _slot_keys(*sites)):
+        return None
+    return sites
+
+
+def calibrate_y(mod, book, y2):
+    if book is None or conv.get_compute_dtype() != "bf16x3" or not y2.is_cuda or torch.cuda.is_current_stream_capturing():
+        return
+    sites = sites_of(mod)
+    if sites is not None:
+        book.operand((sites[1].key, "y"), y2)
+
+
+class ModificationTailFn(Function):
+
+    @staticmethod
+    def forward(ctx, frame, fac, sites, slope, *params):
+        from . import c16, f16scale
+        book = f16scale.active_book()
+        s3, s2 = sites
+        frame, fac = frame.contiguous(), fac.contiguous()
+        B, C, H, W = (int(v) for v in fac.shape)
+        lib = N.lib()
+        sp = lambda site, role: book.ptr(book.slot((site.key, role)))
+        with torch.cuda.device_of(fac):
+            st = N.stream_ptr(fac.device)
+            fac16 = c16.to_c16(fac, sp(s3, "x"))
+            ev1, out = torch.empty_like(fac), torch.empty_like(fac)
+            ev16, y16 = c16.empty(B, C, H, W, fac.device), c16.empty(B, C, H, W, fac.device)
+            rc_fused._conv16(lib, st, fac, s3, s3.bias(), ev1, B, C, H, W, C, 1, slope, ev16, sp(s2, "x"))
+            rc = lib.ebfi_conv2d_packed_x3_prodsum(N.ptr(ev1), s2.fwd_ptr(), s2.fwd_bytes, N.ptr(s2.bias()), N.ptr(out), B, C, H, W, C,
+                                                   conv.ACT_LEAKY, slope, N.ptr(frame), N.ptr(ev1), N.ptr(y16), sp(s2, "y"), st)
+            N.check(rc, "ebfi_conv2d_packed_x3_prodsum")
+        ctx.sites, ctx.slope, ctx.dims = sites, slope, (B, C, H, W)
+        ctx.save_for_backward(frame, ev1, fac16, ev16, y16)
+        return out
+
+    @staticmethod
+    def backward(ctx, g):
+        from . import c16, f16scale
+        frame, ev1, fac16, ev16, y16 = ctx.saved_tensors
+        (s3, s2), slope, (B, C, H, W) = ctx.sites, ctx.slope, ctx.dims
+        book = f16scale.active_book()
+        if book is None:
+            raise RuntimeError("Modification ran its forward with fp16 operand images: backward() must run inside the same scale-book "
+                               "context (Engine._fwd_bwd)")
+        lib = N.lib()
+        g = g.contiguous()
+        sp = lambda site, role: book.ptr(book.slot((site.key, role)))
+        need = ctx.needs_input_grad
+        ws_cache = {}
+        with torch.cuda.device_of(g):
+            st = N.stream_ptr(g.device)
+            g2 = c16.empty(B, C, H, W, g.device)
+            rc = lib.ebfi_to_c16_mask16(N.ptr(g), N.ptr(y16), slope, N.ptr(g2), sp(s2, "g"), B, C, H, W, st)
+            N.check(rc, "ebfi_to_c16_mask16")
+            g3 = c16.empty(B, C, H, W, g.device)
+            gframe = torch.empty_like(g) if need[0] else None
+            rc = lib.ebfi_conv2d_packed_f16_prodsum(N.ptr(g2), 1, s2.tr16_ptr(), s2.tr16_bytes, N.ptr(None), N.ptr(None), N.ptr(gframe), B, C,
+                                                    H, W, C, conv.ACT_NONE, 0.0, N.ptr(g), N.ptr(frame), N.ptr(ev1), N.ptr(ev16), 1, slope,
+                                                    sp(s2, "g"), s2.w_slot_ptr(), N.ptr(g3), sp(s3, "g"), N.ptr(None), N.ptr(None), st)
+            N.check(rc, "ebfi_conv2d_packed_f16_prodsum")
+            gw2, gb2 = rc_fused._wgrad16(lib, st, ev16, g2, B, C, H, W, C, 1, ws_cache, book, s2)
+            gw3, gb3 = rc_fused._wgrad16(lib, st, fac16, g3, B, C, H, W, C, 1, ws_cache, book, s3)
+            gfac = None
+            if need[1]:
+                gfac = torch.empty_like(g)
+                rc_fused._dgrad16(lib, st, g3, s3, B, C, H, W, C, 1, slope, book, out=gfac)
+        return gframe, gfac, None, None, gw3, gb3, gw2, gb2
+
+
+def modification_tail(mod, frame, fac, sites):
+    c3, c2 = mod.Conv3.conv2d, mod.Conv2.conv2d
+    return ModificationTailFn.apply(frame, fac, sites, float(mod.Conv3.activation.negative_slope), c3.weight, c3.bias, c2.weight, c2.bias)
diff --git a/ebfi-be_amd/ebfi_amd/model.py b/ebfi-be_amd/ebfi_amd/model.py
--- a/ebfi-be_amd/ebfi_amd/model.py
+++ b/ebfi-be_amd/ebfi_amd/model.py
@@ -195,9 +195,17 @@
             return None
         return fac.kernelconv_fac_fused((ev, frame), ev, site, self.KPN.kernel_size, float(self.KernelConv.activation.negative_slope))
 
+    def _tail(self, FrameTensor, fac_out, book):
+        from . import mod_fused
+        ev1 = self.Conv3(fac_out)
+        y2 = self.Conv2(ev1)
+        if book is not None and torch.is_grad_enabled():
+            mod_fused.calibrate_y(self, book, y2.detach())
+        return FrameTensor * ev1 + y2
+
     def forward(self, FrameTensor, EventTensor):
         ev = self.Conv1(EventTensor)
-        from . import f16scale, fac as facmod, weightbank
+        from . import f16scale, fac as facmod, mod_fused, weightbank
         book = f16scale.active_book()
         c = self.KernelConv.conv2d
         site = weightbank.lookup(c.weight, "id") if (book is not None and conv.get_compute_dtype() == "bf16x3") else None
@@ -206,8 +214,11 @@
             fuse = self.KernelConv.native(FrameTensor)
             if fuse is not None and fuse[0] == conv.ACT_LEAKY and \
                     facmod.kernelconv_fac_train_usable(site, book, FrameTensor, ev, self.KPN.kernel_size):
-                ev1 = self.Conv3(facmod.KernelConvFacTrain.apply(FrameTensor, ev, site, fuse[1], self.KPN.kernel_size, c.weight, c.bias))
-                return FrameTensor * ev1 + self.Conv2(ev1)
+                fac_out = facmod.KernelConvFacTrain.apply(FrameTensor, ev, site, fuse[1], self.KPN.kernel_size, c.weight, c.bias)
+                tail_sites = mod_fused.usable(self, FrameTensor, fac_out, book)
+                if tail_sites is not None:
+                    return mod_fused.modification_tail(self, FrameTensor, fac_out, tail_sites)
+                return self._tail(FrameTensor, fac_out, book)
         fused = self._fused_filters_apply(ev, FrameTensor)
         if fused is not None:
             ev1 = self.Conv3(fused)
@@ -218,7 +229,7 @@
             filters = self.KernelConv(cat, grad_is_preact=True)
             if site is not None and torch.is_grad_enabled():
                 book.operand((site.key, "f"), filters)
-            ev1 = self.Conv3(self.KPN(ev, filters, kernel_leaky_slope=fuse[1]))
+            return self._tail(FrameTensor, self.KPN(ev, filters, kernel_leaky_slope=fuse[1]), book)
         else:
             ev1 = self.Conv3(self.KPN(ev, self.KernelConv(cat)))
         return FrameTensor * ev1 + self.Conv2(ev1)
diff --git a/include/ebfi_hip.h b/include/ebfi_hip.h
--- a/include/ebfi_hip.h
+++ b/include/ebfi_hip.h
@@ -143,6 +143,8 @@
 int ebfi_to_c16(const float *src, const float *mask_y, float mask_slope, void *dst16, void *slot, int B, int C, int H, int W,
                 void *stream);
 int ebfi_to_c16_cat2(const float *src0, int C0, const float *src1, int C1, void *dst16, void *slot, int B, int H, int W, void *stream);
+int ebfi_to_c16_mask16(const float *src, const void *mask16, float mask_slope, void *dst16, void *slot, int B, int C, int H, int W,
+                       void *stream);
 int ebfi_conv2d_packed_x3_c16(const void *input, const void *packed, size_t packed_bytes, const void *bias, void *output,
                               int B, int Cin_per_group, int H, int W, int Cout, int ksize, int pad, int groups, int act,
                               float slope, const void *addend, const void *mask_y, int mask_act, float mask_slope,
@@ -187,6 +189,14 @@
                              int Cin_per_group, int H, int W, int Cout, int groups, float slope, const void *post_scale,
                              const void *post_res, int res_channels, void *pre16, void *pre_slot, void *out16, void *slot16,
                              void *stream);
+int ebfi_conv2d_packed_x3_prodsum(const void *input, const void *packed, size_t packed_bytes, const void *bias, void *output,
+                                  int B, int Cin, int H, int W, int Cout, int act, float slope, const void *p, const void *q,
+                                  void *pre16, void *pre_slot, void *stream);
+int ebfi_conv2d_packed_f16_prodsum(const void *input, int input_is_c16, const void *packed16, size_t packed_bytes,
+                                   const void *bias, void *output, void *output2, int B, int Cin, int H, int W, int Cout, int act,
+                                   float slope, const void *g, const void *p, const void *q, const void *mask_y, int mask_is_c16,
+                                   float mask_slope, void *in_slot, const void *w_slot, void *out16, void *slot16, void *pre16,
+                                   void *pre_slot, void *stream);
 int ebfi_conv2d_backward_weight_x3g(const void *input, const void *grad_output, void *grad_weight, void *grad_bias,
                                     int B, int Cin_per_group, int H, int W, int Cout, int ksize, int pad, int groups,
                                     void *workspace, size_t workspace_bytes, void *stream);
```

Result: no change. 548.6 frames/s, median of 6 (+0.4%).
